# MultimodalFusion/multimodalfusion

Hardware: AMD Instinct MI355X
Metric: bags/sec fwd+bwd, path-AMIL 50k x 1024 synthetic bag (higher is better)
Workload: dtype f32; 1 GPU; path_attention_mil small gated K=4, one 50000x1024 N(0,1) bag per GPU per step, nll_surv alpha=0, train (1 dropout mask) mode, fwd+loss+bwd, grads materialised, one C-ABI call per bag (model.nll_step), 2 bags in flight per GPU on 2 HIP streams; instances_per_bag=50000, parallelism=dp1 (one bag per GPU per step), bags_in_flight=2

## Files before the change

### multimodalfusion_amd/csrc/mmf_amil_bwd.hip

```cpp
#include <cstdlib>

#include <type_traits>

#include "mmf_gemm_core.h"
#include "mmf_gemm_split.h"
#include "mmf_kernels.h"

namespace mmf {

__global__ __launch_bounds__(256) void bwd_prep_kernel(BwdPrepParams p) {
  __shared__ float red[4];
  const int tid = threadIdx.x, lane = tid & 63, wave = tid >> 6;
  const float m = p.stats[0], inv = 1.0f / p.stats[1];
  float dmm = 0.f;
  for (int c = lane; c < p.H; c += 64) dmm += p.dM[c] * p.M[c];
  dmm = wave_sum(dmm);
  float dbc = 0.f;
  const int64_t nw = (int64_t)gridDim.x * 4;
  for (int64_t i = (int64_t)blockIdx.x * 4 + wave; i < p.N; i += nw) {
    const float* hr = p.h + (size_t)i * p.H;
    float g = 0.f;
    for (int c = 4 * lane; c < p.H; c += 256) {
      float4 hv = ld4(hr + c), dv = ld4(p.dM + c);
      g += hv.x * dv.x + hv.y * dv.y + hv.z * dv.z + hv.w * dv.w;
    }
    g = wave_sum(g);
    if (lane == 0) {
      float pi = __expf(p.A_raw[i] - m) * inv;
      float d = pi * (g - dmm) + (p.gA ? p.gA[i] : 0.f);
      p.p[i] = pi;
      p.ds[i] = d;
      dbc += d;
    }
  }
  if (lane == 0) red[wave] = dbc;
  __syncthreads();
  if (tid == 0) p.dbc_part[blockIdx.x] = red[0] + red[1] + red[2] + red[3];
}

template <int ROWS, int NT, int MODE = -1, bool SEG = false>
struct LoadP_K {
  using Map = KMap<ROWS, NT>;
  GateBwdCtx g;
  rsrc_t ra, rb, rwc;
  int row0, tid, part, d0;
  uint32_t thr;
  float dscale;
  unsigned voff[Map::NV];
  uint32_t rbase[SEG ? Map::NV : 1];
  __device__ inline void init_seg(const uint32_t* ridx, int nrows) {
    if constexpr (SEG) {
#pragma unroll
      for (int i = 0; i < Map::NV; ++i) {
        const int rr = row0 + Map::row(tid, i);
        rbase[i] = (Map::valid(tid, i) && rr < nrows) ? ridx[rr] : 0u;
      }
    }
  }
  __device__ inline uint32_t idx_of(int i, int rr, int c) const {
    if constexpr (SEG) return rbase[i] + (uint32_t)c;
    else return (uint32_t)rr * (uint32_t)g.D + (uint32_t)c;
  }
  float dsr[Map::NV];
  float4 ra4[Map::NV], rb4[Map::NV], wc4;
  __device__ inline void init(const GateBwdCtx& g_, int row0_, int nrows) {
    g = g_; g.resolve_seed(); row0 = row0_; tid = threadIdx.x;
    thr = drop_threshold(g.drop_p);
    dscale = g.drop_p > 0.f ? 1.0f / (1.0f - g.drop_p) : 1.0f;
    const unsigned bytes = (unsigned)nrows * (unsigned)g.D * 4u;
    ra = make_rsrc(g.a, bytes);
    rb = make_rsrc(g.gated ? g.b : g.a, bytes);
    rwc = make_rsrc(g.Wc, (unsigned)g.D * 4u);
    rsrc_t rds = make_rsrc(g.ds, (unsigned)nrows * 4u);
#pragma unroll
    for (int i = 0; i < Map::NV; ++i) {
      int rr = row0 + Map::row(tid, i);
      bool ok = Map::valid(tid, i) && rr < nrows;
      voff[i] = ok ? ((unsigned)rr * (unsigned)g.D + 4u * Map::c4(tid, i)) * 4u : OOB;
      dsr[i] = bld1(rds, ok ? (unsigned)rr * 4u : OOB, 0);
    }
  }
  __device__ inline void init_lds(const GateBwdCtx& g_, int row0_, int nrows, const float* ds_lds) {
    g = g_; g.resolve_seed(); row0 = row0_; tid = threadIdx.x;
    thr = drop_threshold(g.drop_p);
    dscale = g.drop_p > 0.f ? 1.0f / (1.0f - g.drop_p) : 1.0f;
    const unsigned bytes = (unsigned)nrows * (unsigned)g.D * 4u;
    ra = make_rsrc(g.a, bytes);
    rb = make_rsrc(g.gated ? g.b : g.a, bytes);
    rwc = make_rsrc(g.Wc, (unsigned)g.D * 4u);
#pragma unroll
    for (int i = 0; i < Map::NV; ++i) {
      int rl = Map::row(tid, i), rr = row0 + rl;
      bool ok = Map::valid(tid, i) && rr < nrows;
      voff[i] = ok ? ((unsigned)rr * (unsigned)g.D + 4u * Map::c4(tid, i)) * 4u : OOB;
      dsr[i] = ok ? ds_lds[rl] : 0.f;
    }
  }
  __device__ inline void load_meta(int kt) {
    part = g.gated ? (kt & 1) : 0;
    d0 = (g.gated ? (kt >> 1) : kt) * KC;
  }
  __device__ inline void load(int kt) {
    load_meta(kt);
    if (part) return;
    const unsigned soff = (unsigned)d0 * 4u;
    wc4 = bld4(rwc, 16u * (tid & 7), soff);
#pragma unroll
    for (int i = 0; i < Map::NV; ++i) {
      ra4[i] = bld4(ra, voff[i], soff);
      rb4[i] = bld4(rb, voff[i], soff);
    }
  }
  template <bool GATED, bool DROP, int PART>
  __device__ inline void store_t(float* lds) const {
    const int c = d0 + 4 * (tid & 7);
#pragma unroll
    for (int i = 0; i < Map::NV; ++i) {
      if (!Map::valid(tid, i)) continue;
      int rr = row0 + Map::row(tid, i);
      uint32_t idx = idx_of(i, rr, c);
      float dummy;
      float4 o;
      o.x = gate_dp_t<GATED, DROP, PART>(g, ra4[i].x, rb4[i].x, wc4.x, dsr[i], idx + 0, thr, dscale, dummy);
      o.y = gate_dp_t<GATED, DROP, PART>(g, ra4[i].y, rb4[i].y, wc4.y, dsr[i], idx + 1, thr, dscale, dummy);
      o.z = gate_dp_t<GATED, DROP, PART>(g, ra4[i].z, rb4[i].z, wc4.z, dsr[i], idx + 2, thr, dscale, dummy);
      o.w = gate_dp_t<GATED, DROP, PART>(g, ra4[i].w, rb4[i].w, wc4.w, dsr[i], idx + 3, thr, dscale, dummy);
      st4(lds + Map::lds(tid, i), o);
    }
  }
  __device__ inline void store(float* lds) const {
    if constexpr (MODE >= 0) {
      constexpr bool GATED = (MODE & 2) != 0, DROP = (MODE & 1) != 0;
      if (GATED && part) store_t<GATED, DROP, 1>(lds);
      else store_t<GATED, DROP, 0>(lds);
      return;
    }
    const int c = d0 + 4 * (tid & 7);
#pragma unroll
    for (int i = 0; i < Map::NV; ++i) {
      if (!Map::valid(tid, i)) continue;
      int rr = row0 + Map::row(tid, i);
      uint32_t idx = idx_of(i, rr, c);
      float dummy;
      float4 o;
      o.x = gate_dp(g, part, ra4[i].x, rb4[i].x, wc4.x, dsr[i], idx + 0, thr, dscale, dummy);
      o.y = gate_dp(g, part, ra4[i].y, rb4[i].y, wc4.y, dsr[i], idx + 1, thr, dscale, dummy);
      o.z = gate_dp(g, part, ra4[i].z, rb4[i].z, wc4.z, dsr[i], idx + 2, thr, dscale, dummy);
      o.w = gate_dp(g, part, ra4[i].w, rb4[i].w, wc4.w, dsr[i], idx + 3, thr, dscale, dummy);
      st4(lds + Map::lds(tid, i), o);
    }
  }
};

template <int ROWS, int NT>
struct LoadWab_M {
  using Map = MMap<ROWS, NT>;
  rsrc_t ra, rb;
  bool gated;
  int D, tid;
  unsigned hb;
  unsigned voff[Map::NV];
  float4 r[Map::NV];
  __device__ inline void init(const float* wa, const float* wb, int H, int D_, int col0, bool gated_) {
    D = D_; tid = threadIdx.x; hb = (unsigned)H * 4u; gated = gated_ && wb != nullptr;
    ra = make_rsrc(wa, (unsigned)D * hb);
// ... 159 lines not shown
  __device__ inline void init_common(const GateBwdCtx& g_, int row0_, int nrows) {
    g = g_; g.resolve_seed(); row0 = row0_; tid = threadIdx.x;
    thr = drop_threshold(g.drop_p);
    dscale = g.drop_p > 0.f ? 1.0f / (1.0f - g.drop_p) : 1.0f;
    ra = make_rsrc(g.a, (unsigned)nrows * (unsigned)g.D * 4u);
    rwc = make_rsrc(g.Wc, (unsigned)g.D * 4u);
#pragma unroll
    for (int i = 0; i < NV; ++i) {
      const int idx = slot(tid, i), rr = row0 + krow(idx);
      voff[i] = rr < nrows ? ((unsigned)rr * (unsigned)g.D + 4u * (idx & 3)) * 4u : OOB;
    }
  }
  __device__ inline void init(const GateBwdCtx& g_, int row0_, int nrows) {
    init_common(g_, row0_, nrows);
    rsrc_t rds = make_rsrc(g.ds, (unsigned)nrows * 4u);
#pragma unroll
    for (int i = 0; i < NV; ++i) {
      const int rr = row0 + krow(slot(tid, i));
      dsr[i] = bld1(rds, rr < nrows ? (unsigned)rr * 4u : OOB, 0);
    }
  }
  __device__ inline void init_lds(const GateBwdCtx& g_, int row0_, int nrows, const float* ds_lds) {
    init_common(g_, row0_, nrows);
#pragma unroll
    for (int i = 0; i < NV; ++i) {
      const int rl = krow(slot(tid, i));
      dsr[i] = row0 + rl < nrows ? ds_lds[rl] : 0.f;
    }
  }
  __device__ inline void load(int kt) {
    d0 = kt * SKC;
    const unsigned soff = (unsigned)d0 * 4u;
    wc4 = bld4(rwc, 16u * (tid & 3), soff);
#pragma unroll
    for (int i = 0; i < NV; ++i) ra4[i] = bld4(ra, voff[i], soff);
  }
  __device__ inline void store_piece(float* lds, int i) const {
    const int c = d0 + 4 * (tid & 3);
    const int idx = slot(tid, i), rr = row0 + krow(idx);
    const uint32_t e0 = (uint32_t)rr * (uint32_t)g.D + (uint32_t)c;
    float dummy;
    float4 o;
    o.x = gate_dp_t<false, DROP, 0>(g, ra4[i].x, 0.f, wc4.x, dsr[i], e0 + 0, thr, dscale, dummy);
    o.y = gate_dp_t<false, DROP, 0>(g, ra4[i].y, 0.f, wc4.y, dsr[i], e0 + 1, thr, dscale, dummy);
    o.z = gate_dp_t<false, DROP, 0>(g, ra4[i].z, 0.f, wc4.z, dsr[i], e0 + 2, thr, dscale, dummy);
    o.w = gate_dp_t<false, DROP, 0>(g, ra4[i].w, 0.f, wc4.w, dsr[i], e0 + 3, thr, dscale, dummy);
    split_store4(lds + krow(idx) * SROW_F, idx & 3, o);
  }
  __device__ inline void store(float* lds) const {
#pragma unroll
    for (int i = 0; i < NV; ++i) store_piece(lds, i);
  }
};

template <int ROWS, int NT, bool GATED>
struct SplitWab_M {
  static constexpr int TOTAL = ROWS * 2, NV = (TOTAL + NT - 1) / NT, PIECES = NV;
  static_assert(TOTAL % NT == 0 || TOTAL < NT, "whole vector slots only");
  rsrc_t ra, rb;
  int tid;
  unsigned hb;
  unsigned voff[NV];
  float r[NV][8];
  __device__ inline void init(const float* wa, const float* wb, int H, int D, int col0, bool) {
    tid = TOTAL < NT ? (int)threadIdx.x % TOTAL : (int)threadIdx.x; hb = (unsigned)H * 4u;
    ra = make_rsrc(wa, (unsigned)D * hb);
    rb = make_rsrc(GATED ? wb : wa, (unsigned)D * hb);
#pragma unroll
    for (int i = 0; i < NV; ++i) {
      const int idx = tid + i * NT, c = col0 + idx % ROWS, kh = idx / ROWS;
      voff[i] = c < H ? (unsigned)(8 * kh) * hb + (unsigned)c * 4u : OOB;
    }
  }
  __device__ inline void load(int kt) {
    const bool second = GATED && (kt & 1);
    const unsigned soff = (unsigned)((GATED ? (kt >> 1) : kt) * SKC) * hb;
#pragma unroll
    for (int i = 0; i < NV; ++i)
#pragma unroll
      for (int j = 0; j < 8; ++j) r[i][j] = bld1(second ? rb : ra, voff[i], soff + (unsigned)j * hb);
  }
  __device__ inline void store_piece(float* lds, int i) const {
    const int idx = tid + i * NT;
    split_store8(lds + (idx % ROWS) * SROW_F, idx / ROWS, r[i]);
  }
  __device__ inline void store(float* lds) const {
#pragma unroll
    for (int i = 0; i < NV; ++i) store_piece(lds, i);
  }
};

template <class T, class LA, class LB>
__device__ inline void dh_split_mainloop(const LA& la0, const LB& lb0, int nk, float* lds, f32x16 (&acc)[T::MB][T::NB]) {
  const int tid = threadIdx.x, lane = tid & 63, wave = tid >> 6;
  const int wm = wave / T::WN, wn = wave % T::WN;
#pragma unroll
  for (int mb = 0; mb < T::MB; ++mb)
#pragma unroll
    for (int nb = 0; nb < T::NB; ++nb)
#pragma unroll
      for (int i = 0; i < 16; ++i) acc[mb][nb][i] = 0.f;
  LA la[2] = {la0, la0};
  LB lb[4] = {lb0, lb0, lb0, lb0};
  la[0].load_pair(0); la[1].load_pair(2);
#pragma unroll
  for (int j = 0; j < 4; ++j) lb[j].load(j);
  la[0].template store_part<0>(lds);
  lb[0].store(lds + T::A_FLOATS);
  __syncthreads();
  constexpr int NS = split_steps<T>();
  for (int kt0 = 0; kt0 < nk; kt0 += 4) {
    static_for<4>([&](auto jc) {
      constexpr int j = decltype(jc)::value;
      const int kt = kt0 + j;
      float* cur = lds + (j & 1) * T::STAGE_FLOATS;
      float* nxt = lds + ((j + 1) & 1) * T::STAGE_FLOATS;
      compute_chunk_split<T>(cur, cur + T::A_FLOATS, acc, wm, wn, lane, [&](int s) {
        if (s == 0) {
          if constexpr (j == 1) la[0].load_pair(kt0 + 4);
          else if constexpr (j == 3) la[1].load_pair(kt0 + 6);
        }
        if (s == (NS >= 4 ? 1 : 0)) lb[j].load(kt + 4);
        constexpr int PA = LA::NV;
#pragma unroll
        for (int q = 0; q < PA; ++q)
          if (s == q * (NS - 1) / PA) la[((j + 1) & 3) >> 1].template store_part_piece<(j + 1) & 1>(nxt, q);
        if (s == NS - 1) lb[(j + 1) & 3].store(nxt + T::A_FLOATS);
      });
      __syncthreads();
    });
  }
}

template <class T, bool FUSED, int MODE = -1, bool SEG = false>
__global__ __launch_bounds__(T::NT) void bwd_dh_kernel(BwdDhParams p) {
  static_assert(!(SEG && (FUSED || T::SPLIT)), "the grouped step runs K-prep on its own and the exact-fp32 tiles");
  extern __shared__ __align__(16) float lds[];
  int mt, nt;
  if (!tile_of_block(blockIdx.x, p.mt_count, p.nt_count, mt, nt)) return;
  const int row0 = mt * T::BM, col0 = nt * T::BN;
  const int tid = threadIdx.x, lane = tid & 63, wave = tid >> 6;
  float* ds_l = lds + 2 * T::STAGE_FLOATS;
  float* p_l = ds_l + T::BM;
  constexpr bool SGATED = T::SPLIT && MODE >= 2;
  std::conditional_t<T::SPLIT,
                     std::conditional_t<SGATED, SplitP_K<T::BM, T::NT, (SGATED ? MODE : 2)>, SplitP_U<T::BM, T::NT, (T::SPLIT && !SGATED ? MODE : 0)>>,
                     LoadP_K<T::BM, T::NT, MODE, SEG>> la;
  if constexpr (FUSED) {
    constexpr int NW = T::NT / 64;
    constexpr int RPW = (T::BM + NW - 1) / NW;
    float* g_l = p_l + T::BM + 16;
    const int LPR = p.H / 4;
    const int PPL = LPR / 64;
    float4 dm_l[4];
#pragma unroll
    for (int q = 0; q < 4; ++q) dm_l[q] = q < PPL ? ld4(p.dM + 4 * (lane + 64 * q)) : zero4();
    float dmm = 0.f;
    for (int c = lane; c < p.H; c += 64) dmm += p.dM[c] * p.Mpool[c];
    const float smax = p.stats[0], inv = 1.0f / p.stats[1];
    static_assert(T::BM <= T::NT, "one row per thread in K-prep");
    const int prow = row0 + tid;
    const bool pok = tid < T::BM && prow < p.N;
    const float araw = pok ? p.A_raw[prow] : 0.f;
    const float gav = (pok && p.gA) ? p.gA[prow] : 0.f;
    const int wr0 = wave * RPW, wr1 = wr0 + RPW < T::BM ? wr0 + RPW : T::BM;
    auto g_rows = [&](auto nrows_c, int rb) {
      constexpr int NR = decltype(nrows_c)::value;
      float part[NR];
#pragma unroll
      for (int u = 0; u < NR; ++u) {
        const int row = row0 + rb + u;
        const int rc = row < p.N ? row : (int)p.N - 1;
        float acc = 0.f;
#pragma unroll
        for (int q = 0; q < 4; ++q)
          if (q < PPL) {
            const float4 hv = ld4(p.h + (size_t)rc * p.H + 4 * (lane + 64 * q));
            acc += hv.x * dm_l[q].x + hv.y * dm_l[q].y + hv.z * dm_l[q].z + hv.w * dm_l[q].w;
          }
        part[u] = acc;
      }
#pragma unroll
      for (int u = 0; u < NR; ++u) part[u] = wave_sum(part[u]);
      if (lane < NR && rb + lane < wr1) {
        float gv = part[0];
#pragma unroll
        for (int u = 1; u < NR; ++u) gv = lane == u ? part[u] : gv;
        g_l[rb + lane] = gv;
      }
    };
    if (PPL == 1) {
      for (int rb = wr0; rb < wr1; rb += 16) g_rows(std::integral_constant<int, 16>{}, rb);
    } else {
      for (int rb = wr0; rb < wr1; rb += 8) g_rows(std::integral_constant<int, 8>{}, rb);
    }
    dmm = wave_sum(dmm);
    __syncthreads();
    float dbc = 0.f;
    if (tid < T::BM) {
      float pi = 0.f, d = 0.f;
      if (pok) {
        pi = __expf(araw - smax) * inv;
        d = pi * (g_l[tid] - dmm) + gav;
        if (nt == 0) { p.p_out[prow] = pi; p.ds_out[prow] = d; }
      }
      ds_l[tid] = d;
      p_l[tid] = pi;
      dbc = d;
    }
    dbc = wave_sum(dbc);
    float* red = p_l + T::BM;
    if (lane == 0) red[wave] = dbc;
    __syncthreads();
    if (tid == 0 && nt == 0) {
      float s = 0.f;
      for (int w = 0; w < NW; ++w) s += red[w];
      p.dbc_part[mt] = s;
    }
    la.init_lds(p.g, row0, (int)p.N, ds_l);
  } else {
    la.init(p.g, row0, (int)p.N);
    if constexpr (SEG && !T::SPLIT) la.init_seg(p.seg_ridx, (int)p.N);
  }
  std::conditional_t<T::SPLIT, SplitWab_M<T::BN, T::NT, SGATED>, LoadWab_M<T::BN, T::NT>> lb;
  lb.init(p.Wa, p.Wb, p.H, p.g.D, col0, p.g.gated != 0);
  f32x16 acc[T::MB][T::NB];
  f32x4acc acch[T::NB][2];
  const int nk = (p.g.gated ? 2 : 1) * p.g.D / (T::SPLIT ? SKC : KC);
  if constexpr (SGATED) {
    dh_split_mainloop<T>(la, lb, nk, lds, acc);
  } else if constexpr (T::SPLIT) {
    split_mainloop<T, 4>(la, lb, nk, lds, acc);
  } else if constexpr (T::NT == 256 && T::BM <= 64) {
    if (p.deep && p.g.gated) dh_mainloop_deep<T>(la, lb, nk, lds, acc);
    else gemm_mainloop<T, decltype(la), decltype(lb), false>(la, lb, nk, lds, acc);
  } else {
    gemm_mainloop<T, decltype(la), decltype(lb), FUSED && MODE >= 0>(la, lb, nk, lds, acc, acch);
  }
  {
    const int wm = wave / T::WN, wn = wave % T::WN;
    const int rr = lane >> 3, c4 = lane & 7;
    float* blk = lds + wave * (32 * EPI_STRIDE);
    constexpr int NBLK = T::MB * T::NB;
    float4 dm4[T::NB];
#pragma unroll
    for (int nb = 0; nb < T::NB; ++nb) {
      const int col = col0 + epilogue_col<T>(nb);
      dm4[nb] = (!SEG && p.dM && col < p.H) ? ld4(p.dM + col) : zero4();
    }
    if (p.relu_bits) {
      const int cbn = p.H >> 5;
      typedef unsigned long long u64;
      u64 mv[2];
      auto fetch_bits = [&](int b, int s) {
        const int mb = b / T::NB, nb = b % T::NB;
        const int64_t rb16 = (((int64_t)row0 + wm * (T::BM / T::WM) + mb * 32) >> 4) + (lane >> 3);
        const int cb = (col0 >> 5) + wn * T::NB + nb;
        const bool ok = rb16 * 16 < p.N && cb < cbn && lane < (mb == T::MB ? 8 : 16);
        mv[s] = ok ? p.relu_bits[((size_t)rb16 * cbn + cb) * 8 + (lane & 7)] : 0ull;
      };
      fetch_bits(0, 0);
#pragma unroll
      for (int b = 0; b < NBLK; ++b) {
        const int mb = b / T::NB, nb = b % T::NB, s = b & 1;
        if (b + 1 < NBLK) fetch_bits(b + 1, s ^ 1);
        float4 v[4];
        transpose_block(acc[mb][nb], blk, lane, v);
        const int r = wm * (T::BM / T::WM) + mb * 32 + rr, col = col0 + (wn * T::NB + nb) * 32 + 4 * c4;
        if (col >= p.H) continue;
        const float4 dm_c = dm4[nb];
#pragma unroll
        for (int t = 0; t < 4; ++t) {
          const int row = row0 + r + 8 * t;
          const float pi = FUSED ? p_l[r + 8 * t] : p.p[row < p.N ? row : (int)p.N - 1];
          const float4 dm = SEG ? ld4(p.dM + (size_t)p.seg_bag[row < p.N ? row : (int)p.N - 1] * p.H + col) : dm_c;
          const float raw[4] = {(v[t].x + pi * dm.x) * p.scale_h, (v[t].y + pi * dm.y) * p.scale_h,
                                (v[t].z + pi * dm.z) * p.scale_h, (v[t].w + pi * dm.w) * p.scale_h};
          float o[4];
#pragma unroll
          for (int e = 0; e < 4; ++e) {
            const unsigned lo = __builtin_amdgcn_readlane((unsigned)mv[s], 4 * t + e);
            const unsigned hi = __builtin_amdgcn_readlane((unsigned)(mv[s] >> 32), 4 * t + e);
            const u64 m = ((u64)hi << 32) | lo;
            asm volatile("v_cndmask_b32_e64 %0, 0, %1, %2" : "=v"(o[e]) : "v"(raw[e]), "s"(m));
          }
          if (row < p.N) st4(p.du + (size_t)row * p.H + col, make_float4(o[0], o[1], o[2], o[3]));
        }
      }
      if constexpr (T::HALF) {
#pragma unroll
        for (int nb = 0; nb < T::NB; ++nb) {
          fetch_bits(T::MB * T::NB + nb, 0);
          float4 v[2];
          transpose_half(acch[nb][0], acch[nb][1], blk, lane, v);
          const int r = wm * (T::BM / T::WM) + T::MB * 32 + rr, col = col0 + (wn * T::NB + nb) * 32 + 4 * c4;
          if (col >= p.H) continue;
          const float4 dm_c = dm4[nb];
#pragma unroll
          for (int t = 0; t < 2; ++t) {
            const int row = row0 + r + 8 * t;
            const float pi = FUSED ? p_l[r + 8 * t] : p.p[row < p.N ? row : (int)p.N - 1];
            const float4 dm = SEG ? ld4(p.dM + (size_t)p.seg_bag[row < p.N ? row : (int)p.N - 1] * p.H + col) : dm_c;
            const float raw[4] = {(v[t].x + pi * dm.x) * p.scale_h, (v[t].y + pi * dm.y) * p.scale_h,
                                  (v[t].z + pi * dm.z) * p.scale_h, (v[t].w + pi * dm.w) * p.scale_h};
            float o[4];
#pragma unroll
            for (int e = 0; e < 4; ++e) {
              const unsigned lo = __builtin_amdgcn_readlane((unsigned)mv[0], 4 * t + e);
              const unsigned hi = __builtin_amdgcn_readlane((unsigned)(mv[0] >> 32), 4 * t + e);
              const u64 m = ((u64)hi << 32) | lo;
              asm volatile("v_cndmask_b32_e64 %0, 0, %1, %2" : "=v"(o[e]) : "v"(raw[e]), "s"(m));
            }
            if (row < p.N) st4(p.du + (size_t)row * p.H + col, make_float4(o[0], o[1], o[2], o[3]));
          }
        }
      }
    } else {
    float4 hv[2][4];
    float pv[2][4];
    auto fetch = [&](int b, int s) {
      const int mb = b / T::NB, nb = b % T::NB;
      const int r = (wm * T::MB + mb) * 32 + rr, col = col0 + (wn * T::NB + nb) * 32 + 4 * c4;
#pragma unroll
      for (int t = 0; t < 4; ++t) {
        const int row = row0 + r + 8 * t;
        const int rc = row < p.N ? row : (int)p.N - 1;
        hv[s][t] = !p.h ? make_float4(1.f, 1.f, 1.f, 1.f) : (col < p.H ? ld4(p.h + (size_t)rc * p.H + col) : zero4());
        pv[s][t] = FUSED ? p_l[r + 8 * t] : (p.p ? p.p[rc] : 0.f);
      }
    };
    fetch(0, 0);
#pragma unroll
    for (int b = 0; b < NBLK; ++b) {
      const int mb = b / T::NB, nb = b % T::NB, s = b & 1;
      if (b + 1 < NBLK) fetch(b + 1, s ^ 1);
      float4 v[4];
      transpose_block(acc[mb][nb], blk, lane, v);
      const int r = (wm * T::MB + mb) * 32 + rr, col = col0 + (wn * T::NB + nb) * 32 + 4 * c4;
      if (col >= p.H) continue;
      const float4 dm_c = dm4[nb];
#pragma unroll
      for (int t = 0; t < 4; ++t) {
        const int row = row0 + r + 8 * t;
        if (row >= p.N) continue;
        const float4 dm = SEG ? ld4(p.dM + (size_t)p.seg_bag[row] * p.H + col) : dm_c;
        const float4 h4 = hv[s][t];
        const float pi = pv[s][t];
        float4 du;
        du.x = h4.x > 0.f ? (v[t].x + pi * dm.x) * p.scale_h : 0.f;
        du.y = h4.y > 0.f ? (v[t].y + pi * dm.y) * p.scale_h : 0.f;
        du.z = h4.z > 0.f ? (v[t].z + pi * dm.z) * p.scale_h : 0.f;
        du.w = h4.w > 0.f ? (v[t].w + pi * dm.w) * p.scale_h : 0.f;
        st4(p.du + (size_t)row * p.H + col, du);
      }
    }
    }
// ... 392 lines not shown
#pragma unroll
      for (int t = 0; t < 4; ++t) {
        const int row = rowmap(wm * 128 + 4 * (rr + 8 * t) + mb);
        if (row < 0) continue;
        float* o = out + (size_t)row * q.ldc + col;
        if (col < q.Ncols) st4(o, make_float4(v0[t].x, v1[t].x, v0[t].y, v1[t].y));
        if (col + 4 < q.Ncols) st4(o + 4, make_float4(v0[t].z, v1[t].z, v0[t].w, v1[t].w));
      }
    }
    return;
  }
  epilogue_rows<T>(acc, lds, [&](int mb, int nb, int r, int c, const float4 (&v)[4]) {
    const int col = tn * T::BN + c;
    if (col >= q.Ncols) return;
#pragma unroll
    for (int t = 0; t < 4; ++t) {
      const int row = rowmap(r + 8 * t);
      if (row >= 0) st4(out + (size_t)row * q.ldc + col, v[t]);
    }
  });
}

template <class T, bool GATED, int DROP>
__device__ inline void tn_gate_tile(const TnParams& p, const TnProblem& q,
                                    std::conditional_t<T::SPLIT, SplitM<T::BN, T::NT>, LoadM<T::BN, T::NT>>& lb, int split, int tm,
                                    int tn, int kbase, int kmax, int nk, int last_groups, bool do_sum, float* lds) {
  using LA = std::conditional_t<T::SPLIT, SplitA_M_Gate<T::BM, T::NT, GATED, (DROP > 0 ? 1 : 0)>, LoadA_M_Gate<T::BM, T::NT, GATED, DROP>>;
  constexpr int DT = LA::DT;
  const int D = p.g.D, d0 = tm * DT;
  LA la;
  la.init(p.g, d0, kbase, kmax, do_sum);
  if constexpr (!T::SPLIT && DROP == 2) la.rrix = make_rsrc(p.seg_ridx, (unsigned)(kmax > 0 ? kmax : 0) * 4u);
  f32x16 acc[T::MB][T::NB];
  if constexpr (T::SPLIT) split_mainloop<T, 2>(la, lb, nk, lds, acc);
  else gemm_mainloop<T>(la, lb, nk, lds, acc, nullptr, last_groups);
  tn_store<T>(q, split, tn, acc, lds, [&](int r) {
    const int half = r / DT, d = d0 + r - half * DT;
    return d < D ? half * D + d : -1;
  });
  if constexpr (T::SPLIT) {
    if (do_sum) {
      float* cs = q.colsum + (size_t)split * q.colsum_stride;
      colsum1_reduce_store<DT, T::NT>(lds, la.csum_a, cs, d0, D);
      if (GATED) colsum1_reduce_store<DT, T::NT>(lds, la.csum_b, cs + D, d0, D);
      if (q.colsum2) colsum1_reduce_store<DT, T::NT>(lds, la.csum2, q.colsum2 + (size_t)split * q.colsum2_stride, d0, D);
    }
  } else
  if (do_sum) {
    float* cs = q.colsum + (size_t)split * q.colsum_stride;
    colsum_reduce_store<DT, T::NT>(lds, la.csum_a, cs, d0, D);
    if (GATED) colsum_reduce_store<DT, T::NT>(lds, la.csum_b, cs + D, d0, D);
    if (q.colsum2) colsum_reduce_store<DT, T::NT>(lds, la.csum2, q.colsum2 + (size_t)split * q.colsum2_stride, d0, D);
  }
}

template <class T, int DROP = -1>
__global__ __launch_bounds__(T::NT) void tn_kernel(TnParams p) {
  extern __shared__ __align__(16) float lds[];
  const int b = blockIdx.x;
  int split, pi = 0, t;
  if (p.xcd_map == 2) {
    const unsigned e = p.map[b];
    if (e == 0xFFFFu) return;
    split = (int)(e >> 5);
    const int tg = (int)(e & 31u);
    for (int i = 1; i < p.nprob; ++i)
      if (tg >= p.prob[i].tile_begin) pi = i;
    t = tg - p.prob[pi].tile_begin;
  } else {
    for (int i = 1; i < p.nprob; ++i)
      if (b >= p.prob[i].block_begin) pi = i;
    const int rel = b - p.prob[pi].block_begin, nt = p.prob[pi].tiles_m * p.prob[pi].tiles_n;
    split = rel / nt;
    t = rel - split * nt;
  }
  const TnProblem& q = p.prob[pi];
  if (split >= q.splits) return;
  const int tm = t / q.tiles_n, tn = t - tm * q.tiles_n;
  const int64_t kb64 = (int64_t)split * q.k_per_split;
  const int kbase = (int)(kb64 < p.K ? kb64 : p.K);
  const int kmax = (int)((kb64 + q.k_per_split) < p.K ? (kb64 + q.k_per_split) : p.K);
  constexpr int CH = T::SPLIT ? SKC : KC;
  const int nk = T::SPLIT ? 2 * ((kmax - kbase + 2 * CH - 1) / (2 * CH)) : (kmax - kbase + CH - 1) / CH;
  int last_groups = 0;
  if constexpr (!T::SPLIT) last_groups = nk > 0 ? ((kmax - kbase) - (nk - 1) * KC + 2 * T::G - 1) / (2 * T::G) : 0;
  const bool do_sum = tn == 0 && q.colsum != nullptr;

  std::conditional_t<T::SPLIT, SplitM<T::BN, T::NT>, LoadM<T::BN, T::NT>> lb;
  lb.init(q.B, q.ldb, tn * T::BN, q.Ncols, kbase, kmax);
  if (q.kind == TN_A_PLAIN) {
    std::conditional_t<T::SPLIT, SplitA_M_Plain<T::BM, T::NT>, LoadA_M_Plain<T::BM, T::NT>> la;
    la.init(q.A, q.lda, tm * T::BM, q.M, kbase, kmax, do_sum);
    f32x16 acc[T::MB][T::NB];
    if constexpr (T::SPLIT) split_mainloop<T, 2>(la, lb, nk, lds, acc);
    else gemm_mainloop<T>(la, lb, nk, lds, acc, nullptr, last_groups);
    tn_store<T>(q, split, tn, acc, lds, [&](int r) { const int row = tm * T::BM + r; return row < q.M ? row : -1; });
    if (do_sum) {
      if constexpr (T::SPLIT) colsum1_reduce_store<T::BM, T::NT>(lds, la.csum, q.colsum + (size_t)split * q.colsum_stride, tm * T::BM, q.M);
      else colsum_reduce_store<T::BM, T::NT>(lds, la.csum, q.colsum + (size_t)split * q.colsum_stride, tm * T::BM, q.M);
    }
  } else if (p.g.gated) {
    tn_gate_tile<T, true, DROP>(p, q, lb, split, tm, tn, kbase, kmax, nk, last_groups, do_sum, lds);
  } else {
    tn_gate_tile<T, false, DROP>(p, q, lb, split, tm, tn, kbase, kmax, nk, last_groups, do_sum, lds);
  }
}

__global__ __launch_bounds__(256) void reduce_kernel(ReduceParams p) {
  const int b = blockIdx.x;
  int si = 0;
  for (int i = 1; i < p.nseg; ++i)
    if (b >= p.seg[i].block_begin) si = i;
  const ReduceSeg& s = p.seg[si];
  if (s.len < 4) {
    __shared__ float red[4];
    for (int e = 0; e < s.len; ++e) {
      float acc = 0.f;
      for (int k = threadIdx.x; k < s.nsplit; k += 256) acc += s.in[(size_t)k * s.stride + e];
      acc = wave_sum(acc);
      if ((threadIdx.x & 63) == 0) red[threadIdx.x >> 6] = acc;
      __syncthreads();
      if (threadIdx.x == 0) s.out[e] = (p.accumulate ? s.out[e] : 0.f) + (red[0] + red[1] + red[2] + red[3]);
      __syncthreads();
    }
    return;
  }
  if (s.tall) {
    __shared__ __align__(16) float part[16][64];
    const int cq = threadIdx.x & 15, grp = threadIdx.x >> 4;
    const int j = (b - s.block_begin) * 64 + 4 * cq;
    float4 acc = zero4();
    if (j < s.len) {
      const float* in = s.in + j;
      int k = grp;
      for (; k + 7 * 16 < s.nsplit; k += 8 * 16) {
        float4 v[8];
#pragma unroll
        for (int u = 0; u < 8; ++u) v[u] = ld4(in + (size_t)(k + 16 * u) * s.stride);
#pragma unroll
        for (int u = 0; u < 8; ++u) { acc.x += v[u].x; acc.y += v[u].y; acc.z += v[u].z; acc.w += v[u].w; }
      }
      for (; k < s.nsplit; k += 16) {
        float4 v = ld4(in + (size_t)k * s.stride);
        acc.x += v.x; acc.y += v.y; acc.z += v.z; acc.w += v.w;
      }
    }
    st4(&part[grp][4 * cq], acc);
    __syncthreads();
    if (threadIdx.x < 64) {
      float t = 0.f;
#pragma unroll
      for (int g = 0; g < 16; ++g) t += part[g][threadIdx.x];
      const int c = (b - s.block_begin) * 64 + threadIdx.x;
      if (c < s.len) s.out[c] = (p.accumulate ? s.out[c] : 0.f) + t;
    }
    return;
  }
  const int j = ((b - s.block_begin) * 256 + threadIdx.x) * 4;
  if (j >= s.len) return;
  if ((s.len & 3) == 0 && (s.stride & 3) == 0) {
    float4 acc = zero4();
    const float* in = s.in + j;
    int k = 0;
    for (; k + 8 <= s.nsplit; k += 8) {
      float4 v[8];
#pragma unroll
      for (int u = 0; u < 8; ++u) v[u] = ld4(in + (size_t)(k + u) * s.stride);
#pragma unroll
      for (int u = 0; u < 8; ++u) { acc.x += v[u].x; acc.y += v[u].y; acc.z += v[u].z; acc.w += v[u].w; }
    }
    for (; k < s.nsplit; ++k) {
      float4 v = ld4(in + (size_t)k * s.stride);
      acc.x += v.x; acc.y += v.y; acc.z += v.z; acc.w += v.w;
    }
    if (p.accumulate) { const float4 o = ld4(s.out + j); acc.x += o.x; acc.y += o.y; acc.z += o.z; acc.w += o.w; }
    st4(s.out + j, acc);
  } else {
    for (int e = j; e < j + 4 && e < s.len; ++e) {
      float acc = 0.f;
      for (int k = 0; k < s.nsplit; ++k) acc += s.in[(size_t)k * s.stride + e];
      s.out[e] = (p.accumulate ? s.out[e] : 0.f) + acc;
    }
  }
}

int launch_bwd_prep(BwdPrepParams p, hipStream_t st) {
  if (p.H % 4 != 0 || p.H > 1024) return MMF_ERR_SHAPE;
  { ProfScope ps("bwd_prep_kernel", st); hipLaunchKernelGGL(bwd_prep_kernel, dim3(p.n_groups), dim3(256), 0, st, p); }
  return hipGetLastError() == hipSuccess ? MMF_OK : MMF_ERR_LAUNCH;
}

constexpr int DH_MAX_ROWS = 224;

DhPlan plan_bwd_dh(int64_t N, int H, int D, int gated, int dropout, int split, int concurrent, int can_fuse, int dbc_cap) {
  static const int fuse_env = tune_int("MMF_FUSED_PREP", 1);
  static const int short_max = tune_int("MMF_DH_SHORT_MAX", 1024);
  static const int min_64x128 = tune_int("MMF_DH_64X128", 13000);
  const int mode = (gated ? 2 : 0) + (dropout ? 1 : 0);
  const bool split_k = split && ((gated ? 2 : 1) * D / SKC) % 4 == 0;
  const bool split_wide = split_k && use_wide_tiles(N, H, 1);
  const bool split_64 = split_k && !use_wide_tiles(N, H, 1) && N >= split_min_rows();
  const bool wide = use_wide_tiles(N, H, split);
  const bool big = (N / 128) * ((H + 127) / 128) >= 256;
  const bool deep_k = gated && (2 * D / KC) % 4 == 0;
  const bool short_64 = !use_wide_tiles(N, H, split_64) && !big && ((N + 63) / 64) * ((H + 63) / 64) <= short_max;
  auto wide_rows = [&](bool allow_half) {
    const int r = pick_wide_rows(N, H / 256, allow_half, concurrent != 0, DH_MAX_ROWS);
    return r >= 64 && r <= DH_MAX_ROWS && r % 16 == 0 ? r : 224;
  };

  int fuse_rows = 0;
  if (short_64) fuse_rows = 64;
  else if (split_64 || !wide) fuse_rows = 0;
  else fuse_rows = split_wide ? 224 : wide_rows(true);
  DhPlan pl{};
  pl.fused = can_fuse && fuse_env && fuse_rows > 0 && (N + fuse_rows - 1) / fuse_rows <= dbc_cap;
  pl.variant = -1;
  if (pl.fused && split_wide) {
    pl.kind = DH_SPLIT_WIDE; pl.rows = 224; pl.nt_count = H / 256; pl.variant = mode;
  } else if (split_64) {
    pl.kind = DH_SPLIT_64; pl.rows = 64; pl.nt_count = (H + 63) / 64; pl.variant = mode;
  } else if (wide) {
    pl.kind = DH_WIDE; pl.rows = pl.fused ? fuse_rows : wide_rows(false); pl.nt_count = H / 256;
    if (pl.fused && mode < 3) pl.variant = mode;
  } else if (big) {
    pl.kind = DH_128; pl.rows = 128; pl.nt_count = (H + 127) / 128;
  } else if (min_64x128 > 0 && N >= min_64x128 && pl.fused && deep_k && H % 128 == 0) {
    pl.kind = DH_64X128; pl.rows = 64; pl.nt_count = H / 128; pl.deep = 1;
  } else {
    pl.kind = DH_64; pl.rows = 64; pl.nt_count = (H + 63) / 64;
  }
  pl.mt_count = (int)((N + pl.rows - 1) / pl.rows);
  if (pl.kind == DH_64) pl.deep = short_grid((int64_t)pl.mt_count * pl.nt_count) && deep_k ? 1 : 0;
  pl.grid = grid_for_tiles(pl.mt_count, pl.nt_count);
  pl.extra_lds = pl.fused ? (3 * pl.rows + 16) * 4 : 0;
  pl.dbc_groups = pl.fused ? pl.mt_count : 0;
  return pl;
}

template <class T_, bool FUSED_, bool PLAIN_>
struct DhTile { using T = T_; static constexpr bool FUSED = FUSED_, PLAIN = PLAIN_; };
template <int ROWS>
using DhWide = DhTile<Tile<ROWS, 256, 1, 8, true, false>, true, ROWS % 32 == 0>;

template <class F>
static int with_dh_tile(const DhPlan& pl, F&& f) {
  switch (pl.kind) {
    case DH_SPLIT_WIDE: return f(DhTile<TileSp<224, 256, 1, 8>, true, false>{});
    case DH_SPLIT_64: return f(DhTile<TileSp<64, 64, 2, 2>, true, true>{});
    case DH_128: return f(DhTile<Tile<128, 128, 2, 2, true, false>, false, true>{});
    case DH_64X128: return f(DhTile<Tile<64, 128, 2, 2, true, false>, true, false>{});
    case DH_64: return f(DhTile<Tile<64, 64, 2, 2, true, false>, true, true>{});
    case DH_WIDE: return with_wide_rows<DH_MAX_ROWS>(pl.rows, [&](auto r) { return f(DhWide<decltype(r)::value>{}); });
  }
  return MMF_ERR_ARG;
}

template <int LAST, class F>
static int with_variant(int variant, F&& f) {
  switch (variant) {
    case 0: return f(std::integral_constant<int, 0>{});
    case 1: return f(std::integral_constant<int, 1>{});
    case 2: return f(std::integral_constant<int, 2>{});
    default: return f(std::integral_constant<int, LAST>{});
  }
}

template <bool SEG>
static int launch_dh_plan(const DhPlan& pl, BwdDhParams p, hipStream_t st) {
  if (p.g.D % KC != 0 || p.H % 4 != 0) return MMF_ERR_SHAPE;
  if (SEG && (pl.fused || p.split || !p.seg_bag || !p.seg_ridx || !p.dM || !p.p || !p.h)) return MMF_ERR_ARG;
  if (p.N <= 0) return MMF_OK;
  p.mt_count = pl.mt_count; p.nt_count = pl.nt_count; p.deep = pl.deep; p.fused_prep = pl.fused;
  return with_dh_tile(pl, [&](auto tile) -> int {
    using E = decltype(tile);
    using T = typename E::T;
    using Yes = std::true_type;
    using No = std::false_type;
    using RunTime = std::integral_constant<int, -1>;
    auto go = [&](auto fused, auto mode) -> int {
      return launch_tiled<T>(T::SPLIT ? "bwd_dh_split_kernel" : "bwd_dh_kernel",
                             bwd_dh_kernel<T, decltype(fused)::value, decltype(mode)::value, SEG>, p, pl.grid, st, pl.extra_lds);
    };
    if constexpr (SEG) {
      if constexpr (E::PLAIN && !T::SPLIT) return go(No{}, RunTime{});
    } else if (pl.fused) {
      if constexpr (E::FUSED && T::SPLIT) return with_variant<3>(pl.variant, [&](auto mode) { return go(Yes{}, mode); });
      else if constexpr (E::FUSED && T::BN == 256) return with_variant<-1>(pl.variant, [&](auto mode) { return go(Yes{}, mode); });
      else if constexpr (E::FUSED) return go(Yes{}, RunTime{});
    } else if constexpr (E::PLAIN) {
      if constexpr (T::SPLIT) return with_variant<3>(pl.variant, [&](auto mode) { return go(No{}, mode); });
      else return go(No{}, RunTime{});
    }
    return MMF_ERR_ARG;
  });
}
int launch_bwd_dh(const DhPlan& pl, BwdDhParams p, hipStream_t st) { return launch_dh_plan<false>(pl, p, st); }
int launch_bwd_dh_seg(const DhPlan& pl, BwdDhParams p, hipStream_t st) { return launch_dh_plan<true>(pl, p, st); }

__global__ __launch_bounds__(256) void group_bwd_prep_kernel(BwdPrepParams p, const int* bag) {
  __shared__ float red[4];
  const int tid = threadIdx.x, lane = tid & 63, wave = tid >> 6;
  int cur = -1;
  float dmm = 0.f, m = 0.f, inv = 1.f;
  const float* dM = p.dM;
  float dbc = 0.f;
  const int64_t nw = (int64_t)gridDim.x * 4;
  for (int64_t i = (int64_t)blockIdx.x * 4 + wave; i < p.N; i += nw) {
    const int b = __builtin_amdgcn_readfirstlane(bag[i]);
    if (b != cur) {
      cur = b;
      dM = p.dM + (size_t)b * p.H;
      const float* M = p.M + (size_t)b * p.H;
      float t = 0.f;
      for (int c = lane; c < p.H; c += 64) t += dM[c] * M[c];
      dmm = wave_sum(t);
      m = p.stats[2 * b];
      inv = 1.0f / p.stats[2 * b + 1];
    }
    const float* hr = p.h + (size_t)i * p.H;
    float gsum = 0.f;
    for (int c = 4 * lane; c < p.H; c += 256) {
      float4 hv = ld4(hr + c), dv = ld4(dM + c);
      gsum += hv.x * dv.x + hv.y * dv.y + hv.z * dv.z + hv.w * dv.w;
    }
    gsum = wave_sum(gsum);
    if (lane == 0) {
      float pi = __expf(p.A_raw[i] - m) * inv;
      float d = pi * (gsum - dmm) + (p.gA ? p.gA[i] : 0.f);
      p.p[i] = pi;
      p.ds[i] = d;
      dbc += d;
    }
  }
  if (lane == 0) red[wave] = dbc;
  __syncthreads();
  if (tid == 0) p.dbc_part[blockIdx.x] = red[0] + red[1] + red[2] + red[3];
}
int launch_group_bwd_prep(BwdPrepParams p, const int* bag, hipStream_t st) {
  if (!bag || p.n_groups < 1) return MMF_ERR_ARG;
  { ProfScope ps("group_bwd_prep_kernel", st); hipLaunchKernelGGL(group_bwd_prep_kernel, dim3(p.n_groups), dim3(256), 0, st, p, bag); }
  return hipGetLastError() == hipSuccess ? MMF_OK : MMF_ERR_LAUNCH;
}

template <bool ATTR, bool SEG = false>
static int launch_nn_tiles(NnParams p, hipStream_t st) {
  const char* name = SEG ? "gemm_nn_attr_seg_kernel" : ATTR ? "gemm_nn_attr_kernel" : "gemm_nn_kernel";
  const int ntn = (p.N + 127) / 128;
  if ((p.M / 128) * ntn >= 256) {
    using T = Tile<128, 128, 2, 2, true, false>;
    p.mt_count = (int)((p.M + 127) / 128); p.nt_count = ntn;
    return launch_tiled<T>(name, gemm_nn_kernel<T, ATTR, SEG>, p, grid_for_tiles(p.mt_count, p.nt_count), st);
  }
  using T = Tile<64, 64, 2, 2, true, false>;
  p.mt_count = (int)((p.M + 63) / 64); p.nt_count = (p.N + 63) / 64;
  return launch_tiled<T>(name, gemm_nn_kernel<T, ATTR, SEG>, p, grid_for_tiles(p.mt_count, p.nt_count), st);
}

int launch_nn(NnParams p, hipStream_t st) {
  if (p.K % KC != 0 || p.lda % 4 != 0 || p.ldb % 4 != 0 || p.N % 4 != 0) return MMF_ERR_SHAPE;
  if (p.M <= 0) return MMF_OK;
  return launch_nn_tiles<false>(p, st);
}

int launch_nn_attr(NnParams p, float* row_sum, float* row_abs, hipStream_t st) {
  if (!p.mulx || !p.rs_part || !p.ra_part || !row_sum || !row_abs) return MMF_ERR_ARG;
  if (p.K % KC != 0 || p.lda % 4 != 0 || p.ldb % 4 != 0 || p.N % 32 != 0 || p.ldx % 4 != 0 || (p.C && p.ldc % 4 != 0))
    return MMF_ERR_SHAPE;
  if (p.M <= 0) return MMF_OK;
  if (int e = launch_nn_tiles<true>(p, st)) return e;
  ProfScope ps("ig_rows_kernel", st);
  hipLaunchKernelGGL(ig_rows_kernel, dim3((unsigned)((p.M + 255) / 256)), dim3(256), 0, st, p.rs_part, p.ra_part, p.M,
                     p.N / 32, row_sum, row_abs);
  return hipGetLastError() == hipSuccess ? MMF_OK : MMF_ERR_LAUNCH;
}

int launch_nn_attr_seg(NnParams p, float* row_sum, float* row_abs, hipStream_t st) {
  if (!p.rs_part || !p.ra_part || !row_sum || !row_abs) return MMF_ERR_ARG;
  if (p.kseg < 32 || p.kseg % 32 != 0 || p.N % p.kseg != 0 || p.N / p.kseg < 1 || p.N / p.kseg > 4) return MMF_ERR_SHAPE;
  const int nseg = p.N / p.kseg;
  for (int m = 0; m < nseg; ++m)
    if (!p.segx[m]) return MMF_ERR_ARG;
  if (p.K % KC != 0 || p.lda % 4 != 0 || p.ldb % 4 != 0) return MMF_ERR_SHAPE;
  if (p.M <= 0) return MMF_OK;
  if (int e = launch_nn_tiles<true, true>(p, st)) return e;
  const int64_t n = p.M * nseg;
  ProfScope ps("ig_rows_seg_kernel", st);
  hipLaunchKernelGGL(ig_rows_seg_kernel, dim3((unsigned)((n + 255) / 256)), dim3(256), 0, st, p.rs_part, p.ra_part, p.M,
                     p.kseg / 32, nseg, row_sum, row_abs);
  return hipGetLastError() == hipSuccess ? MMF_OK : MMF_ERR_LAUNCH;
}

int launch_ig_fold(const IgFoldParams& p, hipStream_t st) {
  if (!p.du || !p.G) return MMF_ERR_ARG;
  if (p.H % 4 != 0 || p.N < 1 || p.st.S < 0 || p.st.S > GROUP_MAX) return MMF_ERR_SHAPE;
  if (p.st.S == 0 && !p.first) return MMF_OK;
  const size_t n4 = (size_t)p.N * p.H / 4;
  ProfScope ps("ig_fold_kernel", st);
  hipLaunchKernelGGL(ig_fold_kernel, dim3((unsigned)((n4 + 255) / 256)), dim3(256), 0, st, p);
  return hipGetLastError() == hipSuccess ? MMF_OK : MMF_ERR_LAUNCH;
}

TnPlan plan_tn(int64_t K, int split, const TnShape* shapes, int nshape) {
  static const int env_wide = tune_int("MMF_TN_WIDE", 1);
  static const int kmin = tune_int("MMF_TN_WIDE_MIN", 12288);
  static const int env_splits = tune_int("MMF_TN_SPLITS", 0);
  static const int env_gate = tune_int("MMF_TN_GATE_SPLITS", -1);
  TnPlan pl{};
  pl.tile = env_wide && K >= kmin ? 256 : 128;
  pl.kind = pl.tile == 256 ? (split ? TN_SPLIT_256 : TN_256) : (split && K >= split_min_rows() ? TN_SPLIT_128 : TN_128);
  const int td = pl.tile;
  int t_plain = 0, t_gate = 0;
  for (int i = 0; i < nshape; ++i)
    (shapes[i].gate ? t_gate : t_plain) += ((shapes[i].M + td - 1) / td) * ((shapes[i].Ncols + td - 1) / td);
  pl.tiles = t_plain + t_gate;
  auto capped = [&](int64_t s) { if (s > (K + 127) / 128) s = (K + 127) / 128; return (int)(s < 1 ? 1 : s); };
  auto kps = [&](int s) { return (int)(((K + s - 1) / s + 3) / 4 * 4); };
  pl.splits = capped(env_splits > 0 ? env_splits : (td == 256 ? 256 : 512) / (pl.tiles > 0 ? pl.tiles : 1));
  pl.k_per_split = kps(pl.splits);
  pl.splits_g = pl.splits;
  if (t_plain > 0 && t_gate > 0) {
    if (td == 256 && pl.splits >= 8) {
      const int cap = pl.splits + (pl.splits * 12 + 99) / 100;
      const int sg = (256 - t_plain * pl.splits) / t_gate;
      pl.splits_g = sg > cap ? cap : sg < pl.splits ? pl.splits : sg;
    }
    if (env_gate > 0) pl.splits_g = env_gate;
  }
  pl.k_per_split_g = kps(pl.splits_g);
  return pl;
}

template <class T>
static int launch_tn_grid(const TnParams& p, int grid, hipStream_t st) {
  if constexpr (!T::SPLIT) {
    if (p.seg_ridx && p.g.drop_p > 0.f) return launch_tiled<T>("tn_kernel", tn_kernel<T, 2>, p, grid, st);
  }
  if constexpr (T::BM == 256 || T::SPLIT) {
    const char* name = T::SPLIT ? "tn_split_kernel" : "tn_kernel";
    if (p.g.drop_p > 0.f) return launch_tiled<T>(name, tn_kernel<T, 1>, p, grid, st);
    return launch_tiled<T>(name, tn_kernel<T, 0>, p, grid, st);
  } else {
    return launch_tiled<T>("tn_kernel", tn_kernel<T>, p, grid, st);
  }
}

template <class T>
static int launch_tn_t(const TnPlan& pl, TnParams p, hipStream_t st) {
  p.tile = pl.tile; p.splits = pl.splits; p.k_per_split = pl.k_per_split;
  int tiles = 0, blocks = 0;
  for (int i = 0; i < p.nprob; ++i) {
    TnProblem& q = p.prob[i];
    if (q.Ncols % 4 != 0 || q.ldb % 4 != 0 || q.M % 4 != 0) return MMF_ERR_SHAPE;
    if (q.kind == TN_A_PLAIN && q.lda % 4 != 0) return MMF_ERR_SHAPE;
    q.splits = q.kind == TN_A_GATE ? pl.splits_g : pl.splits;
    q.k_per_split = q.kind == TN_A_GATE ? pl.k_per_split_g : pl.k_per_split;
    if (q.k_per_split % 4 != 0 || q.k_per_split < 4) return MMF_ERR_ARG;
    if (q.kind == TN_A_GATE) {
      const int dt = p.g.gated ? T::BM / 2 : T::BM;
      q.tiles_m = (p.g.D + dt - 1) / dt;
    } else {
      q.tiles_m = (q.M + T::BM - 1) / T::BM;
    }
    q.tiles_n = (q.Ncols + T::BN - 1) / T::BN;
    q.tile_begin = tiles;
    q.block_begin = blocks;
    tiles += q.tiles_m * q.tiles_n;
    blocks += q.tiles_m * q.tiles_n * q.splits;
  }
  if (blocks == 0) return MMF_OK;
  p.total_tiles = tiles;
  static const int env_xcd = tune_int("MMF_TN_XCD", -1);
  p.xcd_map = env_xcd == 0 ? 0 : 2;
  if (p.xcd_map == 2) {
    int bin_load[8] = {0, 0, 0, 0, 0, 0, 0, 0};
    bool ok = tiles <= 32;
    for (int i = 0; i < 512; ++i) p.map[i] = 0xFFFFu;
    int order[6], np = p.nprob;
    for (int i = 0; i < np; ++i) order[i] = i;
    for (int i = 0; i < np; ++i)
      for (int j = i + 1; j < np; ++j)
        if (p.prob[order[j]].tiles_m * p.prob[order[j]].tiles_n > p.prob[order[i]].tiles_m * p.prob[order[i]].tiles_n) {
          const int t = order[i]; order[i] = order[j]; order[j] = t;
        }
    for (int oi = 0; oi < np && ok; ++oi) {
      const TnProblem& q = p.prob[order[oi]];
      const int n = q.tiles_m * q.tiles_n;
      if (n == 0) continue;
      if (q.splits >= 2048) { ok = false; break; }
      for (int s = 0; s < q.splits && ok; ++s) {
        int x = 0;
        for (int k = 1; k < 8; ++k) if (bin_load[k] < bin_load[x]) x = k;
        if (8 * (bin_load[x] + n) > 512) { ok = false; break; }
        for (int t = 0; t < n; ++t) p.map[x + 8 * (bin_load[x] + t)] = (uint16_t)((s << 5) | (q.tile_begin + t));
        bin_load[x] += n;
      }
    }
    if (ok) {
      int mx = 0;
      for (int k = 0; k < 8; ++k) mx = bin_load[k] > mx ? bin_load[k] : mx;
      return launch_tn_grid<T>(p, 8 * mx, st);
    }
    p.xcd_map = 0;
  }
  return launch_tn_grid<T>(p, blocks, st);
}

int launch_tn(const TnPlan& pl, TnParams p, hipStream_t st) {
  switch (pl.kind) {
    case TN_SPLIT_256: return launch_tn_t<TileSp<256, 256, 2, 4>>(pl, p, st);
    case TN_256: return launch_tn_t<Tile<256, 256, 2, 4, false, false, 2>>(pl, p, st);
    case TN_SPLIT_128: return launch_tn_t<TileSp<128, 128, 2, 2>>(pl, p, st);
    case TN_128: return launch_tn_t<Tile<128, 128, 2, 2, false, false, 2>>(pl, p, st);
  }
  return MMF_ERR_ARG;
}

int launch_reduce(ReduceParams p, hipStream_t st) {
  int blocks = 0;
  for (int i = 0; i < p.nseg; ++i) {
    ReduceSeg& s = p.seg[i];
    s.tall = s.nsplit >= 64 && s.len >= 4 && (s.len & 3) == 0 && (s.stride & 3) == 0;
    s.block_begin = blocks;
    blocks += s.tall ? (s.len + 63) / 64 : (s.len + 1023) / 1024;
  }
  if (blocks == 0) return MMF_OK;
  { ProfScope ps("reduce_kernel", st); hipLaunchKernelGGL(reduce_kernel, dim3(blocks), dim3(256), 0, st, p); }
  return hipGetLastError() == hipSuccess ? MMF_OK : MMF_ERR_LAUNCH;
}

}
```

### multimodalfusion_amd/csrc/mmf_amil_fwd.hip

```cpp
#include <cstdlib>

#include "mmf_gemm_core.h"
#include "mmf_gemm_split.h"
#include "mmf_kernels.h"

namespace mmf {

__device__ inline float apply_act(float v, int act) {
  switch (act) {
    case ACT_RELU: return fmaxf(v, 0.f);
    case ACT_TANH: return fast_tanh(v);
    case ACT_SIGMOID: return fast_sigmoid(v);
    case ACT_SELU: {
      const float alpha = 1.6732632423543772f, scale = 1.0507009873554805f;
      return scale * (v > 0.f ? v : alpha * (__expf(v) - 1.0f));
    }
    default: return v;
  }
}

struct PartSrc {
  unsigned bytes;
  unsigned base;
  unsigned slab;
  int S;
};

template <class T, int ACT, bool DROP, bool SEG = false>
__device__ inline void linear_epilogue(const LinearParams& p, f32x16 (&acc)[T::MB][T::NB], f32x4acc (*acch)[2], float* lds,
                                       int row0, int col0, const PartSrc ps = PartSrc{}) {
  const uint32_t thr = drop_threshold(p.drop_p);
  const float scale = DROP ? 1.0f / (1.0f - p.drop_p) : 1.0f;
  const uint32_t dkey = p.drop_key + (p.seed_dev ? *p.seed_dev : 0u);
  float4 bias4[T::NB];
#pragma unroll
  for (int nb = 0; nb < T::NB; ++nb) {
    const int col = col0 + epilogue_col<T>(nb);
    bias4[nb] = (p.bias && col < p.N) ? ld4(p.bias + col) : zero4();
  }
  const int lane = threadIdx.x & 63;
  auto rows_op = [&](auto nt_c, int nb, int r, int c, const float4* v) {
    constexpr int NTR = decltype(nt_c)::value;
    const int col = col0 + c;
    const bool col_ok = col < p.N;
    const float4 b4 = bias4[nb];
    unsigned long long mine = 0ull;
#pragma unroll
    for (int t = 0; t < NTR; ++t) {
      const int row = row0 + r + 8 * t;
      const bool ok = col_ok && row < p.M;
      float y[4] = {v[t].x + b4.x, v[t].y + b4.y, v[t].z + b4.z, v[t].w + b4.w};
      uint32_t idx;
      if constexpr (SEG) idx = (row < p.M ? p.seg_ridx[row] : 0u) + (uint32_t)col;
      else idx = (uint32_t)row * (uint32_t)p.N + (uint32_t)col;
#pragma unroll
      for (int e = 0; e < 4; ++e) {
        if constexpr (ACT == ACT_RELU) y[e] = fmaxf(y[e], 0.f);
        else if constexpr (ACT < 0) y[e] = apply_act(y[e], p.act);
        if constexpr (DROP) y[e] = keep(dkey, idx + e, thr) ? y[e] * scale : 0.f;
      }
      if (p.relu_bits) {
#pragma unroll
        for (int e = 0; e < 4; ++e) {
          const unsigned long long bal = __ballot(ok && y[e] > 0.f);
          if (lane == 4 * t + e) mine = bal;
        }
      }
      if (ok) st4(p.y + (size_t)row * p.N + col, make_float4(y[0], y[1], y[2], y[3]));
    }
    if (p.relu_bits && lane < 4 * NTR) {
      const size_t rb16 = ((size_t)(row0 + r - (lane >> 3)) >> 4) + (lane >> 3), cb = (size_t)(col0 + c - 4 * (lane & 7)) >> 5;
      if ((int64_t)rb16 * 16 < p.M && (int)(cb * 32) < p.N) p.relu_bits[(rb16 * (size_t)(p.N >> 5) + cb) * 8 + (lane & 7)] = mine;
    }
  };
  if (ps.S > 0) {
    const int wave = threadIdx.x >> 6, wm = wave / T::WN, wn = wave % T::WN;
    const int rr = lane >> 3, c4 = lane & 7;
    constexpr int NBLK = T::MB * T::NB;
    const rsrc_t prs = make_rsrc(p.kpart, ps.bytes);
    float4 buf[2][4];
    auto fetch = [&](int b, int rows4, float4 (&v)[4]) {
      const int mb = b / T::NB, nb = b % T::NB;
      const int r = wm * (T::BM / T::WM) + mb * 32 + rr, c = (wn * T::NB + nb) * 32 + 4 * c4;
#pragma unroll
      for (int t = 0; t < 4; ++t) {
        if (t >= rows4) break;
        const unsigned o = ps.base + (unsigned)((r + 8 * t) * T::BN + c) * 4u;
        float4 a = bld4_dev(prs, o, 0);
        for (int k = 1; k < ps.S; ++k) {
          const float4 q = bld4_dev(prs, o, (unsigned)k * ps.slab);
          a.x += q.x; a.y += q.y; a.z += q.z; a.w += q.w;
        }
        v[t] = a;
      }
    };
    fetch(0, 4, buf[0]);
#pragma unroll
    for (int b = 0; b < NBLK; ++b) {
      const int mb = b / T::NB, nb = b % T::NB;
      if (b + 1 < NBLK) fetch(b + 1, 4, buf[(b + 1) & 1]);
      else if constexpr (T::HALF) fetch(T::MB * T::NB, 2, buf[(b + 1) & 1]);
      rows_op(std::integral_constant<int, 4>{}, nb, wm * (T::BM / T::WM) + mb * 32 + rr, (wn * T::NB + nb) * 32 + 4 * c4, buf[b & 1]);
    }
    if constexpr (T::HALF) {
#pragma unroll
      for (int nb = 0; nb < T::NB; ++nb) {
        if (nb + 1 < T::NB) fetch(T::MB * T::NB + nb + 1, 2, buf[(NBLK + nb + 1) & 1]);
        rows_op(std::integral_constant<int, 2>{}, nb, wm * (T::BM / T::WM) + T::MB * 32 + rr, (wn * T::NB + nb) * 32 + 4 * c4,
                buf[(NBLK + nb) & 1]);
      }
    }
    return;
  }
  epilogue_rows<T>(acc, lds, [&](int mb, int nb, int r, int c, const float4 (&v)[4]) {
    rows_op(std::integral_constant<int, 4>{}, nb, r, c, v);
  });
  if constexpr (T::HALF) {
    const int wave = threadIdx.x >> 6, wm = wave / T::WN, wn = wave % T::WN;
    float* blk = lds + wave * (32 * EPI_STRIDE);
#pragma unroll
    for (int nb = 0; nb < T::NB; ++nb) {
      float4 v[2];
      transpose_half(acch[nb][0], acch[nb][1], blk, lane, v);
      rows_op(std::integral_constant<int, 2>{}, nb, wm * (T::BM / T::WM) + T::MB * 32 + (lane >> 3),
              (wn * T::NB + nb) * 32 + 4 * (lane & 7), v);
    }
  }
}

template <class T>
__device__ inline bool ksplit_publish(const LinearParams& p, f32x16 (&acc)[T::MB][T::NB], f32x4acc (*acch)[2], float* lds,
                                      int tile, int ks, PartSrc& ps) {
  const int S = p.ksplit;
  ps.bytes = (unsigned)((size_t)p.mt_count * p.nt_count * S * T::BM * T::BN * 4u);
  const rsrc_t prs = make_rsrc(p.kpart, ps.bytes);
  ps.slab = (unsigned)(T::BM * T::BN * 4);
  ps.base = (unsigned)tile * (unsigned)S * ps.slab;
  ps.S = S;
  const unsigned mine = ps.base + (unsigned)ks * ps.slab;
  epilogue_rows<T>(acc, lds, [&](int mb, int nb, int r, int c, const float4 (&v)[4]) {
#pragma unroll
    for (int t = 0; t < 4; ++t) bst4_dev(prs, mine + (unsigned)((r + 8 * t) * T::BN + c) * 4u, 0, v[t]);
  });
  if constexpr (T::HALF) {
    const int lane = threadIdx.x & 63, wave = threadIdx.x >> 6, wm = wave / T::WN, wn = wave % T::WN;
    float* blk = lds + wave * (32 * EPI_STRIDE);
#pragma unroll
    for (int nb = 0; nb < T::NB; ++nb) {
      float4 v[2];
      transpose_half(acch[nb][0], acch[nb][1], blk, lane, v);
      const int r = wm * (T::BM / T::WM) + T::MB * 32 + (lane >> 3), c = (wn * T::NB + nb) * 32 + 4 * (lane & 7);
#pragma unroll
      for (int t = 0; t < 2; ++t) bst4_dev(prs, mine + (unsigned)((r + 8 * t) * T::BN + c) * 4u, 0, v[t]);
    }
  }
  asm volatile("s_waitcnt vmcnt(0)" ::: "memory");
  __syncthreads();
  unsigned* flag = reinterpret_cast<unsigned*>(lds + (T::NT / 64) * 32 * EPI_STRIDE);
  if (threadIdx.x == 0) {
    const unsigned old = __hip_atomic_fetch_add(p.ktick + tile, 1u, __ATOMIC_RELAXED, __HIP_MEMORY_SCOPE_AGENT);
    if (old == (unsigned)(S - 1)) __hip_atomic_store(p.ktick + tile, 0u, __ATOMIC_RELAXED, __HIP_MEMORY_SCOPE_AGENT);
    flag[0] = old;
  }
  __syncthreads();
  return flag[0] == (unsigned)(S - 1);
}

template <class T, bool SEG = false>
__global__ __launch_bounds__(T::NT) void linear_nt_kernel(LinearParams p) {
  extern __shared__ __align__(16) float lds[];
  const int S = p.ksplit > 1 ? p.ksplit : 1;
  int mt, ntk;
  if (!tile_of_block(blockIdx.x, p.mt_count, p.nt_count * S, mt, ntk)) return;
  const int nt = ntk % p.nt_count, ks = ntk / p.nt_count;
  const int row0 = mt * T::BM, col0 = nt * T::BN;
  const int nk = p.K / KC / S;

  LoadK<T::BM, T::NT> la;
  la.init_segments(p.x, p.nseg, p.kseg, p.ldx, row0, (int)p.M);
  LoadK<T::BN, T::NT> lb;
  lb.init(p.w, p.K, col0, p.N);
  la.kt0 = lb.kt0 = ks * nk;

  f32x16 acc[T::MB][T::NB];
  f32x4acc acch[T::NB][2];
  if constexpr (T::NT == 256 && T::BM <= 64) {
    if (p.deep) gemm_mainloop_deep<T, 4>(la, lb, nk, lds, acc);
    else gemm_mainloop<T>(la, lb, nk, lds, acc);
  } else {
    gemm_mainloop<T>(la, lb, nk, lds, acc, acch);
  }
  PartSrc ps{};
  if (S > 1) {
    if (!ksplit_publish<T>(p, acc, acch, lds, mt * p.nt_count + nt, ks, ps)) return;
  }
  const bool drop = p.drop_p > 0.f;
  if constexpr (SEG) {
    linear_epilogue<T, ACT_RELU, true, true>(p, acc, acch, lds, row0, col0, ps);
    return;
  }
  if (p.act == ACT_RELU) {
    if (drop) linear_epilogue<T, ACT_RELU, true>(p, acc, acch, lds, row0, col0, ps);
    else linear_epilogue<T, ACT_RELU, false>(p, acc, acch, lds, row0, col0, ps);
  } else if (p.act == ACT_NONE && !drop) {
    linear_epilogue<T, ACT_NONE, false>(p, acc, acch, lds, row0, col0, ps);
  } else if (drop) {
    linear_epilogue<T, -1, true>(p, acc, acch, lds, row0, col0, ps);
  } else {
    linear_epilogue<T, -1, false>(p, acc, acch, lds, row0, col0, ps);
  }
}

template <class T>
__global__ __launch_bounds__(T::NT) void linear_nt_split_kernel(LinearParams p) {
  extern __shared__ __align__(16) float lds[];
  int mt, nt;
  if (!tile_of_block(blockIdx.x, p.mt_count, p.nt_count, mt, nt)) return;
  const int row0 = mt * T::BM, col0 = nt * T::BN;
  SplitK<T::BM, T::NT> la;
  la.init(p.x[0], p.ldx, row0, (int)p.M);
  SplitK<T::BN, T::NT> lb;
  lb.init(p.w, p.K, col0, p.N);
  f32x16 acc[T::MB][T::NB];
  split_mainloop<T, 4>(la, lb, p.K / SKC, lds, acc);
  const bool drop = p.drop_p > 0.f;
  if (p.act == ACT_RELU) {
    if (drop) linear_epilogue<T, ACT_RELU, true>(p, acc, nullptr, lds, row0, col0);
    else linear_epilogue<T, ACT_RELU, false>(p, acc, nullptr, lds, row0, col0);
  } else if (p.act == ACT_NONE && !drop) {
    linear_epilogue<T, ACT_NONE, false>(p, acc, nullptr, lds, row0, col0);
  } else if (drop) {
    linear_epilogue<T, -1, true>(p, acc, nullptr, lds, row0, col0);
  } else {
    linear_epilogue<T, -1, false>(p, acc, nullptr, lds, row0, col0);
  }
}

template <int ROWS, int NT, bool GATED, bool HALVES>
struct LoadGateW {
  using Map = KMap<ROWS, NT>;
  rsrc_t ra, rb;
  int tid;
  int which[Map::NV];
  unsigned voff[Map::NV];
  float4 r[Map::NV];
  __device__ inline void init(const float* wa, const float* wb, int H, int D, int d0) {
    tid = threadIdx.x;
    ra = make_rsrc(wa, (unsigned)D * (unsigned)H * 4u);
    rb = make_rsrc(GATED ? wb : wa, (unsigned)D * (unsigned)H * 4u);
#pragma unroll
    for (int i = 0; i < Map::NV; ++i) {
      const int j = Map::row(tid, i);
      int w, d;
      if (!GATED) { w = 0; d = d0 + j; }
      else if (HALVES) { w = j >= ROWS / 2 ? 1 : 0; d = d0 + j - w * (ROWS / 2); }
      else { w = (j >> 5) & 1; d = d0 + (j >> 6) * 32 + (j & 31); }
      which[i] = __builtin_amdgcn_readfirstlane(w);
      voff[i] = (Map::valid(tid, i) && d < D) ? ((unsigned)d * (unsigned)H + 4u * Map::c4(tid, i)) * 4u : OOB;
    }
  }
  __device__ inline void load(int kt) {
    const unsigned soff = (unsigned)(kt * KC) * 4u;
#pragma unroll
    for (int i = 0; i < Map::NV; ++i) r[i] = bld4(which[i] ? rb : ra, voff[i], soff);
  }
  __device__ inline void store(float* lds) const {
#pragma unroll
    for (int i = 0; i < Map::NV; ++i)
      if (Map::valid(tid, i)) st4(lds + Map::lds(tid, i), r[i]);
  }
};

template <class T, bool GATED, bool SEG = false>
__device__ inline void gate_fwd_tile(const GateFwdParams& p, float* lds, int row0, int nt);

template <class T, bool GATED, bool SEG = false>
__global__ __launch_bounds__(T::NT) void gate_fwd_kernel(GateFwdParams p) {
  extern __shared__ __align__(16) float lds[];
  int mt, nt;
  if (!tile_of_block(blockIdx.x, p.mt_count, p.nt_count, mt, nt)) return;
  gate_fwd_tile<T, GATED, SEG>(p, lds, (int)p.row_begin + mt * T::BM, nt);
}

template <class TB, class TS, bool GATED, bool SEG = false>
__global__ __launch_bounds__(TB::NT) void gate_fwd_mixed_kernel(GateFwdParams p) {
  static_assert(TB::NT == TS::NT && TB::BN == TS::BN, "mixed tiles share the launch shape");
  extern __shared__ __align__(16) float lds[];
  int r = 0;
  for (int i = 1; i < p.nreg; ++i)
    if ((int)blockIdx.x >= p.reg[i].grid_begin) r = i;
  int mt, nt;
  if (!tile_of_block(blockIdx.x - p.reg[r].grid_begin, p.reg[r].mt_count, p.nt_count, mt, nt)) return;
  if (p.reg[r].tall) gate_fwd_tile<TB, GATED, SEG>(p, lds, (int)p.reg[r].row0 + mt * TB::BM, nt);
  else gate_fwd_tile<TS, GATED, SEG>(p, lds, (int)p.reg[r].row0 + mt * TS::BM, nt);
}

template <class T, bool GATED, bool SEG>
__device__ inline void gate_fwd_tile(const GateFwdParams& p, float* lds, int row0, int nt) {
  constexpr int DT = GATED ? T::BN / 2 : T::BN;
  const int d0 = nt * DT;

  std::conditional_t<T::SPLIT, SplitK<T::BM, T::NT>, LoadK<T::BM, T::NT>> la;
  la.init(p.h, p.H, row0, (int)p.row_end);
  std::conditional_t<T::SPLIT, SplitGateW<T::BN, T::NT, GATED>, LoadGateW<T::BN, T::NT, GATED, false>> lb;
  lb.init(p.Wa, p.Wb, p.H, p.D, d0);

  f32x16 acc[T::MB][T::NB];
  if constexpr (T::SPLIT) {
    split_mainloop<T, 4>(la, lb, p.H / SKC, lds, acc);
  } else if constexpr (T::BM <= 64) {
    if (p.deep) gemm_mainloop_deep<T, 4>(la, lb, p.H / KC, lds, acc);
    else gemm_mainloop<T>(la, lb, p.H / KC, lds, acc);
  } else {
    gemm_mainloop<T>(la, lb, p.H / KC, lds, acc);
  }

  const int tid = threadIdx.x, lane = tid & 63, wave = tid >> 6;
  const int wm = wave / T::WN, wn = wave % T::WN;
  const int rr = lane >> 3, c4 = lane & 7;
  const uint32_t thr = drop_threshold(p.drop_p);
  const bool drop = p.drop_p > 0.f;
  const float dscale = drop ? 1.0f / (1.0f - p.drop_p) : 1.0f;
  const uint32_t sdev = p.seed_dev ? *p.seed_dev : 0u;
  const uint32_t key_a = p.key_a + sdev, key_b = p.key_b + sdev;
  float* blk = lds + wave * (32 * EPI_STRIDE);
  float* sred = lds + (T::NT / 64) * (32 * EPI_STRIDE);

  constexpr int NPAIR = GATED ? T::NB / 2 : T::NB;
  float4 ba_r[NPAIR], bb_r[NPAIR], wc_r[NPAIR];
#pragma unroll
  for (int t = 0; t < NPAIR; ++t) {
    const int d = d0 + (wn * NPAIR + t) * 32 + 4 * c4;
    const bool dok = d < p.D;
    ba_r[t] = dok ? ld4(p.ba + d) : zero4();
    bb_r[t] = (GATED && dok) ? ld4(p.bb + d) : zero4();
    wc_r[t] = dok ? ld4(p.Wc + d) : zero4();
  }
#pragma unroll
  for (int mb = 0; mb < T::MB; ++mb) {
    float rowsum[4] = {0.f, 0.f, 0.f, 0.f};
#pragma unroll
    for (int t = 0; t < NPAIR; ++t) {
      const int d = d0 + (wn * NPAIR + t) * 32 + 4 * c4;
      const bool dok = d < p.D;
      float4 va[4], vb[4];
      transpose_block(acc[mb][GATED ? 2 * t : t], blk, lane, va);
      if constexpr (GATED) transpose_block(acc[mb][2 * t + 1], blk, lane, vb);
      const float4 ba4 = ba_r[t], bb4 = bb_r[t], wc4 = wc_r[t];
#pragma unroll
      for (int q = 0; q < 4; ++q) {
        const int row = row0 + (wm * T::MB + mb) * 32 + rr + 8 * q;
        float av[4] = {fast_tanh(va[q].x + ba4.x), fast_tanh(va[q].y + ba4.y), fast_tanh(va[q].z + ba4.z), fast_tanh(va[q].w + ba4.w)};
        float bv[4] = {1.f, 1.f, 1.f, 1.f};
        if constexpr (GATED) {
          bv[0] = fast_sigmoid(vb[q].x + bb4.x); bv[1] = fast_sigmoid(vb[q].y + bb4.y);
          bv[2] = fast_sigmoid(vb[q].z + bb4.z); bv[3] = fast_sigmoid(vb[q].w + bb4.w);
        }
        if (row < p.row_end && dok) {
          const size_t o = (size_t)row * p.D + d;
          if (p.a) {
            st4(p.a + o, make_float4(av[0], av[1], av[2], av[3]));
            if constexpr (GATED) st4(p.b + o, make_float4(bv[0], bv[1], bv[2], bv[3]));
          }
          const float wc[4] = {wc4.x, wc4.y, wc4.z, wc4.w};
          uint32_t idx;
          if constexpr (SEG) idx = p.seg_ridx[row] + (uint32_t)d;
          else idx = (uint32_t)row * (uint32_t)p.D + (uint32_t)d;
          if (drop) {
#pragma unroll
            for (int e = 0; e < 4; ++e) {
              const float ad = keep(key_a, idx + e, thr) ? av[e] * dscale : 0.f;
              float bd = bv[e];
              if constexpr (GATED) bd = keep(key_b, idx + e, thr) ? bd * dscale : 0.f;
              rowsum[q] += ad * bd * wc[e];
            }
          } else {
#pragma unroll
            for (int e = 0; e < 4; ++e) rowsum[q] += av[e] * bv[e] * wc[e];
          }
        }
      }
    }
#pragma unroll
    for (int q = 0; q < 4; ++q) {
      float s = rowsum[q];
      s += __shfl_xor(s, 1, 64); s += __shfl_xor(s, 2, 64); s += __shfl_xor(s, 4, 64);
      if (c4 == 0) sred[wn * T::BM + (wm * T::MB + mb) * 32 + rr + 8 * q] = s;
    }
  }
  __syncthreads();
  for (int i = tid; i < T::BM; i += T::NT) {
    int row = row0 + i;
    if (row < p.row_end) {
      float s = 0.f;
#pragma unroll
      for (int w = 0; w < T::WN; ++w) s += sred[w * T::BM + i];
      p.s_part[(size_t)nt * p.N + row] = s;
    }
  }
}


__device__ __forceinline__ void pool_partial_rows(const PoolParams& p, int g, int64_t r0, int64_t r1) {
  __shared__ float s_lds[POOL_MAX_ROWS];
  __shared__ float red[256];
  __shared__ __align__(16) float vred[1024];
  const int tid = threadIdx.x;
  const int nrows = r1 > r0 ? (int)(r1 - r0) : 0;
  const float bc = p.bc ? p.bc[0] : 0.f;

  float lmax = -INFINITY;
  for (int i = tid; i < nrows; i += 256) {
    float s = bc;
    for (int t = 0; t < p.n_parts; ++t) s += p.s_part[(size_t)t * p.N + r0 + i];
    p.A_raw[r0 + i] = s;
    s_lds[i] = s;
    lmax = fmaxf(lmax, s);
  }
  lmax = wave_max(lmax);
  if ((tid & 63) == 0) red[tid >> 6] = lmax;
  __syncthreads();
  const float m = fmaxf(fmaxf(red[0], red[1]), fmaxf(red[2], red[3]));
  __syncthreads();

  const int VPR = p.H / 4;
  const int RG = 256 / VPR;
  const int cv = tid % VPR, rg = tid / VPR;
  float4 v = zero4();
  float lsum = 0.f;
  int i = rg;
  for (; i + 7 * RG < nrows; i += 8 * RG) {
    float4 hv[8];
    float e[8];
#pragma unroll
    for (int u = 0; u < 8; ++u) hv[u] = ld4(p.h + (size_t)(r0 + i + u * RG) * p.H + 4 * cv);
#pragma unroll
    for (int u = 0; u < 8; ++u) e[u] = __expf(s_lds[i + u * RG] - m);
#pragma unroll
    for (int u = 0; u < 8; ++u) {
      v.x += e[u] * hv[u].x; v.y += e[u] * hv[u].y; v.z += e[u] * hv[u].z; v.w += e[u] * hv[u].w;
      if (cv == 0) lsum += e[u];
    }
  }
  for (; i < nrows; i += RG) {
    float e = __expf(s_lds[i] - m);
    float4 hv = ld4(p.h + (size_t)(r0 + i) * p.H + 4 * cv);
    v.x += e * hv.x; v.y += e * hv.y; v.z += e * hv.z; v.w += e * hv.w;
    if (cv == 0) lsum += e;
  }
  st4(vred + (rg * VPR + cv) * 4, v);
  if (cv == 0) red[rg] = lsum;
  __syncthreads();
  float* out = p.partials + (size_t)g * (2 + p.H);
  if (tid < VPR) {
    float4 s = zero4();
    for (int q = 0; q < RG; ++q) {
      float4 t = ld4(vred + (q * VPR + tid) * 4);
      s.x += t.x; s.y += t.y; s.z += t.z; s.w += t.w;
    }
    out[2 + 4 * tid + 0] = s.x; out[2 + 4 * tid + 1] = s.y;
    out[2 + 4 * tid + 2] = s.z; out[2 + 4 * tid + 3] = s.w;
  }
  if (tid == 0) {
    float l = 0.f;
    for (int q = 0; q < RG; ++q) l += red[q];
    out[0] = nrows > 0 ? m : -INFINITY;
    out[1] = l;
  }
}

__global__ __launch_bounds__(256) void pool_partial_kernel(PoolParams p) {
  const int g = blockIdx.x;
  const int64_t r0 = (int64_t)g * p.rows_per_group;
  const int64_t r1 = r0 + p.rows_per_group < p.N ? r0 + p.rows_per_group : p.N;
  pool_partial_rows(p, g, r0, r1);
}

struct TailPre {
  float wk_row[16];
  float wk_col[8];
  float bk;
  float c;
  long long y;
};
__device__ inline void tail_preload(const PoolParams& p, TailPre& r) {
  const HeadTail& t = p.tail;
  const int tid = threadIdx.x, lane = tid & 63, wave = tid >> 6;
#pragma unroll
  for (int j = 0; j < 16; ++j) r.wk_row[j] = (wave < t.K && lane + 64 * j < p.H) ? t.Wk[(size_t)wave * p.H + lane + 64 * j] : 0.f;
#pragma unroll
  for (int k = 0; k < 8; ++k) r.wk_col[k] = (k < t.K && tid < p.H) ? t.Wk[(size_t)k * p.H + tid] : 0.f;
  r.bk = (wave < t.K && lane == 0) ? t.bk[wave] : 0.f;
  r.c = (tid == 0 && t.c) ? t.c[0] : 0.f;
  r.y = (tid == 0 && t.Y) ? (long long)t.Y[0] : 0;
}
template <bool M_IN_LDS, bool BWD = true>
__device__ inline void head_tail(const PoolParams& p, const TailPre& r, float* sm ) {
  const HeadTail& t = p.tail;
  const int tid = threadIdx.x, lane = tid & 63, wave = tid >> 6;
  const int H = p.H, K = t.K;
  float* Ml = sm;
  float* z = sm + 1024;
  float *hz = z + 32, *S = z + 64, *gH = z + 96, *gS = z + 128;
  if constexpr (!M_IN_LDS)
    for (int c = tid; c < H; c += 1024) Ml[c] = p.M[c];
  __syncthreads();
  if (wave < K) {
    float acc = 0.f;
#pragma unroll
    for (int j = 0; j < 16; ++j)
      if (lane + 64 * j < H) acc += Ml[lane + 64 * j] * r.wk_row[j];
    acc = wave_sum(acc);
    if (lane == 0) z[wave] = acc + r.bk;
  }
  for (int k = 16 + wave; k < K; k += 16) {
    float acc = 0.f;
    for (int c = lane; c < H; c += 64) acc += Ml[c] * t.Wk[(size_t)k * H + c];
    acc = wave_sum(acc);
    if (lane == 0) z[k] = acc + t.bk[k];
  }
  __syncthreads();
  if (tid == 0) {
    float run = 1.f, best = -INFINITY, ssum = 0.f;
    int arg = 0;
    for (int k = 0; k < K; ++k) {
      const float zz = z[k];
      hz[k] = 1.0f / (1.0f + expf(-zz));
      run *= (1.0f - hz[k]);
      S[k] = run;
      ssum += run;
      t.logits[k] = zz; t.hazards[k] = hz[k]; t.S[k] = run;
      if (zz > best) { best = zz; arg = k; }
    }
    t.Y_hat[0] = arg;
    if (t.risk) t.risk[0] = -ssum;
    if (t.Y) {
      if constexpr (BWD)
        for (int k = 0; k < K; ++k) { gH[k] = 0.f; gS[k] = 0.f; }
      const long long y64 = r.y;
      float l;
      if (y64 < 0 || y64 >= K) {
        l = __builtin_nanf("");
      } else {
        const int y = (int)y64;
        const float c = r.c;
        const float sp_y = y == 0 ? 1.0f : S[y - 1];
        const float hy = hz[y];
        const float unc = -(1.f - c) * (logf(fmaxf(sp_y, t.eps)) + logf(fmaxf(hy, t.eps)));
        const float sp_y1 = S[y];
        const float cen = -c * logf(fmaxf(sp_y1, t.eps));
        if constexpr (BWD) {
          if (y > 0 && sp_y >= t.eps) gS[y - 1] += -(1.f - c) / sp_y;
          if (hy >= t.eps) gH[y] += -(1.f - c) / hy;
          if (sp_y1 >= t.eps) gS[y] += -(1.f - t.alpha) * c / sp_y1;
        }
        l = (1.f - t.alpha) * (cen + unc) + t.alpha * unc;
      }
      t.loss[0] = l;
      if constexpr (BWD)
        for (int k = 0; k < K; ++k) {
          float g = gH[k];
          for (int j = k; j < K; ++j) {
            float prod = 1.f;
            for (int u = 0; u <= j; ++u)
              if (u != k) prod *= (1.0f - hz[u]);
            g -= gS[j] * prod;
          }
          z[k] = g * hz[k] * (1.0f - hz[k]) * t.loss_scale;
        }
    }
  }
  if (!BWD || !t.Y) return;
  __syncthreads();
  for (int c = tid; c < H; c += 1024) {
    float acc = 0.f;
    if (c == tid) {
#pragma unroll
      for (int k = 0; k < 8; ++k)
        if (k < K) acc += z[k] * r.wk_col[k];
      for (int k = 8; k < K; ++k) acc += z[k] * t.Wk[(size_t)k * H + c];
    } else {
      for (int k = 0; k < K; ++k) acc += z[k] * t.Wk[(size_t)k * H + c];
    }
    t.dM[c] = acc;
    for (int k = 0; k < K; ++k) {
      float* o = t.dWk + (size_t)k * H + c;
      const float v = z[k] * Ml[c];
      *o = t.accumulate ? *o + v : v;
    }
  }
  if (tid < K) t.dbk[tid] = t.accumulate ? t.dbk[tid] + z[tid] : z[tid];
}

constexpr int MERGE_MAX_GROUPS = 4096;
__global__ __launch_bounds__(1024) void pool_merge_kernel(PoolParams p) {
  __shared__ float wl[MERGE_MAX_GROUPS];
  __shared__ float red[32];
  __shared__ float colred[1024];
  const int tid = threadIdx.x, lane = tid & 63, wave = tid >> 6;
  const int stride = 2 + p.H;
  float m = -INFINITY;
  for (int g = tid; g < p.n_groups; g += 1024) {
    float mg = p.partials[(size_t)g * stride];
    wl[g] = mg;
    m = fmaxf(m, mg);
  }
  m = wave_max(m);
  if (lane == 0) red[wave] = m;
  __syncthreads();
  m = red[0];
#pragma unroll
  for (int i = 1; i < 16; ++i) m = fmaxf(m, red[i]);
  float l = 0.f;
  for (int g = tid; g < p.n_groups; g += 1024) {
    float mg = wl[g];
    float w = mg > -INFINITY ? __expf(mg - m) : 0.f;
    wl[g] = w;
    l += p.partials[(size_t)g * stride + 1] * w;
  }
  l = wave_sum(l);
  if (lane == 0) red[16 + wave] = l;
  __syncthreads();
  l = 0.f;
#pragma unroll
  for (int i = 0; i < 16; ++i) l += red[16 + i];
  const int cl = tid & 31, sl = tid >> 5;
  const int c = blockIdx.x * 32 + cl;
  float acc = 0.f;
  const float* q = p.partials + 2 + c;
#pragma unroll 8
  for (int g = sl; g < p.n_groups; g += 32) acc += q[(size_t)g * stride] * wl[g];
  colred[tid] = acc;
  __syncthreads();
  if (tid < 32) {
    float s = 0.f;
#pragma unroll
    for (int i = 0; i < 32; ++i) s += colred[i * 32 + tid];
    p.M[c] = s / l;
  }
  if (blockIdx.x == 0 && tid == 0) { p.stats[0] = m; p.stats[1] = l; }
}

__global__ __launch_bounds__(1024) void head_tail_kernel(PoolParams p) {
  __shared__ float tail_sm[1024 + 160];
  TailPre pre;
  tail_preload(p, pre);
  head_tail<false>(p, pre, tail_sm);
}

__global__ __launch_bounds__(256) void score_sum_kernel(const float* s_part, int n_parts, const float* bc, float* A, int64_t N) {
  const int64_t i = (int64_t)blockIdx.x * 256 + threadIdx.x;
  if (i >= N) return;
  float s = bc ? bc[0] : 0.f;
  for (int t = 0; t < n_parts; ++t) s += s_part[(size_t)t * N + i];
  A[i] = s;
}
int launch_score_sum(const float* s_part, int n_parts, const float* bc, float* A, int64_t N, hipStream_t st) {
  { ProfScope ps("score_sum_kernel", st);
    hipLaunchKernelGGL(score_sum_kernel, dim3((unsigned)((N + 255) / 256)), dim3(256), 0, st, s_part, n_parts, bc, A, N); }
  return hipGetLastError() == hipSuccess ? MMF_OK : MMF_ERR_LAUNCH;
}

bool short_grid(int64_t workgroups) {
  static const int env = tune_int("MMF_DEEP", 1);
  static const int cap = tune_int("MMF_DEEP_MAX", 1024);
  return env && workgroups <= cap;
}

using TileNT128 = Tile<128, 128, 2, 2, true, true>;
using TileNT64 = Tile<64, 64, 2, 2, true, true>;

static inline bool use_big_tiles(int64_t M, int N) { return (M / 128) * ((N + 127) / 128) >= 256; }

template <int ROWS>
using TileW = Tile<ROWS, 256, 1, 8, true, true>;

int pick_wide_rows(int64_t M, int ntn, bool allow_half, bool concurrent, int max_rows) {
  static const int env = tune_int("MMF_WIDE_ROWS", 0);
  if (env > 0 && (env % 32 == 0 || allow_half)) return env;
  const int cus = concurrent ? 224 : 256;
  int best = 224;
  double bestc = 1e30;
  for (int rows = max_rows; rows >= 64; rows -= 16) {
    if (rows % 32 != 0 && !allow_half) continue;
    int64_t tiles = ((M + rows - 1) / rows) * ntn;
    int64_t rounds = (tiles + cus - 1) / cus;
    double c = (double)rounds * (rows / 32.0 + 0.35);
    if (c < bestc) { bestc = c; best = rows; }
  }
  return best;
}
bool use_wide_tiles(int64_t M, int N, int split) {
  static const int env = tune_int("MMF_WIDE", 1);
  static const int min_env = tune_int("MMF_WIDE_MIN", 0);
  const int min_rows = min_env > 0 ? min_env : (split ? 80 * 256 : 64 * 256);
  return env && N % 256 == 0 && M * (int64_t)(N / 256) >= min_rows;
}

int split_min_rows() {
  static const int env = tune_int("MMF_SPLIT_MIN", 1);
  return env;
}

LinearPlan plan_linear(int64_t M, int N, int K, int nseg, int kseg, int allow_half, int concurrent, int split, int tick_words) {
  static const int max_wg = tune_int("MMF_KSPLIT_MAX_WG", 512);
  static const int max_tiles = tune_int("MMF_KSPLIT_MAX_TILES", 128);
  static const int deep_seg = tune_int("MMF_DEEP_SEG", 1);
  LinearPlan pl{};
  pl.kind = LIN_64; pl.rows = 64; pl.ksplit = 1;
  if (M <= 0) return pl;
  const bool can_split = split && K % (4 * SKC) == 0 && nseg == 1;
  if (can_split && use_wide_tiles(M, N, 1)) {
    pl.kind = LIN_SPLIT_WIDE; pl.rows = 224;
  } else if (use_wide_tiles(M, N, can_split)) {
    const int r = pick_wide_rows(M, N / 256, allow_half != 0, concurrent != 0, 240);
    pl.kind = LIN_WIDE; pl.rows = r >= 64 && r <= 240 && r % 16 == 0 ? r : 224;
  } else if (!can_split && use_big_tiles(M, N)) {
    pl.kind = LIN_128; pl.rows = 128;
  } else if (can_split && M >= split_min_rows()) {
    pl.kind = LIN_SPLIT_64;
  }
  const int bn = pl.kind == LIN_SPLIT_WIDE || pl.kind == LIN_WIDE ? 256 : pl.rows;
  pl.mt_count = (int)((M + pl.rows - 1) / pl.rows); pl.nt_count = (N + bn - 1) / bn;
  const int64_t tiles = (int64_t)pl.mt_count * pl.nt_count;
  const int nk = K / KC;
  const bool seg_deep = nseg == 1 || kseg % (4 * KC) == 0;
  if (pl.kind == LIN_64) {
    if (tiles <= tick_words && tiles <= max_tiles && N % 4 == 0 && K % KC == 0 && seg_deep)
      for (int S = 4; S >= 2 && pl.ksplit == 1; S -= 2)
        if (tiles * S <= max_wg && nk % (4 * S) == 0 && nk / S >= 8) pl.ksplit = S;
    if (pl.ksplit > 1) {
      pl.kind = LIN_KSPLIT_64;
      pl.deep = short_grid(tiles * pl.ksplit) ? 1 : 0;
      pl.kpart_floats = pl.ksplit * (int)tiles * 64 * 64;
    } else {
      pl.deep = short_grid(tiles) && nk % 4 == 0 && (nseg == 1 || (deep_seg && seg_deep)) ? 1 : 0;
    }
  }
  pl.grid = grid_for_tiles(pl.mt_count, pl.nt_count * pl.ksplit);
  return pl;
}
size_t linear_ksplit_floats(int64_t M, int N, int K, int nseg, int kseg) {
  return (size_t)plan_linear(M, N, K, nseg, kseg, 0, 0, 0, 0x7fffffff).kpart_floats;
}

template <bool SEG>
static int launch_linear_impl(LinearParams p, hipStream_t st) {
  if (p.K % KC != 0 || (p.nseg > 1 && p.kseg % KC != 0)) return MMF_ERR_SHAPE;
  if (p.N % 4 != 0) return MMF_ERR_SHAPE;
  if (p.ldx % 4 != 0) return MMF_ERR_ALIGN;
  if (p.M <= 0) return MMF_OK;
  const LinearPlan pl = plan_linear(p.M, p.N, p.K, p.nseg, p.kseg, p.allow_half, p.concurrent, p.split,
                                    p.kpart && p.ktick ? p.ktick_words : 0);
  p.mt_count = pl.mt_count; p.nt_count = pl.nt_count; p.ksplit = pl.ksplit; p.deep = pl.deep;
  auto go = [&](auto tile) -> int {
    using T = decltype(tile);
    void (*kern)(LinearParams);
    if constexpr (T::SPLIT) kern = linear_nt_split_kernel<T>; else kern = linear_nt_kernel<T, SEG>;
    return launch_tiled<T>(T::SPLIT ? "linear_nt_split_kernel" : "linear_nt_kernel", kern, p, pl.grid, st);
  };
  switch (pl.kind) {
    case LIN_SPLIT_WIDE: return go(TileSp<224, 256, 1, 8>{});
    case LIN_SPLIT_64: return go(TileSp<64, 64, 2, 2>{});
    case LIN_128: return go(TileNT128{});
    case LIN_KSPLIT_64:
    case LIN_64: return go(TileNT64{});
    case LIN_WIDE: return with_wide_rows<240>(pl.rows, [&](auto r) { return go(TileW<decltype(r)::value>{}); });
  }
  return MMF_ERR_ARG;
}

int launch_linear(LinearParams p, hipStream_t st) { return launch_linear_impl<false>(p, st); }
int launch_linear_seg(LinearParams p, hipStream_t st) {
  if (!p.seg_ridx || p.split || p.act != ACT_RELU) return MMF_ERR_ARG;
  return p.drop_p > 0.f ? launch_linear_impl<true>(p, st) : launch_linear_impl<false>(p, st);
}

int gate_parts(int D, int gated) { return gated ? (D + 63) / 64 : (D + 127) / 128; }

GatePlan plan_gate_fwd(int64_t N, int H, int D, int gated, int split) {
  static const int big_min = tune_int("MMF_GATE_BIG_MIN", 400);
  static const int env_gate = tune_int("MMF_GATE_MIXED", -1);
  GatePlan pl{};
  pl.kind = GATE_64; pl.nt_count = gate_parts(D, gated);
  if (N <= 0) return pl;
  const bool split_k = split && H % (4 * SKC) == 0;
  if ((N / 128) * pl.nt_count < big_min) {
    pl.split = split_k && N >= split_min_rows(); pl.mt_count = (int)((N + 63) / 64);
    pl.deep = !pl.split && short_grid((int64_t)pl.mt_count * pl.nt_count) && (H / KC) % 4 == 0 ? 1 : 0;
    pl.grid = grid_for_tiles(pl.mt_count, pl.nt_count);
    return pl;
  }
  pl.split = split_k;
  const int mixed = env_gate >= 0 ? env_gate : (split_k ? 2 : 1);
  const int64_t mt = (N + 127) / 128, slots = 512, total = mt * pl.nt_count;
  const int R = (int)(total / slots);
  if (!mixed || R < 2 || slots % (2 * pl.nt_count) != 0) {
    pl.kind = GATE_128; pl.mt_count = (int)mt;
    pl.grid = grid_for_tiles(pl.mt_count, pl.nt_count);
    return pl;
  }
  pl.kind = GATE_MIXED;
  const int half_m = (int)(slots / 2 / pl.nt_count);
  int64_t row = 0;
  auto region = [&](int tall, int64_t m_tiles) {
    if (m_tiles <= 0) return;
    pl.reg[pl.nreg++] = {(int)row, (int)m_tiles, pl.grid, tall};
    pl.grid += grid_for_tiles((int)m_tiles, pl.nt_count);
    pl.mt_count += (int)m_tiles;
    row += m_tiles * (tall ? 128 : 64);
  };
  if (mixed == 2) {
    region(1, (total - total % slots) / pl.nt_count);
  } else {
    region(1, half_m);
    region(0, half_m);
    region(1, (int64_t)half_m * (2 * R - 2));
    region(0, half_m);
  }
  region(0, (N - row + 63) / 64);
  return pl;
}

template <bool SEG>
static int launch_gate_fwd_impl(GateFwdParams p, hipStream_t st) {
  if (p.H % KC != 0 || p.D % 32 != 0) return MMF_ERR_SHAPE;
  if (p.N <= 0) return MMF_OK;
  const GatePlan pl = plan_gate_fwd(p.N, p.H, p.D, p.gated, p.split);
  p.nt_count = pl.nt_count; p.mt_count = pl.mt_count; p.deep = pl.deep; p.nreg = pl.nreg;
  p.row_begin = 0; p.row_end = p.N;
  for (int i = 0; i < pl.nreg; ++i) p.reg[i] = {pl.reg[i].row0, pl.reg[i].mt_count, pl.reg[i].grid_begin, pl.reg[i].tall};
  auto go = [&](auto tb, auto... ts) -> int {
    using TB = decltype(tb);
    constexpr bool S = SEG && !TB::SPLIT;
    void (*kern)(GateFwdParams);
    if constexpr (sizeof...(ts) == 0) kern = p.gated ? gate_fwd_kernel<TB, true, S> : gate_fwd_kernel<TB, false, S>;
    else kern = p.gated ? gate_fwd_mixed_kernel<TB, decltype(ts)..., true, S> : gate_fwd_mixed_kernel<TB, decltype(ts)..., false, S>;
    return launch_tiled<TB>(TB::SPLIT ? "gate_fwd_split_kernel" : "gate_fwd_kernel", kern, p, pl.grid, st);
  };
  using TS = Tile<64, 128, 2, 2, true, true>;
  using SB = TileSp<128, 128, 2, 2>;
  using SS = TileSp<64, 128, 2, 2>;
  switch (pl.kind) {
    case GATE_64: return pl.split ? go(SS{}) : go(TS{});
    case GATE_128: return pl.split ? go(SB{}) : go(TileNT128{});
    case GATE_MIXED: return pl.split ? go(SB{}, SS{}) : go(TileNT128{}, TS{});
  }
  return MMF_ERR_ARG;
}

int launch_gate_fwd(GateFwdParams p, hipStream_t st) { return launch_gate_fwd_impl<false>(p, st); }
int launch_gate_fwd_seg(GateFwdParams p, hipStream_t st) {
  if (!p.seg_ridx || p.split) return MMF_ERR_ARG;
  return p.drop_p > 0.f ? launch_gate_fwd_impl<true>(p, st) : launch_gate_fwd_impl<false>(p, st);
}

int pool_groups(int64_t N) {
  static const int cap = tune_int("MMF_POOL_GROUPS", 256);
  int64_t g = (N + 63) / 64;
  if (g > cap) g = cap;
  if (g < 1) g = 1;
  while ((N + g - 1) / g > POOL_MAX_ROWS) g *= 2;
  return (int)g;
}

int launch_pool(PoolParams p, hipStream_t st) {
  if (p.H != 256 && p.H != 512 && p.H != 1024) return MMF_ERR_SHAPE;
  p.n_groups = pool_groups(p.N);
  p.rows_per_group = (int)((p.N + p.n_groups - 1) / p.n_groups);
  if (p.rows_per_group > POOL_MAX_ROWS) return MMF_ERR_SHAPE;
  { ProfScope ps("pool_partial_kernel", st); hipLaunchKernelGGL(pool_partial_kernel, dim3(p.n_groups), dim3(256), 0, st, p); }
  return launch_pool_merge(p, st);
}

int launch_pool_merge(PoolParams p, hipStream_t st) {
  if (p.n_groups < 1 || p.n_groups > MERGE_MAX_GROUPS || p.H > 1024 || p.H % 32 != 0) return MMF_ERR_SHAPE;
  if (p.tail.Wk && (p.tail.K < 1 || p.tail.K > 32)) return MMF_ERR_SHAPE;
  {
    ProfScope ps("pool_merge_kernel", st);
    hipLaunchKernelGGL(pool_merge_kernel, dim3(p.H / 32), dim3(1024), 0, st, p);
  }
  if (p.tail.Wk) {
    ProfScope ps("head_tail_kernel", st);
    hipLaunchKernelGGL(head_tail_kernel, dim3(1), dim3(1024), 0, st, p);
  }
  return hipGetLastError() == hipSuccess ? MMF_OK : MMF_ERR_LAUNCH;
}

int launch_head_tail(PoolParams p, hipStream_t st) {
  if (!p.M || !p.tail.Wk || p.H < 1 || p.H > 1024 || p.tail.K < 1 || p.tail.K > 32) return MMF_ERR_SHAPE;
  ProfScope ps("head_tail_kernel", st);
  hipLaunchKernelGGL(head_tail_kernel, dim3(1), dim3(1024), 0, st, p);
  return hipGetLastError() == hipSuccess ? MMF_OK : MMF_ERR_LAUNCH;
}

}

namespace mmf {

__global__ __launch_bounds__(256) void group_rows_kernel(GroupRowsParams p) {
  __shared__ int64_t off[GROUP_MAX + 1];
  const int G = p.s.G;
  for (int i = threadIdx.x; i <= G; i += 256) off[i] = p.s.off[i];
  __syncthreads();
  const int64_t row = (int64_t)blockIdx.x * 256 + threadIdx.x;
  if (row >= off[G]) return;
  int lo = 0, hi = G - 1;
  while (lo < hi) {
    const int mid = (lo + hi + 1) >> 1;
    if (off[mid] <= row) lo = mid; else hi = mid - 1;
  }
  const uint32_t local = (uint32_t)(row - off[lo]), base = p.s.ibase[lo];
  p.ridx_h[row] = local * (uint32_t)p.H + base;
  p.ridx_d[row] = local * (uint32_t)p.D + base;
  p.bag[row] = lo;
}

int launch_group_rows(const GroupRowsParams& p, hipStream_t st) {
  const int64_t R = p.s.off[p.s.G];
  ProfScope ps("group_rows_kernel", st);
  hipLaunchKernelGGL(group_rows_kernel, dim3((unsigned)((R + 255) / 256)), dim3(256), 0, st, p);
  return hipGetLastError() == hipSuccess ? MMF_OK : MMF_ERR_LAUNCH;
}

__global__ __launch_bounds__(256) void group_pool_partial_kernel(PoolParams p, SegTable s) {
  const int b = blockIdx.x;
  int g = 0;
  for (int i = 1; i < s.G; ++i)
    if (b >= s.gbeg[i]) g = i;
  const int64_t r0 = s.off[g] + (int64_t)(b - s.gbeg[g]) * s.rows_per_group;
  const int64_t r1 = r0 + s.rows_per_group < s.off[g + 1] ? r0 + s.rows_per_group : s.off[g + 1];
  pool_partial_rows(p, b, r0, r1);
}

constexpr int GROUP_BAG_MAX_PARTIALS = GROUP_POOL_GROUPS + 64;

__device__ __forceinline__ float bag_merge(const float* part, int n, int H, float* wl, float* red, float& m, float& l) {
  const int tid = threadIdx.x, lane = tid & 63, wave = tid >> 6;
  const int stride = 2 + H;
  m = -INFINITY;
  for (int i = tid; i < n; i += 1024) m = fmaxf(m, part[(size_t)i * stride]);
  m = wave_max(m);
  if (lane == 0) red[wave] = m;
  __syncthreads();
  m = red[0];
#pragma unroll
  for (int i = 1; i < 16; ++i) m = fmaxf(m, red[i]);
  l = 0.f;
  for (int i = tid; i < n; i += 1024) {
    const float mg = part[(size_t)i * stride];
    const float w = mg > -INFINITY ? __expf(mg - m) : 0.f;
    wl[i] = w;
    l += part[(size_t)i * stride + 1] * w;
  }
  l = wave_sum(l);
  if (lane == 0) red[16 + wave] = l;
  __syncthreads();
  l = 0.f;
#pragma unroll
  for (int i = 0; i < 16; ++i) l += red[16 + i];
  float mv = 0.f;
  if (tid < H) {
    const float* col = part + 2 + tid;
    float acc = 0.f;
    for (int sl = 0; sl < 32; ++sl) {
      float a = 0.f;
      for (int i = sl; i < n; i += 32) a += col[(size_t)i * stride] * wl[i];
      acc += a;
    }
    mv = acc / l;
  }
  return mv;
}

__device__ __forceinline__ PoolParams bag_slice(const PoolParams& p, int g, int ldm) {
  PoolParams q = p;
  const int H = p.H, K = p.tail.K;
  if (q.M) q.M += (size_t)g * ldm;
  if (q.stats) q.stats += 2 * g;
  HeadTail& t = q.tail;
  t.logits += (size_t)g * K; t.hazards += (size_t)g * K; t.S += (size_t)g * K; t.Y_hat += g;
  if (t.risk) t.risk += g;
  if (t.Y) t.Y += g;
  if (t.c) t.c += g;
  if (t.loss) t.loss += g;
  if (t.dM) t.dM += (size_t)g * H;
  if (t.dWk) t.dWk += (size_t)g * K * H;
  if (t.dbk) t.dbk += (size_t)g * K;
  t.accumulate = 0;
  return q;
}

__global__ __launch_bounds__(1024) void group_tail_kernel(PoolParams p, SegTable s) {
  __shared__ float tail_sm[1024 + 160];
  __shared__ float wl[GROUP_BAG_MAX_PARTIALS];
  __shared__ float red[32];
  const int g = blockIdx.x, tid = threadIdx.x;
  const int gb = s.gbeg[g], n = s.gbeg[g + 1] - gb, H = p.H;
  const PoolParams q = bag_slice(p, g, H);
  TailPre pre;
  tail_preload(q, pre);
  float m, l;
  const float mv = bag_merge(p.partials + (size_t)gb * (2 + H), n, H, wl, red, m, l);
  if (tid < H) {
    q.M[tid] = mv;
    tail_sm[tid] = mv;
  }
  if (tid == 0) { q.stats[0] = m; q.stats[1] = l; }
  head_tail<true>(q, pre, tail_sm);
}

int group_pool_check(const PoolParams& p, const SegTable& s) {
  if (p.H != 256 && p.H != 512 && p.H != 1024) return MMF_ERR_SHAPE;
  if (s.G < 1 || s.G > GROUP_MAX || s.rows_per_group < 1 || s.rows_per_group > POOL_MAX_ROWS) return MMF_ERR_SHAPE;
  for (int g = 0; g < s.G; ++g)
    if (s.gbeg[g + 1] - s.gbeg[g] > GROUP_BAG_MAX_PARTIALS) return MMF_ERR_SHAPE;
  return MMF_OK;
}

int launch_group_pool_partial(PoolParams p, const SegTable& s, hipStream_t st) {
  if (int e = group_pool_check(p, s)) return e;
  ProfScope ps("group_pool_partial_kernel", st);
  hipLaunchKernelGGL(group_pool_partial_kernel, dim3(s.gbeg[s.G]), dim3(256), 0, st, p, s);
  return hipGetLastError() == hipSuccess ? MMF_OK : MMF_ERR_LAUNCH;
}

int launch_group_pool(PoolParams p, const SegTable& s, hipStream_t st) {
// ... 249 lines not shown
```

### multimodalfusion_amd/csrc/mmf_api.hip

```cpp
#include <cmath>
#include <cstdio>
#include <cstdlib>
#include <cstring>
#include <map>
#include <mutex>
#include <new>
#include <string>
#include <unordered_set>
#include <vector>

#include "../../include/mmf_amil.h"
#include "mmf_common.h"
#include "mmf_gemm_core.h"
#include "mmf_kernels.h"
#include "mmf_small.h"
#include "mmf_mlp.h"
#include "mmf_bf16.h"

namespace mmf {

int set_dyn_lds(const void* kern, int bytes) {
  if (bytes <= 48 * 1024) return MMF_OK;
  static std::mutex mu;
  static std::unordered_set<const void*> done;
  std::lock_guard<std::mutex> lock(mu);
  if (done.count(kern)) return MMF_OK;
  if (hipFuncSetAttribute(kern, hipFuncAttributeMaxDynamicSharedMemorySize, bytes) != hipSuccess) return MMF_ERR_LAUNCH;
  done.insert(kern);
  return MMF_OK;
}

}

struct mmf_trace {
  struct Rec { const char* name; hipEvent_t a, b; };
  std::mutex mu;
  std::vector<Rec> recs;
  std::vector<hipEvent_t> pool;
  int cap = 0;
};

namespace mmf {

static thread_local mmf_trace* tls_trace = nullptr;
struct TraceScope {
  mmf_trace* prev;
  explicit TraceScope(mmf_trace* t) : prev(tls_trace) { tls_trace = t; }
  ~TraceScope() { tls_trace = prev; }
};

void prof_begin(const char* name, hipStream_t st) {
  mmf_trace* t = tls_trace;
  if (!t) return;
  std::lock_guard<std::mutex> lock(t->mu);
  if ((int)t->recs.size() >= t->cap) return;
  auto take = [&](hipEvent_t& e) {
    if (!t->pool.empty()) { e = t->pool.back(); t->pool.pop_back(); return true; }
    return hipEventCreate(&e) == hipSuccess;
  };
  mmf_trace::Rec r{name, nullptr, nullptr};
  if (!take(r.a)) return;
  if (!take(r.b)) { t->pool.push_back(r.a); return; }
  hipEventRecord(r.a, st);
  t->recs.push_back(r);
}
void prof_end(hipStream_t st) {
  mmf_trace* t = tls_trace;
  if (!t) return;
  std::lock_guard<std::mutex> lock(t->mu);
  if (!t->recs.empty()) hipEventRecord(t->recs.back().b, st);
}

static inline size_t align_up(size_t v, size_t a) { return (v + a - 1) / a * a; }
static inline bool aligned16(const void* p) { return (reinterpret_cast<uintptr_t>(p) & 15) == 0; }

struct Carver {
  uintptr_t base;
  size_t off = 0;
  explicit Carver(void* b = nullptr) : base(reinterpret_cast<uintptr_t>(b)) {}
  template <class T> T* take(size_t n) {
    T* r = reinterpret_cast<T*>(base + off);
    off += align_up(n * sizeof(T), 256);
    return r;
  }
};

struct ReduceList {
  ReduceParams p{};
  int err = MMF_OK;
  int add(const float* in, float* out, int len, int nsplit, size_t stride) {
    constexpr int cap = (int)(sizeof(p.seg) / sizeof(p.seg[0]));
    if (p.nseg == cap) return err = MMF_ERR_SHAPE;
    p.seg[p.nseg++] = ReduceSeg{in, out, len, nsplit, stride, 0, 0};
    return MMF_OK;
  }
  int launch(int accumulate, hipStream_t st) {
    if (err) return err;
    p.accumulate = accumulate;
    return launch_reduce(p, st);
  }
};

static int check_grads(const mmf_amil_desc* d, const mmf_amil_grads* g) {
  if (!g->dW1 || !g->db1 || !g->dWa || !g->dba || !g->dWc || !g->dbc) return MMF_ERR_ARG;
  if (d->gated && (!g->dWb || !g->dbb)) return MMF_ERR_ARG;
  return MMF_OK;
}
static bool grads_aligned(const mmf_amil_desc* d, const mmf_amil_grads* g) {
  return aligned16(g->dW1) && aligned16(g->dWa) && (!d->gated || aligned16(g->dWb)) && (!g->dx || aligned16(g->dx));
}

struct AmilWs {
  float *M_step, *dM_step;
  unsigned long long* relu_bits;
  float *h, *a, *b, *s_part, *partials, *stats, *p, *ds, *dbc_part, *du;
  float *slab_w1, *slab_wab, *cs_b1, *cs_bab, *cs_wc;
  float* kpart;
  int parts, groups, mstk;
  TnPlan tn;
  size_t bytes;
};

static AmilWs carve(Carver& c, int64_t N, int L, int H, int D, int gated, bool infer = false) {
  AmilWs w{};
  auto take = [&](size_t n) { return c.take<float>(n); };
  w.parts = gate_parts(D, gated);
  w.groups = pool_groups(N);
  w.mstk = gated ? 2 * D : D;
  const TnShape shapes[2] = {{H, L, 0}, {w.mstk, H, 1}};
  w.tn = plan_tn(N, 0, shapes, 2);
  const int splits = w.tn.splits;
  w.M_step = take(H);
  w.dM_step = take(H);
  w.h = take((size_t)N * H);
  w.s_part = take((size_t)w.parts * N);
  w.partials = take((size_t)w.groups * (2 + H));
  w.stats = take(4);
  {
    const size_t kf = linear_ksplit_floats(N, H, L, 1, L);
    w.kpart = kf ? take(kf) : nullptr;
  }
  if (infer) {
    w.bytes = c.off;
    return w;
  }
  w.relu_bits = c.take<unsigned long long>((size_t)((N + 15) / 16 + 2) * (H / 32) * 8);
  w.a = take((size_t)N * D);
  w.b = take(gated ? (size_t)N * D : 0);
  w.p = take((size_t)N);
  w.ds = take((size_t)N);
  w.dbc_part = take(PREP_GROUPS);
  w.du = take((size_t)N * H);
  w.slab_w1 = take((size_t)splits * H * L);
  w.slab_wab = take((size_t)w.tn.splits_g * w.mstk * H);
  w.cs_b1 = take((size_t)splits * H);
  w.cs_bab = take((size_t)w.tn.splits_g * w.mstk);
  w.cs_wc = take((size_t)w.tn.splits_g * D);
  w.bytes = c.off;
  return w;
}

static int check_desc(const mmf_amil_desc* d, int elem_bytes = 4) {
  if (!d || !d->W1 || !d->b1 || !d->Wa || !d->ba || !d->Wc || !d->bc) return MMF_ERR_ARG;
  if (d->gated && (!d->Wb || !d->bb)) return MMF_ERR_ARG;
  if (d->N < 1) return MMF_ERR_SHAPE;
  if (d->L % KC != 0 || d->H % KC != 0) return MMF_ERR_SHAPE;
  if (d->H != 256 && d->H != 512 && d->H != 1024) return MMF_ERR_SHAPE;
  if (d->D % 128 != 0) return MMF_ERR_SHAPE;
  if (d->N * (int64_t)(d->H > d->D ? d->H : d->D) >= (int64_t)1 << 32) return MMF_ERR_SHAPE;
  int64_t widest = d->L > 2 * d->D ? d->L : 2 * d->D;
  if (d->H > widest) widest = d->H;
  if (d->N * widest * elem_bytes >= (int64_t)1 << 31) return MMF_ERR_SHAPE;
  if (d->p_h < 0.f || d->p_h >= 1.f || d->p_att < 0.f || d->p_att >= 1.f) return MMF_ERR_ARG;
  if (d->gemm != MMF_GEMM_F32 && d->gemm != MMF_GEMM_BF16X3) return MMF_ERR_ARG;
  return MMF_OK;
}

static int check_operands(const mmf_amil_desc* d, const void* x, const void* workspace, const float* A_raw, bool bf16) {
  if (!x || !workspace || !A_raw) return MMF_ERR_ARG;
  if (!aligned16(x) || !aligned16(workspace)) return MMF_ERR_ALIGN;
  if (!bf16 && (!aligned16(d->W1) || !aligned16(d->Wa) || (d->gated && !aligned16(d->Wb)))) return MMF_ERR_ALIGN;
  return MMF_OK;
}


static GateFwdParams gate_fwd_params(const mmf_amil_desc* d, const float* h, float* a, float* b, float* s_part,
                                     uint32_t seed) {
  GateFwdParams gp{};
  gp.h = h; gp.Wa = d->Wa; gp.ba = d->ba; gp.Wb = d->Wb; gp.bb = d->bb; gp.Wc = d->Wc;
  gp.a = a; gp.b = b; gp.s_part = s_part;
  gp.N = d->N; gp.H = d->H; gp.D = d->D; gp.gated = d->gated;
  gp.drop_p = d->p_att; gp.key_a = drop_key(seed, 1); gp.key_b = drop_key(seed, 2); gp.seed_dev = d->seed_dev;
  return gp;
}

static GateBwdCtx gate_bwd_ctx(const mmf_amil_desc* d, const float* a, const float* b, const float* ds, uint32_t seed) {
  GateBwdCtx gc{};
  gc.a = a; gc.b = b; gc.ds = ds; gc.Wc = d->Wc; gc.D = d->D; gc.gated = d->gated;
  gc.drop_p = d->p_att; gc.key_a = drop_key(seed, 1); gc.key_b = drop_key(seed, 2); gc.seed_dev = d->seed_dev;
  return gc;
}

static TnProblem tn_gate_problem(const mmf_amil_desc* d, const float* B, float* out, float* cs_bab, float* cs_wc) {
  const int mstk = d->gated ? 2 * d->D : d->D;
  TnProblem q{};
  q.kind = TN_A_GATE; q.A = nullptr; q.lda = 0; q.M = mstk;
  q.B = B; q.ldb = d->H; q.Ncols = d->H;
  q.out = out; q.split_stride = (size_t)mstk * d->H; q.ldc = d->H;
  q.colsum = cs_bab; q.colsum_stride = mstk; q.colsum2 = cs_wc; q.colsum2_stride = d->D;
  return q;
}

static LinearParams stack_linear(const mmf_amil_desc* d, const AmilWs& w, const float* x, uint32_t seed) {
  LinearParams lp{};
  lp.x[0] = x; lp.nseg = 1; lp.kseg = d->L; lp.ldx = d->L;
  lp.w = d->W1; lp.bias = d->b1; lp.y = w.h;
  lp.M = d->N; lp.N = d->H; lp.K = d->L;
  lp.act = ACT_RELU; lp.drop_p = d->p_h; lp.drop_key = drop_key(seed, 0); lp.seed_dev = d->seed_dev;
  lp.relu_bits = w.relu_bits;
  lp.allow_half = 1; lp.concurrent = d->concurrent ? 1 : 0;
  lp.split = d->gemm == MMF_GEMM_BF16X3;
  lp.kpart = w.kpart; lp.ktick = d->sync; lp.ktick_words = d->sync ? d->sync_words : 0;
  return lp;
}

static GateFwdParams stack_gate_fwd(const mmf_amil_desc* d, const AmilWs& w, uint32_t seed) {
  GateFwdParams gp = gate_fwd_params(d, w.h, w.a, w.b, w.s_part, seed);
  gp.split = d->gemm == MMF_GEMM_BF16X3;
  return gp;
}

static PoolParams stack_pool(const mmf_amil_desc* d, const AmilWs& w, float* A_raw) {
  PoolParams pp{};
  pp.s_part = w.s_part; pp.n_parts = w.parts; pp.bc = d->bc; pp.h = w.h; pp.N = d->N; pp.H = d->H;
  pp.A_raw = A_raw;
  return pp;
}

static BwdPrepParams stack_prep(const mmf_amil_desc* d, const AmilWs& w, const float* A_raw, const float* stats,
                                const float* M, const float* dM, const float* gA) {
  BwdPrepParams bp{};
  bp.h = w.h; bp.A_raw = A_raw; bp.stats = stats; bp.dM = dM; bp.M = M; bp.gA = gA;
  bp.N = d->N; bp.H = d->H; bp.p = w.p; bp.ds = w.ds; bp.dbc_part = w.dbc_part;
  bp.n_groups = (int)((d->N + 3) / 4 < PREP_GROUPS ? (d->N + 3) / 4 : PREP_GROUPS);
  return bp;
}

static BwdDhParams stack_dh(const mmf_amil_desc* d, const AmilWs& w, const GateBwdCtx& gc, const float* dM) {
  BwdDhParams dp{};
  dp.g = gc; dp.Wa = d->Wa; dp.Wb = d->Wb; dp.p = w.p; dp.dM = dM; dp.h = w.h; dp.du = w.du;
  dp.relu_bits = w.relu_bits;
  dp.concurrent = d->concurrent ? 1 : 0;
  dp.split = d->gemm == MMF_GEMM_BF16X3;
  dp.N = d->N; dp.H = d->H; dp.scale_h = d->p_h > 0.f ? 1.0f / (1.0f - d->p_h) : 1.0f;
  return dp;
}

static DhPlan dh_plan(const BwdDhParams& p, bool can_fuse) {
  return plan_bwd_dh(p.N, p.H, p.g.D, p.g.gated, p.g.drop_p > 0.f, p.split, p.concurrent, can_fuse, PREP_GROUPS);
}

static NnParams stack_dx(const mmf_amil_desc* d, const AmilWs& w, float* dx) {
  NnParams np{};
  np.A = w.du; np.lda = d->H; np.B = d->W1; np.ldb = d->L; np.C = dx; np.ldc = d->L;
  np.M = d->N; np.N = d->L; np.K = d->H;
  return np;
}

static TnPlan stack_tn(const mmf_amil_desc* d, const AmilWs& w, const float* x, const GateBwdCtx& gc, TnParams& tp) {
  tp.nprob = 2; tp.K = d->N; tp.g = gc;
  tp.split = d->gemm == MMF_GEMM_BF16X3;
  TnProblem& q1 = tp.prob[0];
  q1.kind = TN_A_PLAIN; q1.A = w.du; q1.lda = d->H; q1.M = d->H;
  q1.B = x; q1.ldb = d->L; q1.Ncols = d->L;
  q1.out = w.slab_w1; q1.split_stride = (size_t)d->H * d->L; q1.ldc = d->L;
  q1.colsum = w.cs_b1; q1.colsum_stride = d->H; q1.colsum2 = nullptr; q1.colsum2_stride = 0;
  tp.prob[1] = tn_gate_problem(d, w.h, w.slab_wab, w.cs_bab, w.cs_wc);
  TnPlan pl = w.tn;
  if (tp.split) pl.kind = plan_tn(d->N, 1, nullptr, 0).kind;
  return pl;
}

template <class W>
static void reduce_slabs(const mmf_amil_desc* d, const W& w, const mmf_amil_grads* g, int splits, int splits_g, ReduceList& rl) {
  const size_t wab_stride = (size_t)w.mstk * d->H;
  rl.add(w.slab_w1, g->dW1, d->H * d->L, splits, (size_t)d->H * d->L);
  rl.add(w.slab_wab, g->dWa, d->D * d->H, splits_g, wab_stride);
  if (d->gated) rl.add(w.slab_wab + (size_t)d->D * d->H, g->dWb, d->D * d->H, splits_g, wab_stride);
  rl.add(w.cs_b1, g->db1, d->H, splits, d->H);
  rl.add(w.cs_bab, g->dba, d->D, splits_g, w.mstk);
  if (d->gated) rl.add(w.cs_bab + d->D, g->dbb, d->D, splits_g, w.mstk);
}

static void stack_reduce(const mmf_amil_desc* d, const AmilWs& w, const mmf_amil_grads* g, int dbc_parts, ReduceList& rl) {
  reduce_slabs(d, w, g, w.tn.splits, w.tn.splits_g, rl);
  rl.add(w.cs_wc, g->dWc, d->D, w.tn.splits_g, d->D);
  rl.add(w.dbc_part, g->dbc, 1, dbc_parts, 1);
}

struct AmilWsBf {
  float *M_step, *dM_step;
  bf16_t *w1, *wab, *wabT, *h, *a, *b, *du, *dP;
  float *s_part, *partials, *stats, *p, *ds, *dbc_part, *dwc_part;
  float *slab_w1, *slab_wab, *cs_b1, *cs_bab;
  int parts, groups, splits, k_per_split, mstk, dbc_cap;
  size_t bytes;
};

static AmilWsBf carve_bf16(Carver& c, int64_t N, int L, int H, int D, int gated, bool infer = false) {
  AmilWsBf w{};
  auto take16 = [&](size_t n) { return c.take<bf16_t>(n); };
  auto take32 = [&](size_t n) { return c.take<float>(n); };
  w.parts = gate_parts_bf16(D, gated);
  w.groups = pool_groups(N);
  w.mstk = gated ? 2 * D : D;
  const int td = TNB_TILE;
  const int tiles = ((H + td - 1) / td) * ((L + td - 1) / td) + ((w.mstk + td - 1) / td) * ((H + td - 1) / td);
  w.splits = tn_bf16_splits(N, tiles);
  const int64_t kps = (N + w.splits - 1) / w.splits;
  w.k_per_split = (int)((kps + TNB_KCH - 1) / TNB_KCH * TNB_KCH);
  w.dbc_cap = dh_bf16_row_tiles(N);
  w.M_step = take32(H);
  w.dM_step = take32(H);
  w.w1 = take16((size_t)H * L);
  w.wab = take16((size_t)w.mstk * H);
  w.wabT = take16((size_t)H * w.mstk);
  w.h = take16((size_t)N * H);
  w.s_part = take32((size_t)w.parts * N);
  {
    const int tiles = fused_fwd_tiles(N);
    w.partials = take32((size_t)(w.groups > tiles ? w.groups : tiles) * (2 + H));
  }
  w.stats = take32(4);
  if (infer) {
    w.bytes = c.off;
    return w;
  }
  w.a = take16((size_t)N * D);
  w.b = take16(gated ? (size_t)N * D : 0);
  w.du = take16((size_t)N * H);
  w.dP = take16((size_t)N * w.mstk);
  w.p = take32((size_t)N);
  w.ds = take32((size_t)N);
  w.dbc_part = take32((size_t)w.dbc_cap);
  w.dwc_part = take32((size_t)w.dbc_cap * D);
  w.slab_w1 = take32((size_t)w.splits * H * L);
  w.slab_wab = take32((size_t)w.splits * w.mstk * H);
  w.cs_b1 = take32((size_t)w.splits * H);
  w.cs_bab = take32((size_t)w.splits * w.mstk);
  w.bytes = c.off;
  return w;
}

static int check_desc_bf16(const mmf_amil_desc* d) {
  if (int e = check_desc(d, 2)) return e;
  if (d->L % 64 != 0 || d->H % 256 != 0) return MMF_ERR_SHAPE;
  return MMF_OK;
}

static CvtParams stack_cvt_bf16(const mmf_amil_desc* d, const AmilWsBf& w, bool fused2, bool bwd) {
  CvtParams cp{};
  auto cvt = [&](const float* src, bf16_t* dst, int rows, int cols, int dst_ld, int c0, int transpose) {
    cp.seg[cp.nseg++] = CvtSeg{src, dst, rows, cols, dst_ld, c0, transpose, 0};
  };
  const bool dh2 = bwd && dh2_bf16_ok(d->N, d->H, d->D, d->gated);
  cvt(d->W1, w.w1, d->H, d->L, d->L, 0, fused2 ? 3 : 0);
  cvt(d->Wa, w.wab, d->D, d->H, d->H, 0, fused2 ? 4 : 0);
  if (bwd) cvt(d->Wa, w.wabT, d->D, d->H, w.mstk, 0, dh2 ? 5 : (d->gated ? 2 : 1));
  if (d->gated) {
    if (fused2) cvt(d->Wb, w.wab, d->D, d->H, d->H, 16, 4);
    else cvt(d->Wb, w.wab + (size_t)d->D * d->H, d->D, d->H, d->H, 0, 0);
    if (bwd) cvt(d->Wb, w.wabT, d->D, d->H, w.mstk, 32, dh2 ? 5 : 2);
  }
  return cp;
}

static LinearBfParams stack_linear_bf16(const mmf_amil_desc* d, const AmilWsBf& w, const uint16_t* x, uint32_t seed) {
  LinearBfParams lp{};
  lp.x = x; lp.w = w.w1; lp.bias = d->b1; lp.y = w.h;
  lp.M = d->N; lp.N = d->H; lp.K = d->L;
  lp.drop_p = d->p_h; lp.drop_key = drop_key(seed, 0); lp.seed_dev = d->seed_dev;
  return lp;
}

static GateBfParams stack_gate_bf16(const mmf_amil_desc* d, const AmilWsBf& w, uint32_t seed) {
  GateBfParams gp{};
  gp.h = w.h; gp.Wa = w.wab; gp.Wb = d->gated ? w.wab + (size_t)d->D * d->H : nullptr;
  gp.ba = d->ba; gp.bb = d->bb; gp.Wc = d->Wc;
  gp.a = w.a; gp.b = w.b; gp.s_part = w.s_part;
  gp.N = d->N; gp.H = d->H; gp.D = d->D; gp.gated = d->gated;
  gp.drop_p = d->p_att; gp.key_a = drop_key(seed, 1); gp.key_b = drop_key(seed, 2); gp.seed_dev = d->seed_dev;
  return gp;
}

static PoolBfParams stack_pool_bf16(const mmf_amil_desc* d, const AmilWsBf& w, float* A_raw) {
  PoolBfParams pb{};
  PoolParams& pp = pb.base;
  pp.s_part = w.s_part; pp.n_parts = w.parts; pp.bc = d->bc; pp.h = nullptr; pp.N = d->N; pp.H = d->H;
  pp.A_raw = A_raw;
  pb.h = w.h;
  return pb;
}

}

using namespace mmf;

extern "C" {

int mmf_abi_version(void) { return 12; }

const char* mmf_strerror(int code) {
  switch (code) {
    case MMF_OK: return "ok";
    case MMF_ERR_ARG: return "invalid argument (null pointer or bad flag)";
    case MMF_ERR_SHAPE: return "unsupported shape (need L,H % 32 == 0, H in {256,512,1024}, D % 128 == 0, K % 32 == 0, N % 4 == 0 of a dense layer, every operand < 2 GiB)";
    case MMF_ERR_ALIGN: return "pointer or leading dimension not 16-byte aligned";
    case MMF_ERR_WORKSPACE: return "workspace too small (see mmf_*_workspace_bytes)";
    case MMF_ERR_LAUNCH: return "HIP launch failed";
    default: return "unknown mmf error";
  }
}

size_t mmf_amil_workspace_bytes(int64_t N, int32_t L, int32_t H, int32_t D, int32_t gated) {
  if (N < 1) N = 1;
  Carver c;
  return carve(c, N, L, H, D, gated).bytes;
}

static int amil_forward_impl(const mmf_amil_desc* d, const float* x, void* workspace, size_t workspace_bytes,
                             float* M, float* A_raw, void* stream, bool infer, const HeadTail* tail = nullptr) {
  if (int e = check_desc(d)) return e;
  if (int e = check_operands(d, x, workspace, A_raw, false)) return e;
  Carver c(workspace);
  AmilWs w = carve(c, d->N, d->L, d->H, d->D, d->gated, infer);
  if (w.bytes > workspace_bytes) return MMF_ERR_WORKSPACE;
  if (!M) M = w.M_step;
  hipStream_t st = static_cast<hipStream_t>(stream);
  TraceScope ts(d->trace);

  if (int e = launch_linear(stack_linear(d, w, x, d->seed), st)) return e;
  if (int e = launch_gate_fwd(stack_gate_fwd(d, w, d->seed), st)) return e;
  PoolParams pp = stack_pool(d, w, A_raw);
  pp.partials = w.partials; pp.M = M; pp.stats = w.stats;
  if (tail) { pp.tail = *tail; pp.tail.dM = w.dM_step; }
  return launch_pool(pp, st);
}

int mmf_amil_forward(const mmf_amil_desc* d, const float* x, void* workspace, size_t workspace_bytes,
                     float* M, float* A_raw, void* stream) {
  return amil_forward_impl(d, x, workspace, workspace_bytes, M, A_raw, stream, false);
}

size_t mmf_amil_infer_workspace_bytes(int64_t N, int32_t L, int32_t H, int32_t D, int32_t gated) {
  if (N < 1) N = 1;
  Carver c;
  return carve(c, N, L, H, D, gated, true).bytes;
}

int mmf_amil_infer(const mmf_amil_desc* d, const float* x, void* workspace, size_t workspace_bytes,
                   float* M, float* A_raw, void* stream) {
  return amil_forward_impl(d, x, workspace, workspace_bytes, M, A_raw, stream, true);
}

static int amil_backward_impl(const mmf_amil_desc* d, const float* x, void* workspace, size_t workspace_bytes,
                              const float* M, const float* A_raw, const float* dM, const float* gA,
                              const mmf_amil_grads* g, void* stream, int accumulate) {
  if (int e = check_desc(d)) return e;
  if (!x || !workspace || !A_raw || !g) return MMF_ERR_ARG;
  if (int e = check_grads(d, g)) return e;
  if (!grads_aligned(d, g)) return MMF_ERR_ALIGN;
  Carver c(workspace);
  AmilWs w = carve(c, d->N, d->L, d->H, d->D, d->gated);
  if (w.bytes > workspace_bytes) return MMF_ERR_WORKSPACE;
  if (!M) M = w.M_step;
  if (!dM) dM = w.dM_step;
  hipStream_t st = static_cast<hipStream_t>(stream);
  TraceScope ts(d->trace);

  const GateBwdCtx gc = gate_bwd_ctx(d, w.a, w.b, w.ds, d->seed);
  BwdDhParams dp = stack_dh(d, w, gc, dM);
  const DhPlan pl = dh_plan(dp, true);
  int dbc_groups = pl.dbc_groups;
  if (pl.fused) {
    dp.A_raw = A_raw; dp.stats = w.stats; dp.Mpool = M; dp.gA = gA;
    dp.p_out = w.p; dp.ds_out = w.ds; dp.dbc_part = w.dbc_part;
  } else {
    const BwdPrepParams bp = stack_prep(d, w, A_raw, w.stats, M, dM, gA);
    dbc_groups = bp.n_groups;
    if (int e = launch_bwd_prep(bp, st)) return e;
  }
  if (int e = launch_bwd_dh(pl, dp, st)) return e;
  if (g->dx) {
    if (int e = launch_nn(stack_dx(d, w, g->dx), st)) return e;
  }

  TnParams tp{};
  const TnPlan tn = stack_tn(d, w, x, gc, tp);
  if (int e = launch_tn(tn, tp, st)) return e;

  ReduceList rl;
  stack_reduce(d, w, g, dbc_groups, rl);
  return rl.launch(accumulate, st);
}

int mmf_amil_backward(const mmf_amil_desc* d, const float* x, void* workspace, size_t workspace_bytes,
                      const float* M, const float* A_raw, const float* dM, const float* gA,
                      const mmf_amil_grads* g, void* stream) {
  if (!M || !dM) return MMF_ERR_ARG;
  return amil_backward_impl(d, x, workspace, workspace_bytes, M, A_raw, dM, gA, g, stream, 0);
}

size_t mmf_amil_bf16_workspace_bytes(int64_t N, int32_t L, int32_t H, int32_t D, int32_t gated) {
  if (N < 1) N = 1;
  Carver c;
  return carve_bf16(c, N, L, H, D, gated).bytes;
}

static int amil_bf16_forward_impl(const mmf_amil_desc* d, const uint16_t* x, void* workspace, size_t workspace_bytes,
                                  float* M, float* A_raw, void* stream, bool infer, const HeadTail* tail = nullptr) {
  if (int e = check_desc_bf16(d)) return e;
  if (int e = check_operands(d, x, workspace, A_raw, true)) return e;
  Carver c(workspace);
  AmilWsBf w = carve_bf16(c, d->N, d->L, d->H, d->D, d->gated, infer);
  if (w.bytes > workspace_bytes) return MMF_ERR_WORKSPACE;
  if (!M) M = w.M_step;
  hipStream_t st = static_cast<hipStream_t>(stream);
  TraceScope ts(d->trace);
  HeadTail tl{};
  if (tail) { tl = *tail; tl.dM = w.dM_step; }

  const bool fused2 = d->gated && fused_fwd2_ok(d->N, d->L, d->H, d->D);
  if (int e = launch_cvt_bf16(stack_cvt_bf16(d, w, fused2, !infer), st)) return e;

  if (fused2 || (d->gated && d->D == 256 && fused_fwd_ok(d->N, d->L, d->H, d->D))) {
    FusedFwdParams fp{};
    fp.x = x; fp.w1 = w.w1; fp.b1 = d->b1;
    fp.Wa = w.wab; fp.Wb = d->gated ? w.wab + (size_t)d->D * d->H : nullptr;
    fp.w1f = w.w1; fp.wabf = w.wab;
    fp.ba = d->ba; fp.bb = d->bb; fp.Wc = d->Wc; fp.bc = d->bc;
    fp.h = infer ? nullptr : w.h; fp.a = w.a; fp.b = w.b;
    fp.A_raw = A_raw; fp.partials = w.partials;
    fp.N = d->N; fp.L = d->L; fp.D = d->D;
    fp.p_h = d->p_h; fp.p_att = d->p_att;
    fp.key_h = drop_key(d->seed, 0); fp.key_a = drop_key(d->seed, 1); fp.key_b = drop_key(d->seed, 2);
    fp.seed_dev = d->seed_dev;
    if (fused2) {
      if (int e = launch_fused_fwd2_bf16(fp, d->gated, st)) return e;
    } else
    if (int e = launch_fused_fwd_bf16(fp, d->gated, st)) return e;
    PoolParams pm{};
    pm.N = d->N; pm.H = d->H; pm.partials = w.partials; pm.M = M; pm.stats = w.stats;
    pm.n_groups = fused_fwd_tiles(d->N);
    pm.tail = tl;
    return launch_pool_merge(pm, st);
  }

  if (int e = launch_linear_bf16(stack_linear_bf16(d, w, x, d->seed), st)) return e;
  if (int e = launch_gate_bf16(stack_gate_bf16(d, w, d->seed), st)) return e;
  PoolBfParams pb = stack_pool_bf16(d, w, A_raw);
  pb.base.partials = w.partials; pb.base.M = M; pb.base.stats = w.stats; pb.base.tail = tl;
  return launch_pool_bf16(pb, st);
}

int mmf_amil_bf16_forward(const mmf_amil_desc* d, const uint16_t* x, void* workspace, size_t workspace_bytes,
                          float* M, float* A_raw, void* stream) {
  return amil_bf16_forward_impl(d, x, workspace, workspace_bytes, M, A_raw, stream, false);
}

size_t mmf_amil_bf16_infer_workspace_bytes(int64_t N, int32_t L, int32_t H, int32_t D, int32_t gated) {
  if (N < 1) N = 1;
  Carver c;
  return carve_bf16(c, N, L, H, D, gated, true).bytes;
}

int mmf_amil_bf16_infer(const mmf_amil_desc* d, const uint16_t* x, void* workspace, size_t workspace_bytes,
                        float* M, float* A_raw, void* stream) {
  return amil_bf16_forward_impl(d, x, workspace, workspace_bytes, M, A_raw, stream, true);
}

static int amil_bf16_backward_impl(const mmf_amil_desc* d, const uint16_t* x, void* workspace, size_t workspace_bytes,
                                   const float* M, const float* A_raw, const float* dM, const float* gA,
                                   const mmf_amil_grads* g, void* stream, int accumulate) {
  if (int e = check_desc_bf16(d)) return e;
  if (!x || !workspace || !A_raw || !g) return MMF_ERR_ARG;
  if (int e = check_grads(d, g)) return e;
  if (g->dx) return MMF_ERR_ARG;
  if (!grads_aligned(d, g)) return MMF_ERR_ALIGN;
  Carver c(workspace);
  AmilWsBf w = carve_bf16(c, d->N, d->L, d->H, d->D, d->gated);
  if (w.bytes > workspace_bytes) return MMF_ERR_WORKSPACE;
  if (!M) M = w.M_step;
  if (!dM) dM = w.dM_step;
  hipStream_t st = static_cast<hipStream_t>(stream);
  TraceScope ts(d->trace);
  const uint32_t* const seed_dev = d->seed_dev;

  GateBwdBf gc{};
  gc.a = w.a; gc.b = w.b; gc.ds = w.ds; gc.Wc = d->Wc; gc.D = d->D; gc.gated = d->gated;
  gc.drop_p = d->p_att; gc.key_a = drop_key(d->seed, 1); gc.key_b = drop_key(d->seed, 2); gc.seed_dev = seed_dev;

  DhBfParams dp{};
  dp.g = gc; dp.WabT = w.wabT; dp.dM = dM; dp.h = w.h; dp.du = w.du;
  dp.N = d->N; dp.H = d->H; dp.scale_h = d->p_h > 0.f ? 1.0f / (1.0f - d->p_h) : 1.0f;
  dp.A_raw = A_raw; dp.stats = w.stats; dp.Mpool = M; dp.gA = gA;
  dp.p_out = w.p; dp.ds_out = w.ds; dp.dbc_part = w.dbc_part; dp.dP = w.dP; dp.dwc_part = w.dwc_part;
  if (dh2_bf16_ok(d->N, d->H, d->D, d->gated)) {
    if (int e = launch_dh2_bf16(dp, st)) return e;
  } else if (int e = launch_dh_bf16(dp, st)) return e;
  const int ntn = d->H / 256;

  TnBfParams tp{};
  tp.nprob = 2; tp.K = d->N; tp.splits = w.splits; tp.k_per_split = w.k_per_split;
  TnBfProblem& q1 = tp.prob[0];
  q1.A = w.du; q1.lda = d->H; q1.M = d->H;
  q1.B = x; q1.ldb = d->L; q1.Ncols = d->L;
  q1.out = w.slab_w1; q1.split_stride = (size_t)d->H * d->L; q1.ldc = d->L;
  q1.colsum = w.cs_b1; q1.colsum_stride = d->H;
  TnBfProblem& q2 = tp.prob[1];
  q2.A = w.dP; q2.lda = w.mstk; q2.M = w.mstk;
  q2.B = w.h; q2.ldb = d->H; q2.Ncols = d->H;
  q2.out = w.slab_wab; q2.split_stride = (size_t)w.mstk * d->H; q2.ldc = d->H;
  q2.colsum = w.cs_bab; q2.colsum_stride = w.mstk;
  if (int e = launch_tn_bf16(tp, st)) return e;

  ReduceList rl;
  reduce_slabs(d, w, g, w.splits, w.splits, rl);
  rl.add(w.dwc_part, g->dWc, d->D, dh_bf16_tiles_used(d->N, ntn), d->D);
  rl.add(w.dbc_part, g->dbc, 1, dh_bf16_tiles_used(d->N, ntn), 1);
  return rl.launch(accumulate, st);
}

int mmf_amil_bf16_backward(const mmf_amil_desc* d, const uint16_t* x, void* workspace, size_t workspace_bytes,
                           const float* M, const float* A_raw, const float* dM, const float* gA,
                           const mmf_amil_grads* g, void* stream) {
  if (!M || !dM) return MMF_ERR_ARG;
  return amil_bf16_backward_impl(d, x, workspace, workspace_bytes, M, A_raw, dM, gA, g, stream, 0);
}

static int head_tail_of(const mmf_surv_head* h, const mmf_nll_target* t, HeadTail& tl, bool grads = true) {
  if (!h || !h->Wk || !h->bk || !h->logits || !h->hazards || !h->S || !h->Y_hat) return MMF_ERR_ARG;
  if (h->K < 1 || h->K > 32) return MMF_ERR_SHAPE;
  tl = HeadTail{};
  tl.Wk = h->Wk; tl.bk = h->bk; tl.K = h->K;
  tl.logits = h->logits; tl.hazards = h->hazards; tl.S = h->S; tl.Y_hat = h->Y_hat; tl.risk = h->risk;
  if (t) {
    if (!t->Y || !t->c || !t->loss || (grads && (!t->dWk || !t->dbk))) return MMF_ERR_ARG;
    tl.Y = t->Y; tl.c = t->c; tl.alpha = t->alpha; tl.eps = t->eps; tl.loss = t->loss;
    if (grads) { tl.loss_scale = t->loss_scale; tl.dWk = t->dWk; tl.dbk = t->dbk; tl.accumulate = t->accumulate; }
  }
  return MMF_OK;
}

int mmf_amil_head_forward(const mmf_amil_desc* d, const void* x, int32_t x_bf16, void* workspace, size_t workspace_bytes,
                          const mmf_surv_head* head, float* M, float* A_raw, void* stream) {
  if (!d || !M) return MMF_ERR_ARG;
  HeadTail tl;
  if (int e = head_tail_of(head, nullptr, tl)) return e;
  return x_bf16 ? amil_bf16_forward_impl(d, static_cast<const uint16_t*>(x), workspace, workspace_bytes, M, A_raw, stream, false, &tl)
                : amil_forward_impl(d, static_cast<const float*>(x), workspace, workspace_bytes, M, A_raw, stream, false, &tl);
}

int mmf_amil_nll_step(const mmf_amil_desc* d, const void* x, int32_t x_bf16, void* workspace, size_t workspace_bytes,
                      const mmf_surv_head* head, const mmf_nll_target* target, float* A_raw,
                      const mmf_amil_grads* grads, void* stream) {
  if (!d || !target || !grads) return MMF_ERR_ARG;
  HeadTail tl;
  if (int e = head_tail_of(head, target, tl)) return e;
  const int acc = target->accumulate ? 1 : 0;
  if (x_bf16) {
    const uint16_t* xb = static_cast<const uint16_t*>(x);
    if (int e = amil_bf16_forward_impl(d, xb, workspace, workspace_bytes, nullptr, A_raw, stream, false, &tl)) return e;
    return amil_bf16_backward_impl(d, xb, workspace, workspace_bytes, nullptr, A_raw, nullptr, nullptr, grads, stream, acc);
  }
  const float* xf = static_cast<const float*>(x);
  if (int e = amil_forward_impl(d, xf, workspace, workspace_bytes, nullptr, A_raw, stream, false, &tl)) return e;
  return amil_backward_impl(d, xf, workspace, workspace_bytes, nullptr, A_raw, nullptr, nullptr, grads, stream, acc);
}

namespace mmf {
static uint32_t hash_mul_inverse() {
  const uint32_t a = 0x9E3779B1u;
  uint32_t x = a;
  for (int i = 0; i < 5; ++i) x *= 2u - a * x;
  return x;
}

static int group_plan(const int64_t* offsets, int G, SegTable& s) {
  if (!offsets) return MMF_ERR_ARG;
  if (G < 1 || G > GROUP_MAX) return MMF_ERR_SHAPE;
  if (offsets[0] != 0) return MMF_ERR_SHAPE;
  for (int g = 0; g < G; ++g)
    if (offsets[g + 1] <= offsets[g]) return MMF_ERR_SHAPE;
  s = SegTable{};
  s.G = G;
  const int64_t R = offsets[G];
  int64_t rpg = (R + GROUP_POOL_GROUPS - 1) / GROUP_POOL_GROUPS;
  if (rpg < 64) rpg = 64;
  if (rpg > 8192) return MMF_ERR_SHAPE;
  s.rows_per_group = (int)rpg;
  int gb = 0;
  for (int g = 0; g <= G; ++g) {
    s.off[g] = offsets[g];
    s.gbeg[g] = gb;
    if (g < G) gb += (int)((offsets[g + 1] - offsets[g] + rpg - 1) / rpg);
  }
  return MMF_OK;
}

struct WindowWs {
  AmilWs w;
  float *M, *dM, *stats, *partials;
  uint32_t *ridx_h, *ridx_d;
  int* bag;
};
struct GroupWs : WindowWs {
  float *wk, *bk;
  size_t bytes;
};
static GroupWs carve_group(Carver& c, const SegTable& s, int L, int H, int D, int gated) {
  GroupWs g{};
  const int64_t R = s.off[s.G];
  g.w = carve(c, R, L, H, D, gated);
  auto take = [&](size_t n) { return c.take<float>(n); };
  g.M = take((size_t)s.G * H);
  g.dM = take((size_t)s.G * H);
  g.stats = take((size_t)2 * s.G);
  g.wk = take((size_t)s.G * 32 * H);
  g.bk = take((size_t)s.G * 32);
  g.partials = take((size_t)s.gbeg[s.G] * (2 + H));
  g.ridx_h = c.take<uint32_t>((size_t)R);
  g.ridx_d = c.take<uint32_t>((size_t)R);
  g.bag = c.take<int>((size_t)R);
  g.bytes = c.off;
  return g;
}
}

namespace mmf {
struct GroupExtra {
  float* dx;
  TnProblem prob[4]; int nprob;
  TnPlan tn;
};

static int window_plan(const mmf_amil_desc* d, const mmf_bag_group* group, int bf16, SegTable& s) {
  if (int e = group_plan(group->offsets, group->G, s)) return e;
  if (d->N != s.off[s.G]) return MMF_ERR_SHAPE;
  return bf16 ? check_desc_bf16(d) : check_desc(d);
}

static int group_check(const mmf_amil_desc* d, const mmf_bag_group* group, const void* x, const void* workspace,
                       const mmf_surv_head* head, const mmf_nll_target* target, const float* A_raw,
                       const mmf_amil_grads* g, SegTable& s, HeadTail& tl) {
  if (!d || !group || !target || !g) return MMF_ERR_ARG;
  if (d->gemm != MMF_GEMM_F32 || g->dx) return MMF_ERR_ARG;
  if (!group->seeds) return MMF_ERR_ARG;
  if (int e = window_plan(d, group, 0, s)) return e;
  if (int e = head_tail_of(head, target, tl)) return e;
  if (int e = check_grads(d, g)) return e;
  if (int e = check_operands(d, x, workspace, A_raw, false)) return e;
  if (!grads_aligned(d, g)) return MMF_ERR_ALIGN;
  const uint32_t inv = hash_mul_inverse();
  for (int b = 0; b < s.G; ++b) s.ibase[b] = group->seeds[b] * inv;
  return MMF_OK;
}

static int window_rows(const mmf_amil_desc* d, const SegTable& s, const WindowWs& g, hipStream_t st) {
  GroupRowsParams rp{};
  rp.s = s; rp.H = d->H; rp.D = d->D; rp.ridx_h = g.ridx_h; rp.ridx_d = g.ridx_d; rp.bag = g.bag;
  return launch_group_rows(rp, st);
}
static int window_pool(const mmf_amil_desc* d, const SegTable& s, const WindowWs& g, float* M, int ldm, float* A_raw,
                       hipStream_t st) {
  PoolParams pp = stack_pool(d, g.w, A_raw);
  pp.partials = g.partials; pp.M = M; pp.stats = g.stats;
  if (int e = launch_group_pool_partial(pp, s, st)) return e;
  return launch_group_merge(pp, s, ldm, g.M, st);
}
static int window_dh(const mmf_amil_desc* d, const WindowWs& g, const GateBwdCtx& gc, const float* dM, const float* A_raw,
                     int& dbc_parts, hipStream_t st) {
  const BwdPrepParams bp = stack_prep(d, g.w, A_raw, g.stats, g.M, dM, nullptr);
  dbc_parts = bp.n_groups;
  if (int e = launch_group_bwd_prep(bp, g.bag, st)) return e;
  BwdDhParams dp = stack_dh(d, g.w, gc, dM);
  dp.seg_ridx = g.ridx_d; dp.seg_bag = g.bag;
  return launch_bwd_dh_seg(dh_plan(dp, false), dp, st);
}

static int group_chain_fwd(const mmf_amil_desc* d, const SegTable& s, const float* x, const GroupWs& gw, hipStream_t st) {
  const AmilWs& w = gw.w;
  if (int e = window_rows(d, s, gw, st)) return e;

  LinearParams lp = stack_linear(d, w, x, 0);
  lp.seg_ridx = gw.ridx_h;
  if (int e = launch_linear_seg(lp, st)) return e;

  GateFwdParams gp = stack_gate_fwd(d, w, 0);
  gp.seg_ridx = gw.ridx_d;
  return launch_gate_fwd_seg(gp, st);
}

static int group_chain_bwd(const mmf_amil_desc* d, const float* x, const GroupWs& gw, const float* dM, const float* A_raw,
                           const mmf_amil_grads* g, const GroupExtra* ex, ReduceList& rl, hipStream_t st) {
  const AmilWs& w = gw.w;
  const GateBwdCtx gc = gate_bwd_ctx(d, w.a, w.b, w.ds, 0);
  int dbc_parts;
  if (int e = window_dh(d, gw, gc, dM, A_raw, dbc_parts, st)) return e;

  if (ex && ex->dx) {
    if (int e = launch_nn(stack_dx(d, w, ex->dx), st)) return e;
  }

  TnParams tp{};
  const TnPlan tn = stack_tn(d, w, x, gc, tp);
  tp.seg_ridx = gw.ridx_d;
  if (int e = launch_tn(tn, tp, st)) return e;
  if (ex) {
    TnParams tr{};
    for (int i = 0; i < ex->nprob; ++i) tr.prob[i] = ex->prob[i];
    tr.nprob = ex->nprob; tr.K = d->N;
    if (int e = launch_tn(ex->tn, tr, st)) return e;
  }

  stack_reduce(d, w, g, dbc_parts, rl);
  return MMF_OK;
}

static int group_chain(const mmf_amil_desc* d, const SegTable& s, const float* x, const GroupWs& gw, const HeadTail& tl,
                       int K, const mmf_nll_target* target, float* A_raw, const mmf_amil_grads* g,
// ... 1378 lines not shown
```

### multimodalfusion_amd/csrc/mmf_kernels.h

```cpp
#pragma once
#include <hip/hip_runtime.h>
#include <stdint.h>
#include <type_traits>

#include "mmf_common.h"

namespace mmf {

enum : int { ACT_NONE = 0, ACT_RELU = 1, ACT_TANH = 2, ACT_SIGMOID = 3, ACT_SELU = 4 };

struct LinearParams {
  const float* x[4];
  int nseg, kseg, ldx;
  const float* w;
  const float* bias;
  float* y;
  int64_t M;
  int N, K;
  int act;
  float drop_p;
  uint32_t drop_key;
  const uint32_t* seed_dev;
  int mt_count, nt_count;
  unsigned long long* relu_bits;
  int allow_half;
  int concurrent;
  int deep;
  int split;
  int ksplit;
  float* kpart;
  unsigned* ktick;
  int ktick_words;
  const uint32_t* seg_ridx;
};
enum : int { LIN_SPLIT_WIDE, LIN_WIDE, LIN_128, LIN_SPLIT_64, LIN_KSPLIT_64, LIN_64 };
struct LinearPlan {
  int kind;
  int rows;
  int ksplit;
  int deep;
  int mt_count, nt_count, grid;
  int kpart_floats;
};
LinearPlan plan_linear(int64_t M, int N, int K, int nseg, int kseg, int allow_half, int concurrent, int split, int tick_words);
size_t linear_ksplit_floats(int64_t M, int N, int K, int nseg, int kseg);

struct GateFwdParams {
  const float* h;
  const float *Wa, *ba, *Wb, *bb, *Wc;
  float *a, *b;
  float* s_part;
  int64_t N;
  int H, D, gated;
  float drop_p;
  uint32_t key_a, key_b;
  const uint32_t* seed_dev;
  int mt_count, nt_count;
  int64_t row_begin, row_end;
  struct Region { int64_t row0; int mt_count, grid_begin, tall; } reg[5];
  int nreg;
  int deep;
  int split;
  const uint32_t* seg_ridx;
};

struct HeadTail {
  const float *Wk, *bk;
  int K;
  float *logits, *hazards, *S;
  int64_t* Y_hat;
  float* risk;
  const int64_t* Y; const float* c;
  float alpha, eps, loss_scale;
  float *loss;
  float *dM;
  float *dWk, *dbk;
  int accumulate;
};

struct PoolParams {
  const float* s_part;
  int n_parts;
  const float* bc;
  const float* h;
  int64_t N;
  int H;
  float* A_raw;
  float* partials;
  float* M;
  float* stats;
  int n_groups, rows_per_group;
  HeadTail tail;
};
constexpr int POOL_MAX_ROWS = 8192;

struct BwdPrepParams {
  const float* h;
  const float* A_raw;
  const float* stats;
  const float* dM;
  const float* M;
  const float* gA;
  int64_t N;
  int H;
  float* p;
  float* ds;
  float* dbc_part;
  int n_groups;
};

struct GateBwdCtx {
  const float *a, *b, *ds, *Wc;
  int D, gated;
  float drop_p;
  uint32_t key_a, key_b;
  const uint32_t* seed_dev;
  __device__ inline void resolve_seed() {
    if (seed_dev) { const uint32_t sd = *seed_dev; key_a += sd; key_b += sd; seed_dev = nullptr; }
  }
};

template <bool GATED, bool DROP, int PART>
__device__ inline float gate_dp_t(const GateBwdCtx& g, float av, float bv, float wc, float dsv,
                                  uint32_t idx, uint32_t thr, float dscale, float& a_d_b_d) {
  float ma = 1.f, mb = 1.f;
  if constexpr (DROP) {
    ma = keep(g.key_a, idx, thr) ? dscale : 0.f;
    if constexpr (GATED) mb = keep(g.key_b, idx, thr) ? dscale : 0.f;
  }
  if constexpr (GATED) {
    a_d_b_d = (av * ma) * (bv * mb);
    return PART == 0 ? dsv * wc * (bv * mb) * ma * (1.f - av * av)
                     : dsv * wc * (av * ma) * mb * bv * (1.f - bv);
  }
  a_d_b_d = av * ma;
  return dsv * wc * ma * (1.f - av * av);
}
__device__ inline float gate_dp(const GateBwdCtx& g, int part, float av, float bv, float wc, float dsv,
                                uint32_t idx, uint32_t thr, float dscale, float& a_d_b_d) {
  float ma = 1.f, mb = 1.f;
  if (g.drop_p > 0.f) {
    ma = keep(g.key_a, idx, thr) ? dscale : 0.f;
    if (g.gated) mb = keep(g.key_b, idx, thr) ? dscale : 0.f;
  }
  if (g.gated) {
    a_d_b_d = (av * ma) * (bv * mb);
    return part == 0 ? dsv * wc * (bv * mb) * ma * (1.f - av * av)
                     : dsv * wc * (av * ma) * mb * bv * (1.f - bv);
  }
  a_d_b_d = av * ma;
  return dsv * wc * ma * (1.f - av * av);
}

struct BwdDhParams {
  GateBwdCtx g;
  const float *Wa, *Wb;
  const float* p;
  const float* dM;
  const float* h;
  const unsigned long long* relu_bits;
  float* du;
  int64_t N;
  int H;
  float scale_h;
  int mt_count, nt_count;
  int deep;
  int allow_half;
  int concurrent;
  int split;
  int fused_prep;
  const float *A_raw, *stats, *Mpool, *gA;
  float *p_out, *ds_out, *dbc_part;
  const uint32_t* seg_ridx;
  const int* seg_bag;
};

enum : int { TN_A_PLAIN = 0, TN_A_GATE = 1 };

struct TnProblem {
  int kind;
  const float* A; int lda; int M;
  const float* B; int ldb; int Ncols;
  float* out; size_t split_stride; int ldc;
  float* colsum; size_t colsum_stride;
  float* colsum2; size_t colsum2_stride;
  int tiles_m, tiles_n, block_begin;
  int tile_begin;
  int splits, k_per_split;
};

struct TnParams {
  TnProblem prob[6];
  int nprob;
  int64_t K;
  int splits, k_per_split;
  int total_tiles;
  int xcd_map;
  int tile;
  int split;
  GateBwdCtx g;
  uint16_t map[512];
  const uint32_t* seg_ridx;
};

struct NnParams {
  const float* A; int lda;
  const float* B; int ldb;
  float* C; int ldc;
  int64_t M;
  int N, K;
  int mt_count, nt_count;
  const float* mulx; int ldx;
  float *rs_part, *ra_part;
  const float* segx[4]; int kseg;
};

struct ReduceSeg { const float* in; float* out; int len; int nsplit; size_t stride; int block_begin; int tall; };
struct ReduceParams { ReduceSeg seg[12]; int nseg; int accumulate; };

int launch_linear(LinearParams p, hipStream_t st);
int launch_linear_seg(LinearParams p, hipStream_t st);
enum : int { GATE_64, GATE_128, GATE_MIXED };
struct GatePlan {
  int kind;
  int split;
  int deep;
  int mt_count, nt_count, grid;
  int nreg;
  struct Region { int row0, mt_count, grid_begin, tall; } reg[5];
};
GatePlan plan_gate_fwd(int64_t N, int H, int D, int gated, int split);
int gate_parts(int D, int gated);
int launch_gate_fwd(GateFwdParams p, hipStream_t st);
int launch_gate_fwd_seg(GateFwdParams p, hipStream_t st);
int pool_groups(int64_t N);
int launch_pool(PoolParams p, hipStream_t st);
int launch_score_sum(const float* s_part, int n_parts, const float* bc, float* A, int64_t N, hipStream_t st);
int launch_head_tail(PoolParams p, hipStream_t st);
int launch_pool_merge(PoolParams p, hipStream_t st);
int launch_bwd_prep(BwdPrepParams p, hipStream_t st);

constexpr int PREP_GROUPS = 512;
enum : int { DH_SPLIT_WIDE, DH_SPLIT_64, DH_WIDE, DH_128, DH_64X128, DH_64 };
struct DhPlan {
  int kind;
  int rows;
  int fused;
  int variant;
  int deep;
  int mt_count, nt_count, grid;
  int extra_lds;
  int dbc_groups;
};
DhPlan plan_bwd_dh(int64_t N, int H, int D, int gated, int dropout, int split, int concurrent, int can_fuse, int dbc_cap);
int launch_bwd_dh(const DhPlan& pl, BwdDhParams p, hipStream_t st);
int launch_bwd_dh_seg(const DhPlan& pl, BwdDhParams p, hipStream_t st);
int split_min_rows();
enum : int { TN_128, TN_256, TN_SPLIT_128, TN_SPLIT_256 };
struct TnShape { int M, Ncols, gate; };
struct TnPlan {
  int kind, tile;
  int splits, k_per_split;
  int splits_g, k_per_split_g;
  int tiles;
};
TnPlan plan_tn(int64_t K, int split, const TnShape* shapes, int nshape);
int launch_tn(const TnPlan& pl, TnParams p, hipStream_t st);
int pick_wide_rows(int64_t M, int ntn, bool allow_half, bool concurrent, int max_rows);
bool use_wide_tiles(int64_t M, int N, int split = 0);
bool short_grid(int64_t workgroups);
int launch_nn(NnParams p, hipStream_t st);
int launch_reduce(ReduceParams p, hipStream_t st);

constexpr int GROUP_MAX = 64;
constexpr int GROUP_POOL_GROUPS = 256;
struct SegTable {
  int G;
  int rows_per_group;
  int64_t off[GROUP_MAX + 1];
  int gbeg[GROUP_MAX + 1];
  uint32_t ibase[GROUP_MAX];
};
struct GroupRowsParams { SegTable s; int H, D; uint32_t *ridx_h, *ridx_d; int* bag; };
int launch_group_rows(const GroupRowsParams& p, hipStream_t st);
int launch_group_pool(PoolParams p, const SegTable& s, hipStream_t st);
int launch_group_bwd_prep(BwdPrepParams p, const int* bag, hipStream_t st);
int group_pool_check(const PoolParams& p, const SegTable& s);
int launch_group_pool_partial(PoolParams p, const SegTable& s, hipStream_t st);
int launch_group_infer_tail(PoolParams p, const SegTable& s, hipStream_t st);
int launch_group_merge(PoolParams p, const SegTable& s, int ldm, float* Mw, hipStream_t st);
int launch_group_dm_gather(const float* src, int ld, float* dst, int G, int H, hipStream_t st);
int launch_surv_head_group(PoolParams p, int ldf, int G, hipStream_t st);
struct HeadSegs { const float* x[3]; int width[3]; int n; };
int launch_surv_head_infer_group(PoolParams p, const HeadSegs& s, int G, hipStream_t st);

struct IgSteps { int S; float alpha[GROUP_MAX]; float w[GROUP_MAX]; };
struct IgExpandParams {
  const float* U;
  const float* b1;
  float* h;
  unsigned long long* relu_bits;
  int64_t N;
  int H;
  IgSteps st;
};
int launch_ig_expand(const IgExpandParams& p, hipStream_t st);
struct IgHeadParams {
  const float* M;
  const float *Wk, *bk;
  int K, H;
  float* dM;
  int step0, n_steps;
  float *step_risk, *risk_x, *risk_base;
  float *logits, *hazards, *S, *risk;
  int64_t* Y_hat;
};
int launch_ig_head(const IgHeadParams& p, int S, hipStream_t st);
struct IgFoldParams { const float* du; float* G; int64_t N; int H; int first; IgSteps st; };
int launch_ig_fold(const IgFoldParams& p, hipStream_t st);
int launch_nn_attr(NnParams p, float* row_sum, float* row_abs, hipStream_t st);
int launch_ig_bias(const float* W1, const float* br, const float* b1, float* out, int H, int L, hipStream_t st);
int launch_nn_attr_seg(NnParams p, float* row_sum, float* row_abs, hipStream_t st);

int set_dyn_lds(const void* kern, int bytes);

void prof_begin(const char* name, hipStream_t st);
void prof_end(hipStream_t st);
struct ProfScope {
  hipStream_t st;
  ProfScope(const char* name, hipStream_t s) : st(s) { prof_begin(name, s); }
  ~ProfScope() { prof_end(st); }
};

template <int MAX, int R = 64, class F>
int with_wide_rows(int rows, F&& f) {
  if constexpr (R <= MAX) return rows == R ? f(std::integral_constant<int, R>{}) : with_wide_rows<MAX, R + 16>(rows, f);
  else return MMF_ERR_ARG;
}

template <class T, class P>
int launch_tiled(const char* name, void (*kern)(P), const P& p, int grid, hipStream_t st, int extra_bytes = 0) {
  const int bytes = T::LDS_BYTES + extra_bytes;
  if (int e = set_dyn_lds(reinterpret_cast<const void*>(kern), bytes)) return e;
  ProfScope ps(name, st);
  hipLaunchKernelGGL(kern, dim3(grid), dim3(T::NT), bytes, st, p);
  return hipGetLastError() == hipSuccess ? MMF_OK : MMF_ERR_LAUNCH;
}

}
```

Measured before the change: 1382 bags/s.

## Route AMIL head through per-row classifier projections q = h·Wk instead of pooling h

The forward linear epilogue now projects each hidden row onto the K classifier weights (q = h·Wk), so pooling and the head logits need only K-wide per-row sums instead of the full H-wide attention pool over h. In backward, the per-row gradient dot product h·dM becomes a K-wide dz·q, which removes a full read of h in the bwd prep or fused K-prep. The pooled M is rebuilt after dh with a separate pool_m pass, and dWk is produced by a scaled reduce. This adds epilogue work, shuffles and LDS traffic to the first GEMM, plus an extra pool_m pass over h. It changes fp32 summation order.

```diff
diff --git a/multimodalfusion_amd/csrc/mmf_amil_bwd.hip b/multimodalfusion_amd/csrc/mmf_amil_bwd.hip
--- a/multimodalfusion_amd/csrc/mmf_amil_bwd.hip
+++ b/multimodalfusion_amd/csrc/mmf_amil_bwd.hip
@@ -11,6 +11,30 @@
 __global__ __launch_bounds__(256) void bwd_prep_kernel(BwdPrepParams p) {
   __shared__ float red[4];
   const int tid = threadIdx.x, lane = tid & 63, wave = tid >> 6;
+  if (p.q_part) {
+    const float m = p.qstats[QSTAT_M], inv = 1.0f / p.qstats[QSTAT_L], dmm = p.qstats[QSTAT_DMM];
+    float dz[Q_STRIDE];
+#pragma unroll
+    for (int k = 0; k < Q_STRIDE; ++k) dz[k] = p.qstats[QSTAT_DZ + k];
+    float dbc = 0.f;
+    for (int64_t i = (int64_t)blockIdx.x * 256 + tid; i < p.N; i += (int64_t)gridDim.x * 256) {
+      float q[Q_STRIDE];
+      q_row(p.q_part, p.q_parts, p.N, i, p.Kq, q);
+      float g = 0.f;
+#pragma unroll
+      for (int k = 0; k < Q_STRIDE; ++k) g += dz[k] * q[k];
+      const float pi = __expf(p.A_raw[i] - m) * inv;
+      const float d = pi * (g - dmm) + (p.gA ? p.gA[i] : 0.f);
+      p.p[i] = pi;
+      p.ds[i] = d;
+      dbc += d;
+    }
+    dbc = wave_sum(dbc);
+    if (lane == 0) red[wave] = dbc;
+    __syncthreads();
+    if (tid == 0) p.dbc_part[blockIdx.x] = red[0] + red[1] + red[2] + red[3];
+    return;
+  }
   const float m = p.stats[0], inv = 1.0f / p.stats[1];
   float dmm = 0.f;
   for (int c = lane; c < p.H; c += 64) dmm += p.dM[c] * p.M[c];
@@ -476,17 +500,29 @@
     float* g_l = p_l + T::BM + 16;
     const int LPR = p.H / 4;
     const int PPL = LPR / 64;
-    float4 dm_l[4];
-#pragma unroll
-    for (int q = 0; q < 4; ++q) dm_l[q] = q < PPL ? ld4(p.dM + 4 * (lane + 64 * q)) : zero4();
-    float dmm = 0.f;
-    for (int c = lane; c < p.H; c += 64) dmm += p.dM[c] * p.Mpool[c];
-    const float smax = p.stats[0], inv = 1.0f / p.stats[1];
     static_assert(T::BM <= T::NT, "one row per thread in K-prep");
     const int prow = row0 + tid;
     const bool pok = tid < T::BM && prow < p.N;
+    bool qmode = false;
+    if constexpr (!T::SPLIT) qmode = p.q_part != nullptr;
+    float dmm = 0.f, smax = 0.f, inv = 0.f, g_q = 0.f;
+    if (qmode) {
+      smax = p.qstats[QSTAT_M]; inv = 1.0f / p.qstats[QSTAT_L]; dmm = p.qstats[QSTAT_DMM];
+      if (pok) {
+        float q[Q_STRIDE];
+        q_row(p.q_part, p.q_parts, p.N, prow, p.Kq, q);
+#pragma unroll
+        for (int k = 0; k < Q_STRIDE; ++k) g_q += p.qstats[QSTAT_DZ + k] * q[k];
+      }
+    }
     const float araw = pok ? p.A_raw[prow] : 0.f;
     const float gav = (pok && p.gA) ? p.gA[prow] : 0.f;
+    if (!qmode) {
+    float4 dm_l[4];
+#pragma unroll
+    for (int q = 0; q < 4; ++q) dm_l[q] = q < PPL ? ld4(p.dM + 4 * (lane + 64 * q)) : zero4();
+    for (int c = lane; c < p.H; c += 64) dmm += p.dM[c] * p.Mpool[c];
+    smax = p.stats[0]; inv = 1.0f / p.stats[1];
     const int wr0 = wave * RPW, wr1 = wr0 + RPW < T::BM ? wr0 + RPW : T::BM;
     auto g_rows = [&](auto nrows_c, int rb) {
       constexpr int NR = decltype(nrows_c)::value;
@@ -520,12 +556,13 @@
     }
     dmm = wave_sum(dmm);
     __syncthreads();
+    }
     float dbc = 0.f;
     if (tid < T::BM) {
       float pi = 0.f, d = 0.f;
       if (pok) {
         pi = __expf(araw - smax) * inv;
-        d = pi * (g_l[tid] - dmm) + gav;
+        d = pi * ((qmode ? g_q : g_l[tid]) - dmm) + gav;
         if (nt == 0) { p.p_out[prow] = pi; p.ds_out[prow] = d; }
       }
       ds_l[tid] = d;
@@ -1224,7 +1261,14 @@
 #pragma unroll
       for (int g = 0; g < 16; ++g) t += part[g][threadIdx.x];
       const int c = (b - s.block_begin) * 64 + threadIdx.x;
-      if (c < s.len) s.out[c] = (p.accumulate ? s.out[c] : 0.f) + t;
+      if (c < s.len) {
+        if (s.scale) {
+          for (int k = 0; k < s.nscale; ++k) {
+            float* o = s.out + (size_t)k * s.len + c;
+            *o = (p.accumulate ? *o : 0.f) + s.scale[k] * t;
+          }
+        } else s.out[c] = (p.accumulate ? s.out[c] : 0.f) + t;
+      }
     }
     return;
   }
@@ -1245,6 +1289,16 @@
       float4 v = ld4(in + (size_t)k * s.stride);
       acc.x += v.x; acc.y += v.y; acc.z += v.z; acc.w += v.w;
     }
+    if (s.scale) {
+      for (int k = 0; k < s.nscale; ++k) {
+        float* o = s.out + (size_t)k * s.len + j;
+        const float w = s.scale[k];
+        float4 r = make_float4(w * acc.x, w * acc.y, w * acc.z, w * acc.w);
+        if (p.accumulate) { r.x += o[0]; r.y += o[1]; r.z += o[2]; r.w += o[3]; }
+        o[0] = r.x; o[1] = r.y; o[2] = r.z; o[3] = r.w;
+      }
+      return;
+    }
     if (p.accumulate) { const float4 o = ld4(s.out + j); acc.x += o.x; acc.y += o.y; acc.z += o.z; acc.w += o.w; }
     st4(s.out + j, acc);
   } else {
@@ -1258,6 +1312,7 @@
 
 int launch_bwd_prep(BwdPrepParams p, hipStream_t st) {
   if (p.H % 4 != 0 || p.H > 1024) return MMF_ERR_SHAPE;
+  if (p.q_part && (!p.qstats || p.q_parts < 1 || p.Kq < 1 || p.Kq > Q_STRIDE)) return MMF_ERR_ARG;
   { ProfScope ps("bwd_prep_kernel", st); hipLaunchKernelGGL(bwd_prep_kernel, dim3(p.n_groups), dim3(256), 0, st, p); }
   return hipGetLastError() == hipSuccess ? MMF_OK : MMF_ERR_LAUNCH;
 }
@@ -1342,6 +1397,7 @@
 static int launch_dh_plan(const DhPlan& pl, BwdDhParams p, hipStream_t st) {
   if (p.g.D % KC != 0 || p.H % 4 != 0) return MMF_ERR_SHAPE;
   if (SEG && (pl.fused || p.split || !p.seg_bag || !p.seg_ridx || !p.dM || !p.p || !p.h)) return MMF_ERR_ARG;
+  if (p.q_part && (SEG || !pl.fused || !p.qstats || p.q_parts < 1 || p.Kq < 1 || p.Kq > Q_STRIDE)) return MMF_ERR_ARG;
   if (p.N <= 0) return MMF_OK;
   p.mt_count = pl.mt_count; p.nt_count = pl.nt_count; p.deep = pl.deep; p.fused_prep = pl.fused;
   return with_dh_tile(pl, [&](auto tile) -> int {
@@ -1592,6 +1648,7 @@
   int blocks = 0;
   for (int i = 0; i < p.nseg; ++i) {
     ReduceSeg& s = p.seg[i];
+    if (s.scale && (s.len < 4 || (s.len & 3) != 0 || (s.stride & 3) != 0 || s.nscale < 1)) return MMF_ERR_SHAPE;
     s.tall = s.nsplit >= 64 && s.len >= 4 && (s.len & 3) == 0 && (s.stride & 3) == 0;
     s.block_begin = blocks;
     blocks += s.tall ? (s.len + 63) / 64 : (s.len + 1023) / 1024;
diff --git a/multimodalfusion_amd/csrc/mmf_amil_fwd.hip b/multimodalfusion_amd/csrc/mmf_amil_fwd.hip
--- a/multimodalfusion_amd/csrc/mmf_amil_fwd.hip
+++ b/multimodalfusion_amd/csrc/mmf_amil_fwd.hip
@@ -26,7 +26,7 @@
   int S;
 };
 
-template <class T, int ACT, bool DROP, bool SEG = false>
+template <class T, int ACT, bool DROP, bool SEG = false, int QK = 0>
 __device__ inline void linear_epilogue(const LinearParams& p, f32x16 (&acc)[T::MB][T::NB], f32x4acc (*acch)[2], float* lds,
                                        int row0, int col0, const PartSrc ps = PartSrc{}) {
   const uint32_t thr = drop_threshold(p.drop_p);
@@ -38,6 +38,42 @@
     const int col = col0 + epilogue_col<T>(nb);
     bias4[nb] = (p.bias && col < p.N) ? ld4(p.bias + col) : zero4();
   }
+  constexpr int QN = QK > 0 ? QK : 1;
+  constexpr int QSTRIPS = T::BN / 32;
+  float* qred = lds + (T::NT / 64) * (32 * EPI_STRIDE) + 4;
+  static_assert(QK == 0 || ((T::NT / 64) * 32 * EPI_STRIDE + 4 + QSTRIPS * T::BM * QK) * 4 <= T::LDS_BYTES, "q partials fit the tile's LDS");
+  static_assert(QK == 0 || T::BM <= T::NT, "one row per thread in the q sum");
+  float4 wk4[T::NB][QN];
+  if constexpr (QK > 0) {
+#pragma unroll
+    for (int nb = 0; nb < T::NB; ++nb) {
+      const int col = col0 + epilogue_col<T>(nb);
+#pragma unroll
+      for (int k = 0; k < QK; ++k) wk4[nb][k] = (k < p.Kq && col < p.N) ? ld4(p.wk + (size_t)k * p.N + col) : zero4();
+    }
+  }
+  auto q_finish = [&]() {
+    if constexpr (QK > 0) {
+      __syncthreads();
+      const int i = threadIdx.x;
+      if (i < T::BM && row0 + i < p.M) {
+        float* out = p.q_part + ((size_t)(col0 / T::BN) * (size_t)p.M + (size_t)(row0 + i)) * Q_STRIDE;
+#pragma unroll
+        for (int k4 = 0; k4 < QK / 4; ++k4) {
+          float4 s = ld4(qred + i * QK + 4 * k4);
+#pragma unroll
+          for (int w = 1; w < QSTRIPS; ++w) {
+            const float4 v = ld4(qred + (w * T::BM + i) * QK + 4 * k4);
+            s.x += v.x; s.y += v.y; s.z += v.z; s.w += v.w;
+          }
+          const float sv[4] = {s.x, s.y, s.z, s.w};
+#pragma unroll
+          for (int e = 0; e < 4; ++e)
+            if (4 * k4 + e < p.Kq) out[4 * k4 + e] = sv[e];
+        }
+      }
+    }
+  };
   const int lane = threadIdx.x & 63;
   auto rows_op = [&](auto nt_c, int nb, int r, int c, const float4* v) {
     constexpr int NTR = decltype(nt_c)::value;
@@ -45,6 +81,7 @@
     const bool col_ok = col < p.N;
     const float4 b4 = bias4[nb];
     unsigned long long mine = 0ull;
+    float qacc[NTR * QN];
 #pragma unroll
     for (int t = 0; t < NTR; ++t) {
       const int row = row0 + r + 8 * t;
@@ -67,6 +104,29 @@
         }
       }
       if (ok) st4(p.y + (size_t)row * p.N + col, make_float4(y[0], y[1], y[2], y[3]));
+      if constexpr (QK > 0) {
+#pragma unroll
+        for (int k = 0; k < QK; ++k) {
+          const float4 w4 = wk4[nb][k];
+          qacc[t * QK + k] = y[0] * w4.x + y[1] * w4.y + y[2] * w4.z + y[3] * w4.w;
+        }
+      }
+    }
+    if constexpr (QK > 0) {
+      constexpr int V = NTR * QK;
+      const int c4l = lane & 7;
+      const bool b2 = c4l & 4, b1 = c4l & 2, b0 = c4l & 1;
+      float w1[V / 2], w2[V / 4], w3[V / 8];
+#pragma unroll
+      for (int i = 0; i < V / 2; ++i) w1[i] = (b2 ? qacc[V / 2 + i] : qacc[i]) + __shfl_xor(b2 ? qacc[i] : qacc[V / 2 + i], 4, 64);
+#pragma unroll
+      for (int i = 0; i < V / 4; ++i) w2[i] = (b1 ? w1[V / 4 + i] : w1[i]) + __shfl_xor(b1 ? w1[i] : w1[V / 4 + i], 2, 64);
+#pragma unroll
+      for (int i = 0; i < V / 8; ++i) w3[i] = (b0 ? w2[V / 8 + i] : w2[i]) + __shfl_xor(b0 ? w2[i] : w2[V / 8 + i], 1, 64);
+      const int j0 = (b2 ? V / 2 : 0) + (b1 ? V / 4 : 0) + (b0 ? V / 8 : 0);
+      float* o = qred + ((c >> 5) * T::BM + r + 8 * (j0 / QK)) * QK + j0 % QK;
+#pragma unroll
+      for (int i = 0; i < V / 8; ++i) o[i] = w3[i];
     }
     if (p.relu_bits && lane < 4 * NTR) {
       const size_t rb16 = ((size_t)(row0 + r - (lane >> 3)) >> 4) + (lane >> 3), cb = (size_t)(col0 + c - 4 * (lane & 7)) >> 5;
@@ -110,6 +170,7 @@
                 buf[(NBLK + nb) & 1]);
       }
     }
+    q_finish();
     return;
   }
   epilogue_rows<T>(acc, lds, [&](int mb, int nb, int r, int c, const float4 (&v)[4]) {
@@ -126,6 +187,7 @@
               (wn * T::NB + nb) * 32 + 4 * (lane & 7), v);
     }
   }
+  q_finish();
 }
 
 template <class T>
@@ -166,8 +228,8 @@
   return flag[0] == (unsigned)(S - 1);
 }
 
-template <class T, bool SEG = false>
-__global__ __launch_bounds__(T::NT) void linear_nt_kernel(LinearParams p) {
+template <class T, bool SEG, bool Q>
+__device__ __forceinline__ void linear_nt_body(const LinearParams& p) {
   extern __shared__ __align__(16) float lds[];
   const int S = p.ksplit > 1 ? p.ksplit : 1;
   int mt, ntk;
@@ -197,6 +259,16 @@
   const bool drop = p.drop_p > 0.f;
   if constexpr (SEG) {
     linear_epilogue<T, ACT_RELU, true, true>(p, acc, acch, lds, row0, col0, ps);
+    return;
+  }
+  if constexpr (Q) {
+    if (p.Kq > 4) {
+      if (drop) linear_epilogue<T, ACT_RELU, true, false, 8>(p, acc, acch, lds, row0, col0, ps);
+      else linear_epilogue<T, ACT_RELU, false, false, 8>(p, acc, acch, lds, row0, col0, ps);
+    } else {
+      if (drop) linear_epilogue<T, ACT_RELU, true, false, 4>(p, acc, acch, lds, row0, col0, ps);
+      else linear_epilogue<T, ACT_RELU, false, false, 4>(p, acc, acch, lds, row0, col0, ps);
+    }
     return;
   }
   if (p.act == ACT_RELU) {
@@ -210,6 +282,11 @@
     linear_epilogue<T, -1, false>(p, acc, acch, lds, row0, col0, ps);
   }
 }
+
+template <class T, bool SEG = false>
+__global__ __launch_bounds__(T::NT) void linear_nt_kernel(LinearParams p) { linear_nt_body<T, SEG, false>(p); }
+template <class T>
+__global__ __launch_bounds__(T::NT) void linear_nt_q_kernel(LinearParams p) { linear_nt_body<T, false, true>(p); }
 
 template <class T>
 __global__ __launch_bounds__(T::NT) void linear_nt_split_kernel(LinearParams p) {
@@ -494,6 +571,8 @@
   r.c = (tid == 0 && t.c) ? t.c[0] : 0.f;
   r.y = (tid == 0 && t.Y) ? (long long)t.Y[0] : 0;
 }
+template <bool BWD> __device__ inline void head_from_z(const HeadTail& t, const TailPre& r, float* z);
+template <bool DWK> __device__ inline void head_grads(const PoolParams& p, const TailPre& r, const float* Ml, const float* z);
 template <bool M_IN_LDS, bool BWD = true>
 __device__ inline void head_tail(const PoolParams& p, const TailPre& r, float* sm ) {
   const HeadTail& t = p.tail;
@@ -501,7 +580,6 @@
   const int H = p.H, K = t.K;
   float* Ml = sm;
   float* z = sm + 1024;
-  float *hz = z + 32, *S = z + 64, *gH = z + 96, *gS = z + 128;
   if constexpr (!M_IN_LDS)
     for (int c = tid; c < H; c += 1024) Ml[c] = p.M[c];
   __syncthreads();
@@ -520,6 +598,16 @@
     if (lane == 0) z[k] = acc + t.bk[k];
   }
   __syncthreads();
+  head_from_z<BWD>(t, r, z);
+  if (!BWD || !t.Y) return;
+  __syncthreads();
+  head_grads<true>(p, r, Ml, z);
+}
+
+template <bool BWD>
+__device__ inline void head_from_z(const HeadTail& t, const TailPre& r, float* z) {
+  const int tid = threadIdx.x, K = t.K;
+  float *hz = z + 32, *S = z + 64, *gH = z + 96, *gS = z + 128;
   if (tid == 0) {
     float run = 1.f, best = -INFINITY, ssum = 0.f;
     int arg = 0;
@@ -570,8 +658,12 @@
         }
     }
   }
-  if (!BWD || !t.Y) return;
-  __syncthreads();
+}
+
+template <bool DWK>
+__device__ inline void head_grads(const PoolParams& p, const TailPre& r, const float* Ml, const float* z) {
+  const HeadTail& t = p.tail;
+  const int tid = threadIdx.x, H = p.H, K = t.K;
   for (int c = tid; c < H; c += 1024) {
     float acc = 0.f;
     if (c == tid) {
@@ -583,11 +675,12 @@
       for (int k = 0; k < K; ++k) acc += z[k] * t.Wk[(size_t)k * H + c];
     }
     t.dM[c] = acc;
-    for (int k = 0; k < K; ++k) {
-      float* o = t.dWk + (size_t)k * H + c;
-      const float v = z[k] * Ml[c];
-      *o = t.accumulate ? *o + v : v;
-    }
+    if constexpr (DWK)
+      for (int k = 0; k < K; ++k) {
+        float* o = t.dWk + (size_t)k * H + c;
+        const float v = z[k] * Ml[c];
+        *o = t.accumulate ? *o + v : v;
+      }
   }
   if (tid < K) t.dbk[tid] = t.accumulate ? t.dbk[tid] + z[tid] : z[tid];
 }
@@ -646,6 +739,134 @@
   TailPre pre;
   tail_preload(p, pre);
   head_tail<false>(p, pre, tail_sm);
+}
+
+__global__ __launch_bounds__(256) void pool_q_partial_kernel(PoolParams p) {
+  __shared__ float s_lds[POOL_MAX_ROWS];
+  __shared__ float red[4];
+  __shared__ float kred[4][2 + Q_STRIDE];
+  const int tid = threadIdx.x, lane = tid & 63, wave = tid >> 6;
+  const int g = blockIdx.x, K = p.tail.K;
+  const int64_t r0 = (int64_t)g * p.rows_per_group;
+  const int64_t r1 = r0 + p.rows_per_group < p.N ? r0 + p.rows_per_group : p.N;
+  const int nrows = r1 > r0 ? (int)(r1 - r0) : 0;
+  const float bc = p.bc ? p.bc[0] : 0.f;
+  float lmax = -INFINITY;
+  for (int i = tid; i < nrows; i += 256) {
+    float s = bc;
+    for (int t = 0; t < p.n_parts; ++t) s += p.s_part[(size_t)t * p.N + r0 + i];
+    p.A_raw[r0 + i] = s;
+    s_lds[i] = s;
+    lmax = fmaxf(lmax, s);
+  }
+  lmax = wave_max(lmax);
+  if (lane == 0) red[wave] = lmax;
+  __syncthreads();
+  const float m = fmaxf(fmaxf(red[0], red[1]), fmaxf(red[2], red[3]));
+  float acc[1 + Q_STRIDE];
+#pragma unroll
+  for (int k = 0; k <= Q_STRIDE; ++k) acc[k] = 0.f;
+  for (int i = tid; i < nrows; i += 256) {
+    const float e = __expf(s_lds[i] - m);
+    float q[Q_STRIDE];
+    q_row(p.q_part, p.q_parts, p.N, r0 + i, K, q);
+    acc[0] += e;
+#pragma unroll
+    for (int k = 0; k < Q_STRIDE; ++k) acc[1 + k] += e * q[k];
+  }
+#pragma unroll
+  for (int k = 0; k <= Q_STRIDE; ++k) {
+    const float v = wave_sum(acc[k]);
+    if (lane == 0) kred[wave][k] = v;
+  }
+  __syncthreads();
+  float* out = p.qpool + (size_t)g * QPOOL_STRIDE;
+  if (tid <= Q_STRIDE) out[1 + tid] = (kred[0][tid] + kred[1][tid]) + (kred[2][tid] + kred[3][tid]);
+  if (tid == 0) out[0] = nrows > 0 ? m : -INFINITY;
+}
+
+__global__ __launch_bounds__(1024) void pool_q_head_kernel(PoolParams p) {
+  __shared__ float tail_sm[1024 + 160];
+  __shared__ float wl[1024];
+  __shared__ float red[48];
+  const int tid = threadIdx.x, lane = tid & 63, wave = tid >> 6;
+  const int K = p.tail.K, n = p.n_groups;
+  TailPre pre;
+  tail_preload(p, pre);
+  float* z = tail_sm + 1024;
+  const float mg = tid < n ? p.qpool[(size_t)tid * QPOOL_STRIDE] : -INFINITY;
+  float m = wave_max(mg);
+  if (lane == 0) red[wave] = m;
+  __syncthreads();
+  m = red[0];
+#pragma unroll
+  for (int i = 1; i < 16; ++i) m = fmaxf(m, red[i]);
+  wl[tid] = mg > -INFINITY ? __expf(mg - m) : 0.f;
+  __syncthreads();
+  if (wave <= Q_STRIDE) {
+    float v = 0.f;
+    for (int g = lane; g < n; g += 64) v += p.qpool[(size_t)g * QPOOL_STRIDE + 1 + wave] * wl[g];
+    v = wave_sum(v);
+    if (lane == 0) red[16 + wave] = v;
+  }
+  __syncthreads();
+  const float l = red[16];
+  float zs = 0.f;
+  if (wave < K && lane == 0) {
+    zs = red[17 + wave] / l;
+    z[wave] = zs + pre.bk;
+  }
+  __syncthreads();
+  head_from_z<true>(p.tail, pre, z);
+  __syncthreads();
+  if (wave < Q_STRIDE && lane == 0) red[32 + wave] = wave < K ? z[wave] * zs : 0.f;
+  __syncthreads();
+  if (tid == 0) {
+    float dmm = 0.f;
+    for (int k = 0; k < K; ++k) dmm += red[32 + k];
+    p.qstats[QSTAT_M] = m; p.qstats[QSTAT_L] = l; p.qstats[QSTAT_DMM] = dmm;
+    p.stats[0] = m; p.stats[1] = l;
+  }
+  if (tid < Q_STRIDE) p.qstats[QSTAT_DZ + tid] = tid < K ? z[tid] : 0.f;
+  head_grads<false>(p, pre, tail_sm, z);
+}
+
+__global__ __launch_bounds__(256) void pool_m_kernel(const float* pw, const float* h, int64_t N, int H, float* M_part,
+                                                     int rows_per_group) {
+  __shared__ __align__(16) float vred[1024];
+  const int tid = threadIdx.x, g = blockIdx.x;
+  const int64_t r0 = (int64_t)g * rows_per_group;
+  const int64_t r1 = r0 + rows_per_group < N ? r0 + rows_per_group : N;
+  const int nrows = r1 > r0 ? (int)(r1 - r0) : 0;
+  const int VPR = H / 4, RG = 256 / VPR;
+  const int cv = tid % VPR, rg = tid / VPR;
+  float4 v = zero4();
+  int i = rg;
+  for (; i + 7 * RG < nrows; i += 8 * RG) {
+    float4 hv[8];
+    float e[8];
+#pragma unroll
+    for (int u = 0; u < 8; ++u) hv[u] = ld4(h + (size_t)(r0 + i + u * RG) * H + 4 * cv);
+#pragma unroll
+    for (int u = 0; u < 8; ++u) e[u] = pw[r0 + i + u * RG];
+#pragma unroll
+    for (int u = 0; u < 8; ++u) { v.x += e[u] * hv[u].x; v.y += e[u] * hv[u].y; v.z += e[u] * hv[u].z; v.w += e[u] * hv[u].w; }
+  }
+  for (; i < nrows; i += RG) {
+    const float e = pw[r0 + i];
+    const float4 hv = ld4(h + (size_t)(r0 + i) * H + 4 * cv);
+    v.x += e * hv.x; v.y += e * hv.y; v.z += e * hv.z; v.w += e * hv.w;
+  }
+  st4(vred + (rg * VPR + cv) * 4, v);
+  __syncthreads();
+  if (tid < VPR) {
+    float4 s = zero4();
+    for (int q = 0; q < RG; ++q) {
+      const float4 t = ld4(vred + (q * VPR + tid) * 4);
+      s.x += t.x; s.y += t.y; s.z += t.z; s.w += t.w;
+    }
+    st4(M_part + (size_t)g * H + 4 * tid, s);
+  }
 }
 
 __global__ __launch_bounds__(256) void score_sum_kernel(const float* s_part, int n_parts, const float* bc, float* A, int64_t N) {
@@ -749,6 +970,7 @@
   if (p.K % KC != 0 || (p.nseg > 1 && p.kseg % KC != 0)) return MMF_ERR_SHAPE;
   if (p.N % 4 != 0) return MMF_ERR_SHAPE;
   if (p.ldx % 4 != 0) return MMF_ERR_ALIGN;
+  if (p.q_part && (SEG || p.split || p.act != ACT_RELU || !p.wk || p.Kq < 1 || p.Kq > Q_STRIDE)) return MMF_ERR_ARG;
   if (p.M <= 0) return MMF_OK;
   const LinearPlan pl = plan_linear(p.M, p.N, p.K, p.nseg, p.kseg, p.allow_half, p.concurrent, p.split,
                                     p.kpart && p.ktick ? p.ktick_words : 0);
@@ -756,7 +978,9 @@
   auto go = [&](auto tile) -> int {
     using T = decltype(tile);
     void (*kern)(LinearParams);
-    if constexpr (T::SPLIT) kern = linear_nt_split_kernel<T>; else kern = linear_nt_kernel<T, SEG>;
+    if constexpr (T::SPLIT) kern = linear_nt_split_kernel<T>;
+    else if constexpr (SEG) kern = linear_nt_kernel<T, true>;
+    else kern = p.q_part ? linear_nt_q_kernel<T> : linear_nt_kernel<T, false>;
     return launch_tiled<T>(T::SPLIT ? "linear_nt_split_kernel" : "linear_nt_kernel", kern, p, pl.grid, st);
   };
   switch (pl.kind) {
@@ -873,6 +1097,27 @@
   return launch_pool_merge(p, st);
 }
 
+int launch_pool_q(PoolParams p, hipStream_t st) {
+  if (p.H != 256 && p.H != 512 && p.H != 1024) return MMF_ERR_SHAPE;
+  if (!p.q_part || !p.qpool || !p.qstats || !p.stats || !p.tail.Wk || !p.tail.Y || !p.tail.dM || !p.tail.dbk) return MMF_ERR_ARG;
+  if (p.tail.K < 1 || p.tail.K > Q_STRIDE || p.q_parts < 1) return MMF_ERR_SHAPE;
+  p.n_groups = pool_groups(p.N);
+  p.rows_per_group = (int)((p.N + p.n_groups - 1) / p.n_groups);
+  if (p.rows_per_group > POOL_MAX_ROWS || p.n_groups > 1024) return MMF_ERR_SHAPE;
+  { ProfScope ps("pool_q_partial_kernel", st); hipLaunchKernelGGL(pool_q_partial_kernel, dim3(p.n_groups), dim3(256), 0, st, p); }
+  { ProfScope ps("pool_q_head_kernel", st); hipLaunchKernelGGL(pool_q_head_kernel, dim3(1), dim3(1024), 0, st, p); }
+  return hipGetLastError() == hipSuccess ? MMF_OK : MMF_ERR_LAUNCH;
+}
+
+int launch_pool_m(const float* pw, const float* h, int64_t N, int H, float* M_part, int n_groups, hipStream_t st) {
+  if (H != 256 && H != 512 && H != 1024) return MMF_ERR_SHAPE;
+  if (!pw || !h || !M_part || n_groups < 1) return MMF_ERR_ARG;
+  const int rows_per_group = (int)((N + n_groups - 1) / n_groups);
+  ProfScope ps("pool_m_kernel", st);
+  hipLaunchKernelGGL(pool_m_kernel, dim3(n_groups), dim3(256), 0, st, pw, h, N, H, M_part, rows_per_group);
+  return hipGetLastError() == hipSuccess ? MMF_OK : MMF_ERR_LAUNCH;
+}
+
 int launch_pool_merge(PoolParams p, hipStream_t st) {
   if (p.n_groups < 1 || p.n_groups > MERGE_MAX_GROUPS || p.H > 1024 || p.H % 32 != 0) return MMF_ERR_SHAPE;
   if (p.tail.Wk && (p.tail.K < 1 || p.tail.K > 32)) return MMF_ERR_SHAPE;
diff --git a/multimodalfusion_amd/csrc/mmf_api.hip b/multimodalfusion_amd/csrc/mmf_api.hip
--- a/multimodalfusion_amd/csrc/mmf_api.hip
+++ b/multimodalfusion_amd/csrc/mmf_api.hip
@@ -116,6 +116,7 @@
   float *h, *a, *b, *s_part, *partials, *stats, *p, *ds, *dbc_part, *du;
   float *slab_w1, *slab_wab, *cs_b1, *cs_bab, *cs_wc;
   float* kpart;
+  float *q_part, *qpool, *qstats;
   int parts, groups, mstk;
   TnPlan tn;
   size_t bytes;
@@ -156,6 +157,9 @@
   w.cs_b1 = take((size_t)splits * H);
   w.cs_bab = take((size_t)w.tn.splits_g * w.mstk);
   w.cs_wc = take((size_t)w.tn.splits_g * D);
+  w.q_part = take((size_t)(H / 64) * N * Q_STRIDE);
+  w.qpool = take((size_t)w.groups * QPOOL_STRIDE);
+  w.qstats = take(QSTAT_FLOATS);
   w.bytes = c.off;
   return w;
 }
@@ -222,6 +226,10 @@
   lp.split = d->gemm == MMF_GEMM_BF16X3;
   lp.kpart = w.kpart; lp.ktick = d->sync; lp.ktick_words = d->sync ? d->sync_words : 0;
   return lp;
+}
+
+static int stack_q_parts(const mmf_amil_desc* d) {
+  return plan_linear(d->N, d->H, d->L, 1, d->L, 1, d->concurrent ? 1 : 0, 0, 0).nt_count;
 }
 
 static GateFwdParams stack_gate_fwd(const mmf_amil_desc* d, const AmilWs& w, uint32_t seed) {
@@ -429,7 +437,8 @@
 }
 
 static int amil_forward_impl(const mmf_amil_desc* d, const float* x, void* workspace, size_t workspace_bytes,
-                             float* M, float* A_raw, void* stream, bool infer, const HeadTail* tail = nullptr) {
+                             float* M, float* A_raw, void* stream, bool infer, const HeadTail* tail = nullptr,
+                             bool qroute = false) {
   if (int e = check_desc(d)) return e;
   if (int e = check_operands(d, x, workspace, A_raw, false)) return e;
   Carver c(workspace);
@@ -439,11 +448,17 @@
   hipStream_t st = static_cast<hipStream_t>(stream);
   TraceScope ts(d->trace);
 
-  if (int e = launch_linear(stack_linear(d, w, x, d->seed), st)) return e;
+  LinearParams lp = stack_linear(d, w, x, d->seed);
+  if (qroute) { lp.wk = tail->Wk; lp.Kq = tail->K; lp.q_part = w.q_part; }
+  if (int e = launch_linear(lp, st)) return e;
   if (int e = launch_gate_fwd(stack_gate_fwd(d, w, d->seed), st)) return e;
   PoolParams pp = stack_pool(d, w, A_raw);
   pp.partials = w.partials; pp.M = M; pp.stats = w.stats;
   if (tail) { pp.tail = *tail; pp.tail.dM = w.dM_step; }
+  if (qroute) {
+    pp.q_part = w.q_part; pp.q_parts = stack_q_parts(d); pp.qpool = w.qpool; pp.qstats = w.qstats;
+    return launch_pool_q(pp, st);
+  }
   return launch_pool(pp, st);
 }
 
@@ -465,7 +480,7 @@
 
 static int amil_backward_impl(const mmf_amil_desc* d, const float* x, void* workspace, size_t workspace_bytes,
                               const float* M, const float* A_raw, const float* dM, const float* gA,
-                              const mmf_amil_grads* g, void* stream, int accumulate) {
+                              const mmf_amil_grads* g, void* stream, int accumulate, const HeadTail* qtail = nullptr) {
   if (int e = check_desc(d)) return e;
   if (!x || !workspace || !A_raw || !g) return MMF_ERR_ARG;
   if (int e = check_grads(d, g)) return e;
@@ -482,15 +497,21 @@
   BwdDhParams dp = stack_dh(d, w, gc, dM);
   const DhPlan pl = dh_plan(dp, true);
   int dbc_groups = pl.dbc_groups;
+  const int q_parts = qtail ? stack_q_parts(d) : 0;
   if (pl.fused) {
     dp.A_raw = A_raw; dp.stats = w.stats; dp.Mpool = M; dp.gA = gA;
     dp.p_out = w.p; dp.ds_out = w.ds; dp.dbc_part = w.dbc_part;
+    if (qtail) { dp.q_part = w.q_part; dp.q_parts = q_parts; dp.Kq = qtail->K; dp.qstats = w.qstats; }
   } else {
-    const BwdPrepParams bp = stack_prep(d, w, A_raw, w.stats, M, dM, gA);
+    BwdPrepParams bp = stack_prep(d, w, A_raw, w.stats, M, dM, gA);
+    if (qtail) { bp.q_part = w.q_part; bp.q_parts = q_parts; bp.Kq = qtail->K; bp.qstats = w.qstats; }
     dbc_groups = bp.n_groups;
     if (int e = launch_bwd_prep(bp, st)) return e;
   }
   if (int e = launch_bwd_dh(pl, dp, st)) return e;
+  if (qtail) {
+    if (int e = launch_pool_m(w.p, w.h, d->N, d->H, w.partials, w.groups, st)) return e;
+  }
   if (g->dx) {
     if (int e = launch_nn(stack_dx(d, w, g->dx), st)) return e;
   }
@@ -501,6 +522,12 @@
 
   ReduceList rl;
   stack_reduce(d, w, g, dbc_groups, rl);
+  if (qtail) {
+    if (rl.add(w.partials, qtail->dWk, d->H, w.groups, (size_t)d->H) == MMF_OK) {
+      ReduceSeg& sg = rl.p.seg[rl.p.nseg - 1];
+      sg.scale = w.qstats + QSTAT_DZ; sg.nscale = qtail->K;
+    }
+  }
   return rl.launch(accumulate, st);
 }
 
@@ -674,8 +701,10 @@
     return amil_bf16_backward_impl(d, xb, workspace, workspace_bytes, nullptr, A_raw, nullptr, nullptr, grads, stream, acc);
   }
   const float* xf = static_cast<const float*>(x);
-  if (int e = amil_forward_impl(d, xf, workspace, workspace_bytes, nullptr, A_raw, stream, false, &tl)) return e;
-  return amil_backward_impl(d, xf, workspace, workspace_bytes, nullptr, A_raw, nullptr, nullptr, grads, stream, acc);
+  const bool qroute = d->gemm == MMF_GEMM_F32 && tl.K <= Q_STRIDE && aligned16(tl.Wk) && !grads->dx;
+  if (int e = amil_forward_impl(d, xf, workspace, workspace_bytes, nullptr, A_raw, stream, false, &tl, qroute)) return e;
+  return amil_backward_impl(d, xf, workspace, workspace_bytes, nullptr, A_raw, nullptr, nullptr, grads, stream, acc,
+                            qroute ? &tl : nullptr);
 }
 
 namespace mmf {
diff --git a/multimodalfusion_amd/csrc/mmf_kernels.h b/multimodalfusion_amd/csrc/mmf_kernels.h
--- a/multimodalfusion_amd/csrc/mmf_kernels.h
+++ b/multimodalfusion_amd/csrc/mmf_kernels.h
@@ -32,7 +32,27 @@
   unsigned* ktick;
   int ktick_words;
   const uint32_t* seg_ridx;
-};
+  const float* wk;
+  int Kq;
+  float* q_part;
+};
+constexpr int Q_STRIDE = 8;
+constexpr int QPOOL_STRIDE = 16;
+enum : int { QSTAT_M = 0, QSTAT_L = 1, QSTAT_DMM = 2, QSTAT_DZ = 4, QSTAT_FLOATS = 16 };
+__device__ inline void q_row(const float* q_part, int q_parts, int64_t N, int64_t row, int K, float (&q)[Q_STRIDE]) {
+#pragma unroll
+  for (int k = 0; k < Q_STRIDE; ++k) q[k] = 0.f;
+  for (int t = 0; t < q_parts; ++t) {
+    const float* src = q_part + ((size_t)t * (size_t)N + (size_t)row) * Q_STRIDE;
+    const float4 lo = ld4(src);
+    const float4 hi = K > 4 ? ld4(src + 4) : zero4();
+    q[0] += lo.x; q[1] += lo.y; q[2] += lo.z; q[3] += lo.w;
+    q[4] += hi.x; q[5] += hi.y; q[6] += hi.z; q[7] += hi.w;
+  }
+#pragma unroll
+  for (int k = 0; k < Q_STRIDE; ++k) q[k] = k < K ? q[k] : 0.f;
+}
+
 enum : int { LIN_SPLIT_WIDE, LIN_WIDE, LIN_128, LIN_SPLIT_64, LIN_KSPLIT_64, LIN_64 };
 struct LinearPlan {
   int kind;
@@ -91,6 +111,9 @@
   float* stats;
   int n_groups, rows_per_group;
   HeadTail tail;
+  const float* q_part;
+  int q_parts;
+  float *qpool, *qstats;
 };
 constexpr int POOL_MAX_ROWS = 8192;
 
@@ -107,6 +130,9 @@
   float* ds;
   float* dbc_part;
   int n_groups;
+  const float* q_part;
+  int q_parts, Kq;
+  const float* qstats;
 };
 
 struct GateBwdCtx {
@@ -171,6 +197,9 @@
   int fused_prep;
   const float *A_raw, *stats, *Mpool, *gA;
   float *p_out, *ds_out, *dbc_part;
+  const float* q_part;
+  int q_parts, Kq;
+  const float* qstats;
   const uint32_t* seg_ridx;
   const int* seg_bag;
 };
@@ -215,7 +244,7 @@
   const float* segx[4]; int kseg;
 };
 
-struct ReduceSeg { const float* in; float* out; int len; int nsplit; size_t stride; int block_begin; int tall; };
+struct ReduceSeg { const float* in; float* out; int len; int nsplit; size_t stride; int block_begin; int tall; const float* scale; int nscale; };
 struct ReduceParams { ReduceSeg seg[12]; int nseg; int accumulate; };
 
 int launch_linear(LinearParams p, hipStream_t st);
@@ -239,6 +268,8 @@
 int launch_head_tail(PoolParams p, hipStream_t st);
 int launch_pool_merge(PoolParams p, hipStream_t st);
 int launch_bwd_prep(BwdPrepParams p, hipStream_t st);
+int launch_pool_q(PoolParams p, hipStream_t st);
+int launch_pool_m(const float* pw, const float* h, int64_t N, int H, float* M_part, int n_groups, hipStream_t st);
 
 constexpr int PREP_GROUPS = 512;
 enum : int { DH_SPLIT_WIDE, DH_SPLIT_64, DH_WIDE, DH_128, DH_64X128, DH_64 };
```

Result: no change. 1371 bags/s (-0.8%).
